# mitsuba-renderer/mitsuba2

Measured on AMD Instinct MI355X. Metric: Msamples/sec (whole node), 1080p/512spp path integrator, higher is better.
Workload: dtype f32

## Files before the change

mitsuba2_amd/csrc/device/resident_kernel.h:

```cpp
#ifndef MIW_KERNEL
#define MIW_KERNEL __global__
#endif
MIW_KERNEL __launch_bounds__(MIW_BLOCK) void k_init_pixels(RenderParams P, U4 *st_out, uint32_t *pixel_out, InitArgs A) {
    uint32_t lane = blockIdx.x * blockDim.x + threadIdx.x;
    if (lane >= P.n_lanes) return;
    uint32_t tile = lane >> A.bs2_log2, i = lane & ((1u << A.bs2_log2) - 1u);
    uint32_t b = A.tile_list ? A.tile_list[tile] : tile;
    uint32_t bx = b % A.blocks_x, by = b / A.blocks_x;
    uint32_t x, y;
    morton_decode2(i, x, y);
    int32_t bw = P.film.crop_w - (int32_t) (bx * A.bs), bh = P.film.crop_h - (int32_t) (by * A.bs);
    if (bw > (int32_t) A.bs) bw = (int32_t) A.bs;
    if (bh > (int32_t) A.bs) bh = (int32_t) A.bs;
    if ((int32_t) x >= bw || (int32_t) y >= bh) {
        U4 st; st.x = st.y = 0; st.z = LF_DONE; st.w = 0;
        st_out[lane] = st; pixel_out[lane] = 0;
        return;
    }
    uint32_t px = (uint32_t) P.film.crop_x + bx * A.bs + x, py = (uint32_t) P.film.crop_y + by * A.bs + y;
    pixel_out[lane] = px | (py << 16);
    st_out[lane] = lane_seed_state(A.base_seed + (uint64_t) A.block_ids[b] * (uint64_t) (A.bs * A.bs) + i);
}

struct TileArgs {
// ... 15 lines not shown
        ticks = 0; quarter = 0; tail_prio = 0; sample_end_ = spp;
        if (Jobs) job_pend() = 0u;
        if (Placed && Q->simd_ids) {
            const uint32_t hw = (uint32_t) __builtin_amdgcn_s_getreg(4 | (0 << 6) | (31 << 11)),
                           xcc = (uint32_t) __builtin_amdgcn_s_getreg(20 | (0 << 6) | (3 << 11));
            const uint32_t key = ((xcc & 15u) << 10) | (((hw >> 13) & 7u) << 7) | (((hw >> 12) & 1u) << 6) | (((hw >> 8) & 15u) << 2) | ((hw >> 4) & 3u);
            if (nq > 1u) { const uint32_t id = Q->simd_ids[1u + key]; q = id < nq ? id : key % nq; }
            else if ((threadIdx.x & 63u) == 0u) Q->simd_ids[1u + key] = 1u;
        }
    }
    uint32_t ticks, quarter, tail_prio, sample_end_; uint32_t *prog;
    __device__ __forceinline__ void tick(uint32_t sample_idx, bool has_pixel) {
        if (!tail_prio) { ++ticks; return; }
        if ((uint32_t) __builtin_amdgcn_readfirstlane((int) ++ticks) & 15u) return;
        if (has_pixel) atomicMin(prog, sample_idx);
        const uint32_t v = *prog;
        *prog = 0xffffffffu;
        const uint32_t v4 = 4u * v, se = sample_end_;
        uint32_t qtr = v == 0xffffffffu ? 3u : (v4 >= se ? 1u : 0u) + (v4 >= 2u * se ? 1u : 0u) + (v4 >= 3u * se ? 1u : 0u);
        qtr = (uint32_t) __builtin_amdgcn_readfirstlane((int) qtr);
        if (qtr == quarter) return;
        quarter = qtr;
        if (qtr == 0u) __builtin_amdgcn_s_setprio(3); else if (qtr == 1u) __builtin_amdgcn_s_setprio(2);
        else if (qtr == 2u) __builtin_amdgcn_s_setprio(1); else __builtin_amdgcn_s_setprio(0);
    }
    __device__ __forceinline__ void enable_tail_prio(uint32_t sample_end, uint32_t *wave_word) {
        tail_prio = 1u; sample_end_ = sample_end; quarter = 0; prog = wave_word; *prog = 0xffffffffu; __builtin_amdgcn_s_setprio(3);
    }
    typedef uint32_t U4v __attribute__((ext_vector_type(4)));
    __device__ __forceinline__ static uint32_t &job_pend() { __shared__ uint32_t s_job_pend[MIW_BLOCK]; return s_job_pend[threadIdx.x & (MIW_BLOCK - 1)]; }
    __device__ __forceinline__ bool exhausted() const { return !Jobs || !Q->job_chunk || job_pend() == 0xffffffffu; }
    __device__ __forceinline__ uint32_t job_end(uint32_t sample_idx, uint32_t sample_end) const {
        const uint32_t r = spp - sample_idx;
        return Jobs && (r & (r - 1u)) == 0u && r >= Q->job_min ? sample_idx : sample_end;
    }
    __device__ __forceinline__ bool fetch_job(uint32_t &pixel, U4 &st) {
        for (;;) {
            const uint32_t parked = job_pend();
            if (parked == 0xffffffffu) return false;
            uint32_t id = parked - 1u;
            const bool fresh = parked == 0u;
            const unsigned long long b = __ballot(fresh);
            if (fresh) {
                const uint32_t me = threadIdx.x & 63u, leader = (uint32_t) __ffsll((long long) b) - 1u;
                uint32_t base = 0;
                if (me == leader) base = atomicAdd(next_pixel, (uint32_t) __popcll(b));
                base = (uint32_t) __shfl((int) base, (int) leader, 64);
                id = base + __builtin_amdgcn_mbcnt_hi((uint32_t) (b >> 32), __builtin_amdgcn_mbcnt_lo((uint32_t) b, 0u));
                if (id >= Q->job_total) { job_pend() = 0xffffffffu; return false; }
            }
            const uint32_t j = id / n_lanes, slot = id - j * n_lanes;
            const uint32_t px = Q->pixel[slot];
            U4v w;
#if defined(__HIP_DEVICE_COMPILE__)
            asm volatile("global_load_dwordx4 %0, %1, off sc1\n\ts_waitcnt vmcnt(0)" : "=&v"(w) : "v"(Q->st + slot) : "memory");
#endif
            if (w.z & LF_DONE) { job_pend() = 0u; continue; }
            if (w.w != (j ? spp - (Q->job_pow >> (j - 1u)) : 0u)) { job_pend() = id + 1u; return false; }
            job_pend() = 0u;
            lane = slot; pixel = px;
            st.x = w.x; st.y = w.y; st.z = w.z; st.w = w.w;
            return true;
        }
    }
    __device__ __forceinline__ bool fetch(uint32_t &pixel, U4 &st) {
        if (Jobs && Q->job_chunk) return fetch_job(pixel, st);
        for (;;) {
            if (!Placed) {
                const unsigned long long b = __ballot(1);
                const uint32_t me = threadIdx.x & 63u, leader = (uint32_t) __ffsll((long long) b) - 1u;
                uint32_t base = 0;
                if (me == leader) base = atomicAdd(next_pixel, (uint32_t) __popcll(b));
                base = (uint32_t) __shfl((int) base, (int) leader, 64);
                const uint32_t l = base + __builtin_amdgcn_mbcnt_hi((uint32_t) (b >> 32), __builtin_amdgcn_mbcnt_lo((uint32_t) b, 0u));
                if (l >= n_lanes) return false;
                lane = l;
                st = Q->st[lane];
                if (st.z & LF_DONE) continue;
                pixel = Q->pixel[lane];
                return true;
            }
            if (dry >= nq) {
                if (nq > 1u) Q->simd_ids[0] = 1u;
                return false;
            }
            if (nq > 1u && __hip_atomic_load(Q->simd_ids, __ATOMIC_RELAXED, __HIP_MEMORY_SCOPE_AGENT)) { dry = nq; return false; }
            const unsigned long long all = __ballot(1);
            const uint32_t me = threadIdx.x & 63u, leader = (uint32_t) __ffsll((long long) all) - 1u;
            const uint32_t q_lead = (uint32_t) __shfl((int) q, (int) leader, 64);
            const bool mine = q == q_lead;
            const unsigned long long b = __ballot(mine);
            if (!mine) continue;
            uint32_t base = 0;
            if (me == leader) base = atomicAdd(next_pixel + q, (uint32_t) __popcll(b));
            base = (uint32_t) __shfl((int) base, (int) leader, 64);
            const uint32_t idx = base + __builtin_amdgcn_mbcnt_hi((uint32_t) (b >> 32), __builtin_amdgcn_mbcnt_lo((uint32_t) b, 0u));
            uint32_t l = idx;
            if (nq > 1u) {
                const uint32_t piece = idx < per ? Q->piece_list[q * MIW_PLACE_PIECES + (idx >> 6)] : 0xffffffffu;
                if (piece == 0xffffffffu) { q = q + 1u == nq ? 0u : q + 1u; ++dry; continue; }
                l = Q->lane_sorted[piece * Q->piece_a + (idx & 63u) * Q->piece_b];
                if (l >= n_lanes) continue;
            } else if (l >= n_lanes) { ++dry; continue; }
            lane = l;
            st = Q->st[lane];
            if (st.z & LF_DONE) continue;
            pixel = Q->pixel[lane];
            if (Placed) t_fetch = cost_clock();
            return true;
        }
    }
    __device__ __forceinline__ uint32_t cost_clock() const {
        return Clock ? (uint32_t) (__builtin_amdgcn_s_memtime() >> 8) : ticks;
    }
    __device__ __forceinline__ void store(U4 st) {
        if (Jobs && Q->job_chunk) {
            unsigned long long *words = reinterpret_cast<unsigned long long *>(Q->st + lane);
            __hip_atomic_store(words, (unsigned long long) st.x | ((unsigned long long) st.y << 32), __ATOMIC_RELAXED, __HIP_MEMORY_SCOPE_AGENT);
            asm volatile("s_waitcnt vmcnt(0)" ::: "memory");
            __hip_atomic_store(words + 1, (unsigned long long) st.z | ((unsigned long long) st.w << 32), __ATOMIC_RELAXED, __HIP_MEMORY_SCOPE_AGENT);
            return;
        }
        Q->st[lane] = st;
        if (Placed && Q->lane_cost) Q->lane_cost[lane] = cost_clock() - t_fetch + 1u;
        if (Groups && Q->group_done && (st.z & LF_DONE)) {
            __threadfence();
            const uint32_t g = lane >> Q->group_shift;
            if (atomicAdd(Q->group_done + g, 1u) + 1u == Q->group_expected[g]) {
                __threadfence_system();
                __hip_atomic_store(Q->group_flag + g, 1u, __ATOMIC_RELEASE, __HIP_MEMORY_SCOPE_SYSTEM);
            }
        }
    }
    __device__ __forceinline__ void put(uint32_t pixel, uint32_t sample_idx, V2 pos, const float *aovs) {
        if (Q->log_rec) {
            LogSink16<const float *> sink{ Q->log_rec, thr, film, lane, spp, Q->log_rej & 255u, Q->log_rej >> 8 };
            sink(pixel, sample_idx, pos, aovs);
        } else {
            LogSink sink; sink.log_pos = Q->log_pos; sink.log_val = Q->log_val; sink.lane = lane; sink.spp = spp; sink.warn_negative = warn_negative;
            sink(0u, sample_idx, pos, aovs);
        }
    }
};

#ifndef MIW_DIRECT_WAVES
#define MIW_DIRECT_WAVES 3
#endif
#ifndef MIW_PACKET_WAVES_ALL
#define MIW_PACKET_WAVES_ALL 4
#endif
#ifndef MIW_PACKET_WAVES
#define MIW_PACKET_WAVES 5
#endif
template <bool UseLog, int Tiny, int Mats = MATS_ALL, bool Analytic = (Tiny == 0), uint32_t Integ = INTEG_PATH, bool Groups = false, int Waves = 0>
__global__ __launch_bounds__(MIW_BLOCK, Waves ? Waves : Integ == INTEG_DIRECT ? MIW_DIRECT_WAVES : Tiny ? ((Mats == MATS_DIFFUSE && !MIW_SPECTRAL) ? (Tiny == 2 ? MIW_PACKET_WAVES : 4) : MIW_PACKET_WAVES_ALL) : MIW_TREE_WAVES) void k_path_resident(RenderParams P, SceneView sc, LaneQueues Q, double *accum, Counters *cnt,
                                                               TraceLds cfg, uint32_t sample_end, TileArgs T, uint32_t *next_pixel) {
    extern __shared__ uint4 smem[];
    stage_to_lds(sc, cfg, smem);
    const float *thr = stage_thresholds(smem, cfg, UseLog && Q.log_rec ? Q.log_thr : nullptr);
    constexpr bool Frames = MIW_LDS_TABLES && UseLog && Tiny != 0 && Integ != INTEG_DIRECT;
#if MIW_LDS_TABLES
    if constexpr (UseLog && Tiny != 0) stage_tables<true, mats_lights(Mats), mats_full(Mats), Frames>(sc, cfg, smem);
#endif
#if defined(MIW_SECTION_PROFILE) && defined(__HIP_DEVICE_COMPILE__)
    if ((threadIdx.x & 63u) == 0) { unsigned long long *b_ = miw_sec_buf(); for (int i = 0; i < 15; ++i) b_[i] = 0; b_[15] = __builtin_amdgcn_s_memtime(); }
#endif
    const uint32_t lane = blockIdx.x * blockDim.x + threadIdx.x;
    double *tile = reinterpret_cast<double *>(smem + T.geom16);
    int tile_x0 = 0, tile_y0 = 0;
    if (!UseLog && T.side) {
        const uint32_t lane0 = blockIdx.x * blockDim.x, t = lane0 >> T.bs2_log2, q0 = lane0 & ((1u << T.bs2_log2) - 1u);
        const uint32_t b = T.tile_list ? T.tile_list[t] : t;
        uint32_t qx, qy;
        morton_decode2(q0, qx, qy);
        const int margin = (int) (T.side - 16u) / 2;
        tile_x0 = (int) ((b % T.blocks_x) * T.bs + qx) - margin;
        tile_y0 = (int) ((b / T.blocks_x) * T.bs + qy) - margin;
        for (uint32_t i = threadIdx.x; i < T.side * T.side * MIW_FILM_CHANNELS; i += blockDim.x) tile[i] = 0.0;
        __syncthreads();
    }
    LaneCounters local; local.segments = local.samples = local.shadow_rays = 0;
    auto tr2 = [&](V3 o, float mint, V3 dE, float maxtE, bool hasE, V3 dS, float maxtS, bool hasS, F4 &hE, bool &occS) {
        trace2<Tiny, Analytic, Integ != INTEG_DIRECT>(sc, cfg, smem, o, mint, dE, maxtE, hasE, dS, maxtS, hasS, hE, occS);
    };
    if (UseLog) {
        QueueWork<Tiny != 0, false, Groups> work; work.Q = &Q; work.next_pixel = next_pixel; work.n_lanes = P.n_lanes; work.spp = P.spp; work.lane = 0; work.warn_negative = P.film.warn_negative;
        work.film = &P.film; work.thr = thr; work.init_queues(cfg.queues ? cfg.queues : 1u);
        __shared__ uint32_t s_prog[MIW_BLOCK / 64];
        if (cfg.tail_prio) work.enable_tail_prio(sample_end, &s_prog[threadIdx.x >> 6]);
        if constexpr (Integ == INTEG_DIRECT) pixel_stream_render_direct<Mats, Analytic>(P, sc, sample_end, work, tr2, &local);
        else pixel_stream_render<Mats, Analytic, Frames>(P, sc, sample_end, work, tr2, &local);
    } else if (lane < P.n_lanes) {
        U4 st = Q.st[lane];
        if (!(st.z & LF_DONE)) {
            const uint32_t pixel = Q.pixel[lane];
            if (T.side) {
                TileAdd add; add.tile = tile; add.x0 = tile_x0; add.y0 = tile_y0; add.side = (int) T.side;
                SplatXYSink<TileAdd> sink; sink.film = &P.film; sink.add = add;
                st = pixel_render<Integ, mats_nested(Mats) ? Mats : MATS_ALL>(P, sc, pixel, st, sample_end, tr2, sink, &local);
            } else {
                FilmAdd add; add.accum = accum;
                SplatSink<FilmAdd> sink; sink.film = &P.film; sink.add = add;
                st = pixel_render<Integ, mats_nested(Mats) ? Mats : MATS_ALL>(P, sc, pixel, st, sample_end, tr2, sink, &local);
            }
            Q.st[lane] = st;
        }
    }
    if (!UseLog && T.side) {
        __syncthreads();
        const int n = (int) (T.side * T.side);
        for (int i = (int) threadIdx.x; i < n * MIW_FILM_CHANNELS; i += (int) blockDim.x) {
            const double v = tile[i];
            if (v == 0.0) continue;
            const int texel = i / MIW_FILM_CHANNELS, k = i - texel * MIW_FILM_CHANNELS;
            const int fx = tile_x0 + texel % (int) T.side, fy = tile_y0 + texel / (int) T.side;
            unsafeAtomicAdd(accum + ((size_t) fy * P.film.crop_w + fx) * MIW_FILM_CHANNELS + k, v);
        }
    }
    unsigned long long a = wave_sum(local.segments), b = wave_sum(local.samples), c = wave_sum(local.shadow_rays);
    if ((threadIdx.x & 63) == 0) {
        Counters *shard = cnt + ((blockIdx.x * (MIW_BLOCK / 64) + (threadIdx.x >> 6)) & (MIW_CNT_SHARDS - 1));
        if (a) atomicAdd(&shard->segments, a);
        if (b) atomicAdd(&shard->samples, b);
        if (c) atomicAdd(&shard->shadow_rays, c);
#if defined(MIW_SECTION_PROFILE) && defined(__HIP_DEVICE_COMPILE__)
        { unsigned long long *b_ = miw_sec_buf(); for (int i = 0; i < 15; ++i) if (b_[i]) atomicAdd(&g_sections[i], b_[i]); }
#endif
    }
}
```

mitsuba2_amd/csrc/kernel_pick.h:

```cpp
#pragma once

namespace miw_pick {

enum : int { ALL = 0, DIFFUSE = 1, PLAIN = 2, TRIO = 3, NESTED = 4, LIGHTS = 5 };

struct Facts {
    bool tiny;
    bool small;
    bool diffuse_only, trio, nested, textured, lights_on;
    bool no_rects;
    bool trio_on;
};

struct Pick {
    int tiny;
    int mats;
    bool analytic;
};
inline bool operator==(const Pick &a, const Pick &b) { return a.tiny == b.tiny && a.mats == b.mats && a.analytic == b.analytic; }

inline bool trio_kernel(const Facts &f) { return f.trio && f.trio_on && f.no_rects && !f.textured; }

inline Pick resident_path(const Facts &f, bool with_trio) {
    if (f.tiny && f.diffuse_only) return { f.small ? 2 : 1, DIFFUSE, false };
    if (f.lights_on) return { f.tiny ? 1 : 0, LIGHTS, !f.tiny };
    if (f.nested) return { f.tiny ? 1 : 0, NESTED, !f.tiny };
    if (f.textured) return { f.tiny ? 1 : 0, ALL, !f.tiny };
    if (f.tiny) return { f.small ? 2 : 1, PLAIN, false };
    if (with_trio && trio_kernel(f)) return { 0, TRIO, false };
    return { 0, PLAIN, !f.no_rects };
}

inline Pick resident_direct(const Facts &f) {
    const int mats = f.lights_on ? LIGHTS : f.nested ? NESTED : f.textured ? ALL : PLAIN;
    return { f.tiny ? 1 : 0, mats, !f.tiny };
}

inline Pick resident_atomic(const Facts &f) {
    return { f.tiny ? 1 : 0, f.lights_on ? LIGHTS : f.nested ? NESTED : ALL, !f.tiny };
}

inline Pick tree_class(const Facts &f) {
    if (f.lights_on) return { 0, LIGHTS, true };
    if (f.nested) return { 0, NESTED, true };
    if (f.textured) return { 0, ALL, true };
    if (trio_kernel(f)) return { 0, TRIO, false };
    return { 0, PLAIN, !f.no_rects };
}

}
```

mitsuba2_amd/csrc/miw/path.h:

```cpp
#pragma once
#include "base.h"
#include "rng.h"
#include "scene.h"
#include "film.h"

namespace miw {

enum : uint32_t {
    LF_DEPTH_MASK  = 0x0fffu,
    LF_VALID_RAY   = 1u << 12,
    LF_PREV_DELTA  = 1u << 13,
    LF_HAS_SHADOW  = 1u << 14,
    LF_RAY_ACTIVE  = 1u << 15,
    LF_DONE        = 1u << 16,
    LF_DEAD_PENDING= 1u << 17,
};

struct LaneQueues {
    F4 *tp;
    F4 *res;
    U4 *st;
    F2 *pos;
    const uint32_t *pixel;
    F4 *ray_o;
    F4 *ray_d;
    F4 *hit;
    F4 *sh_d;
    F4 *sh_c;
    uint32_t *sh_vis;
    F2 *log_pos;
    F4 *log_val;
    U4 *log_rec;
    const float *log_thr;
    uint32_t log_rej;
    uint32_t *lane_cost; const uint32_t *lane_sorted; const uint32_t *piece_list; uint32_t *simd_ids; uint32_t piece_a, piece_b;
    uint32_t *group_done = nullptr; const uint32_t *group_expected = nullptr; uint32_t *group_flag = nullptr; uint32_t group_shift = 0;
    uint32_t job_chunk = 0, job_pow = 0, job_total = 0, job_min = 0x80000000u;
};

enum : uint32_t { INTEG_PATH = 0, INTEG_DIRECT = 1 };
struct DirectRec {
    uint32_t emitter_samples, bsdf_samples, hide_emitters;
    float frac_bsdf, frac_lum, weight_bsdf, weight_lum;
};

struct RenderParams {
    SensorRec sensor;
    FilmRec film;
    uint32_t spp;
    int32_t max_depth, rr_depth;
    uint32_t n_lanes;
    uint32_t integrator;
    DirectRec direct;
    uint32_t moment_pass;
    float cam_o[3];
    float crop_f[4];
};
MIW_HD void render_params_prepare(RenderParams &P) {
    const V3 o = sensor_origin(P.sensor);
    P.cam_o[0] = o.x; P.cam_o[1] = o.y; P.cam_o[2] = o.z;
    P.crop_f[0] = (float) P.film.crop_x; P.crop_f[1] = (float) P.film.crop_y; P.crop_f[2] = (float) P.film.crop_w; P.crop_f[3] = (float) P.film.crop_h;
}

struct Counters {
    unsigned long long segments;
    unsigned long long samples;
    unsigned long long shadow_rays;
    unsigned long long active_lanes;
};
struct LaneCounters { uint32_t segments, samples, shadow_rays; };

MIW_HD float next_1d(PCG32 &r) { return pcg32_next_f32(r); }
MIW_HD V2 next_2d(PCG32 &r) { float a = pcg32_next_f32(r); float b = pcg32_next_f32(r); return v2(a, b); }

struct LaneRegs {
    PCG32 rng;
    uint32_t flags, sample_idx;
    Spec tp, res; float eta, prev_pdf;
    V2 pos;
    Ray ray;
    Wavelengths wl; Spec ray_weight;
};

MIW_HD void lane_begin_sample(const RenderParams &P, uint32_t pixel, LaneRegs &L, uint32_t sample_end) {
    if (L.sample_idx >= sample_end) {
        L.flags = LF_DONE;
        L.ray.o = L.ray.d = v3(0.f); L.ray.mint = 0.f; L.ray.maxt = -1.f;
        return;
    }
    float px = (float) (pixel & 0xffffu), py = (float) (pixel >> 16);
    V2 j = next_2d(L.rng);
    L.pos = v2(px + j.x, py + j.y);
    const float wavelength_sample = next_1d(L.rng);
#if MIW_SPECTRAL
    sample_wavelengths(wavelength_sample, L.wl, L.ray_weight);
#else
    (void) wavelength_sample; L.ray_weight = spec(1.f);
#endif
    V2 adj = v2((L.pos.x - P.crop_f[0]) / P.crop_f[2],
                (L.pos.y - P.crop_f[1]) / P.crop_f[3]);
    L.ray = sensor_sample_ray(P.sensor, adj, v3(P.cam_o[0], P.cam_o[1], P.cam_o[2]));
    L.tp = spec(1.f); L.res = spec(0.f); L.eta = 1.f; L.prev_pdf = 0.f;
    L.flags = 1u | LF_RAY_ACTIVE;
}

template <typename Sink>
MIW_HD void lane_finish_sample(const RenderParams &P, uint32_t pixel, LaneRegs &L, Sink sink) {
#if MIW_SPECTRAL
    V3 xyz = spectrum_to_xyz(L.ray_weight * L.res, L.wl);
#else
    V3 xyz = srgb_to_xyz(L.res);
#endif
    float aovs[5] = { xyz.x, xyz.y, xyz.z, (L.flags & LF_VALID_RAY) ? 1.f : 0.f, 1.f };
    if (P.moment_pass) {
        const float sq[3] = { sqr(xyz.x), sqr(xyz.y), sqr(xyz.z) };
        bool ok = true;
        for (int k = 0; k < 3; ++k) ok = ok && isfinite_(aovs[k]) && isfinite_(sq[k]);
        if (P.moment_pass == 2u) { aovs[0] = sq[0]; aovs[1] = sq[1]; aovs[2] = sq[2]; }
        if (!ok) aovs[0] = __builtin_nanf("");
    }
    sink(pixel, L.sample_idx, L.pos, aovs);
    L.sample_idx++;
}

template <typename Add> struct SplatSink {
    const FilmRec *film; Add add;
    MIW_HD void operator()(uint32_t pixel, uint32_t, V2 pos, const float *aovs) const {
        film_splat(*film, (int) (pixel & 0xffffu), (int) (pixel >> 16), pos, aovs, add);
    }
};
template <typename AddXY> struct SplatXYSink {
    const FilmRec *film; AddXY add;
    MIW_HD void operator()(uint32_t pixel, uint32_t, V2 pos, const float *aovs) const {
        film_splat_xy(*film, (int) (pixel & 0xffffu), (int) (pixel >> 16), pos, aovs, add);
    }
};
struct LogSink {
    F2 *log_pos; F4 *log_val; uint32_t lane, spp;
    uint32_t warn_negative;
    MIW_HD void operator()(uint32_t, uint32_t sample_idx, V2 pos, const float *aovs) const {
        size_t i = (size_t) lane * spp + sample_idx;
        F2 p; p.x = sample_is_valid(aovs, warn_negative != 0) ? pos.x : __builtin_nanf(""); p.y = pos.y;
        F4 v; v.x = aovs[0]; v.y = aovs[1]; v.z = aovs[2]; v.w = aovs[3];
        log_pos[i] = p; log_val[i] = v;
    }
};

#ifndef MIW_LOG_NT
#define MIW_LOG_NT 1
#endif
template <typename Thr>
struct LogSink16 {
    U4 *log_rec; Thr thr; const FilmRec *film; uint32_t lane, spp, rej, il;
    MIW_HD void operator()(uint32_t pixel, uint32_t sample_idx, V2 pos, const float *aovs) const {
        const size_t i = log_index(il, lane, spp, sample_idx);
        U4 r; r.x = r.y = r.z = 0u; r.w = film_pack_meta(rej, rej, false);
        float least = aovs[0];
        bool ok = isfinite_(aovs[0]);
        for (int k = 1; k < MIW_FILM_CHANNELS; ++k) { least = __builtin_fminf(least, aovs[k]); ok = ok & isfinite_(aovs[k]); }
        ok = ok & ((film->warn_negative == 0) | (least >= -1e-5f));
        if (ok) {
            const uint32_t cx = film_class_of(thr, film_phase(*film, pos.x, (int) (pixel & 0xffffu), film->crop_x)),
                           cy = film_class_of(thr, film_phase(*film, pos.y, (int) (pixel >> 16), film->crop_y));
            r.x = f2u(aovs[0]); r.y = f2u(aovs[1]); r.z = f2u(aovs[2]); r.w = film_pack_meta(cx, cy, aovs[3] != 0.f);
        }
#if defined(__HIP_DEVICE_COMPILE__) && MIW_LOG_NT
        typedef uint32_t u4v_ __attribute__((ext_vector_type(4)));
        u4v_ v_; v_.x = r.x; v_.y = r.y; v_.z = r.z; v_.w = r.w;
        __builtin_nontemporal_store(v_, reinterpret_cast<u4v_ *>(log_rec + i));
#else
        log_rec[i] = r;
#endif
    }
};

MIW_HD void lane_load(const LaneQueues &Q, uint32_t lane, LaneRegs &L) {
    U4 st = Q.st[lane];
    L.rng.state = (uint64_t) st.x | ((uint64_t) st.y << 32);
    L.rng.inc = MIW_PCG32_SCALAR_INC;
    L.flags = st.z; L.sample_idx = st.w;
}
#if !MIW_SPECTRAL
MIW_HD void lane_load_path(const LaneQueues &Q, uint32_t lane, LaneRegs &L) {
    F4 a = Q.tp[lane], b = Q.res[lane];
    L.tp = v3(a.x, a.y, a.z); L.eta = a.w;
    L.res = v3(b.x, b.y, b.z); L.prev_pdf = b.w;
    L.pos = v2(0.f, 0.f);
}
MIW_HD void lane_store(const LaneQueues &Q, uint32_t lane, const LaneRegs &L, bool store_pos) {
    U4 st; st.x = (uint32_t) L.rng.state; st.y = (uint32_t) (L.rng.state >> 32);
    st.z = L.flags; st.w = L.sample_idx;
    Q.st[lane] = st;
    F4 a; a.x = L.tp.x; a.y = L.tp.y; a.z = L.tp.z; a.w = L.eta; Q.tp[lane] = a;
    F4 b; b.x = L.res.x; b.y = L.res.y; b.z = L.res.z; b.w = L.prev_pdf; Q.res[lane] = b;
    if (store_pos) { F2 p; p.x = L.pos.x; p.y = L.pos.y; Q.pos[lane] = p; }
    F4 o; o.x = L.ray.o.x; o.y = L.ray.o.y; o.z = L.ray.o.z; o.w = L.ray.mint; Q.ray_o[lane] = o;
    F4 d; d.x = L.ray.d.x; d.y = L.ray.d.y; d.z = L.ray.d.z; d.w = L.ray.maxt; Q.ray_d[lane] = d;
}
MIW_HD void lane_clear_shadow(const LaneQueues &Q, uint32_t lane) {
    F4 dead; dead.x = dead.y = dead.z = 0.f; dead.w = -1.f;
    Q.sh_d[lane] = dead;
}

MIW_HD void lane_init(const RenderParams &P, const LaneQueues &Q, uint32_t lane, uint32_t pixel, uint64_t seed) {
    LaneRegs L;
    pcg32_seed(L.rng, seed, MIW_PCG32_DEFAULT_STREAM);
    L.sample_idx = 0; L.flags = 0;
    L.tp = v3(1.f); L.res = v3(0.f); L.eta = 1.f; L.prev_pdf = 0.f; L.pos = v2(0.f, 0.f);
    L.ray.o = L.ray.d = v3(0.f); L.ray.mint = 0.f; L.ray.maxt = -1.f;
    lane_begin_sample(P, pixel, L, P.spp);
    lane_store(Q, lane, L, true);
    lane_clear_shadow(Q, lane);
    Q.sh_vis[lane] = 0;
}
MIW_HD void lane_init_unused(const LaneQueues &Q, uint32_t lane) {
    LaneRegs L;
    L.rng.state = 0; L.rng.inc = MIW_PCG32_SCALAR_INC; L.sample_idx = 0; L.flags = LF_DONE;
    L.tp = v3(0.f); L.res = v3(0.f); L.eta = 0.f; L.prev_pdf = 0.f; L.pos = v2(0.f, 0.f);
    L.ray.o = L.ray.d = v3(0.f); L.ray.mint = 0.f; L.ray.maxt = -1.f;
    lane_store(Q, lane, L, true);
    lane_clear_shadow(Q, lane);
    Q.sh_vis[lane] = 0;
}
#endif

#ifndef MIW_SECTION
#define MIW_SECTION(i) do { } while (0)
#endif

struct ShadowOut { bool has; V3 d; float maxt; Spec c; };

enum { STEP_CONTINUE = 0,
       STEP_FINISHED = 1,
       STEP_DEAD_PENDING = 2 };

enum { MATS_ALL = 0, MATS_DIFFUSE = 1, MATS_PLAIN = 2, MATS_TRIO = 3, MATS_NESTED = 4, MATS_LIGHTS = 5 };
MIW_HD constexpr bool mats_full(int mats) { return mats == MATS_ALL || mats == MATS_NESTED || mats == MATS_LIGHTS; }
MIW_HD constexpr bool mats_nested(int mats) { return mats == MATS_NESTED || mats == MATS_LIGHTS; }
MIW_HD constexpr bool mats_lights(int mats) { return mats == MATS_LIGHTS; }
template <int Mats = MATS_ALL, bool Analytic = true, bool Frames = false, typename PrevO, typename Cnt>
MIW_HD int path_step(const RenderParams &P, const SceneView &sc, LaneRegs &L, F4 h, PrevO prev_o,
                     ShadowOut &sh, Cnt *cnt_local) {
    sh.has = false;
    const uint32_t depth = L.flags & LF_DEPTH_MASK;
    const uint32_t tri_idx = f2u(h.w);
    const bool valid = tri_idx != MIW_MISS;
    const V3 ray_d = L.ray.d;

    SurfaceInteraction si;
    uint32_t bsdf_index = 0;
    int32_t emitter = -1;
    if (valid) hit_surface_interaction<Analytic, mats_full(Mats), Frames>(sc, tri_idx, h.x, h.y, h.z, prev_o, ray_d, si, bsdf_index, emitter);
    else emitter = miss_emitter<mats_lights(Mats)>(sc);
    if (depth == 1 && valid) L.flags |= LF_VALID_RAY;
    MIW_SECTION(7);

    if (emitter >= 0) {
        float emission_weight = 1.f;
        if (depth > 1) {
            float emitter_pdf = 0.f;
            if (!(L.flags & LF_PREV_DELTA)) {
                V3 d = ray_d; float dist = 0.f; V3 n = v3(0.f), ref_p = v3(0.f);
                if (valid) {
                    ref_p = prev_o();
                    d = si.p - ref_p;
                    dist = norm(d);
                    d = d / dist;
                    n = si.sh.n;
                }
                emitter_pdf = pdf_emitter_direction<Analytic, mats_lights(Mats)>(sc, (uint32_t) emitter, d, dist, n, ref_p);
            }
            emission_weight = mis_weight(L.prev_pdf, emitter_pdf);
        }
        Spec radiance = valid ? emitter_eval(sc.emitters[emitter], si.wi, L.wl) : miss_eval<mats_lights(Mats)>(sc, ray_d, L.wl);
        L.res = L.res + emission_weight * L.tp * radiance;
    }

    MIW_SECTION(8);
    bool active = valid;

    if ((int32_t) depth > P.rr_depth) {
        float q = min_(hmax(L.tp) * sqr(L.eta), .95f);
        active = (next_1d(L.rng) < q) && active;
        L.tp = L.tp * rcp(q);
    }

    if (depth >= (uint32_t) P.max_depth || !active) return STEP_FINISHED;

    if (cnt_local) cnt_local->segments++;
    BsdfSide bsdf;
    if (Mats == MATS_DIFFUSE) { bsdf.b = sc.bsdfs + bsdf_index; bsdf.flip = bsdf.none = false; bsdf.flags = BSDF_DiffuseReflection; }
    else bsdf = bsdf_side<mats_nested(Mats)>(sc.bsdfs, bsdf_index, si.wi);
    const uint32_t bflags = bsdf.flags;
    L.ray.o = si.p; L.ray.mint = spawn_mint(si.p);
    L.ray.d = v3(0.f); L.ray.maxt = -1.f;

    const TexCtx tc(L.wl, si.uv, mats_full(Mats) ? sc.bitmaps : nullptr, mats_full(Mats) ? sc.bsdf_tables : nullptr);
    constexpr bool Ext = mats_full(Mats);
    constexpr bool Trio = Mats == MATS_TRIO;
    constexpr bool Nested = mats_nested(Mats);

    if (bflags & BSDF_Smooth) {
        DirectionSample ds;
        Spec emitter_val = sample_emitter_direction<Analytic, mats_lights(Mats), Frames>(sc, si.p, next_2d(L.rng), ds, L.wl);
        if (ds.pdf != 0.f) {
            V3 wo = to_local(si.sh, ds.d);
            Spec bsdf_val = Mats == MATS_DIFFUSE ? diffuse_eval(*bsdf.b, si.wi, wo, tc) : bsdf_side_eval<Ext, Trio, Nested>(bsdf, si.wi, wo, tc);
            float bpdf = Mats == MATS_DIFFUSE ? diffuse_pdf(si.wi, wo) : bsdf_side_pdf<Ext, Trio, Nested>(bsdf, si.wi, wo, tc);
            float mis = (mats_lights(Mats) && ds.delta) ? 1.f : mis_weight(ds.pdf, bpdf);
            Spec c = mis * L.tp * bsdf_val * emitter_val;
            if (!all_zero(c)) {
                sh.has = true; sh.d = ds.d; sh.maxt = ds.dist * (1.f - MIW_SHADOW_EPSILON); sh.c = c;
                if (cnt_local) cnt_local->shadow_rays++;
            }
        }
    }

    MIW_SECTION(9);
    float s1 = next_1d(L.rng);
    V2 s2 = next_2d(L.rng);
    BSDFSample bs;
    Spec bsdf_val = Mats == MATS_DIFFUSE ? diffuse_sample(*bsdf.b, si.wi, s2, bs, tc) : bsdf_side_sample<Ext, Trio, Nested>(bsdf, si.wi, s1, s2, bs, tc);
    L.tp = L.tp * bsdf_val;
    if (all_zero(L.tp))
        return sh.has ? STEP_DEAD_PENDING : STEP_FINISHED;
    L.eta *= bs.eta;
    L.ray.d = to_world(si.sh, bs.wo);
    L.ray.maxt = MIW_INFINITY;
    L.prev_pdf = bs.pdf;
    L.flags = (L.flags & ~(LF_DEPTH_MASK | LF_PREV_DELTA)) | ((depth + 1) & LF_DEPTH_MASK)
            | ((bs.sampled_type & BSDF_Delta) ? LF_PREV_DELTA : 0u) | LF_RAY_ACTIVE;
    MIW_SECTION(10);
    return STEP_CONTINUE;
}

#if !MIW_SPECTRAL
template <int Mats = MATS_NESTED, typename Sink, typename Cnt>
MIW_HD uint32_t lane_shade(const RenderParams &P, const SceneView &sc, const LaneQueues &Q,
                           uint32_t lane, Cnt *cnt_local, Sink sink) {
    LaneRegs L;
    lane_load(Q, lane, L);
    if (L.flags & LF_DONE) return LF_DONE;
    lane_load_path(Q, lane, L);
    const bool had_shadow = (L.flags & LF_HAS_SHADOW) != 0;

    if (had_shadow) {
        if (Q.sh_vis[lane]) { F4 c = Q.sh_c[lane]; L.res = L.res + v3(c.x, c.y, c.z); }
        L.flags &= ~LF_HAS_SHADOW;
    }

    bool finished = false;

    if (L.flags & LF_DEAD_PENDING) {
        finished = true;
    } else {
        F4 rd = Q.ray_d[lane];
        L.ray.d = v3(rd.x, rd.y, rd.z);
        ShadowOut sh;
        const int r = path_step<Mats>(P, sc, L, Q.hit[lane],
                                [&]() { F4 ro = Q.ray_o[lane]; return v3(ro.x, ro.y, ro.z); }, sh, cnt_local);
        if (sh.has) {
            F4 sd; sd.x = sh.d.x; sd.y = sh.d.y; sd.z = sh.d.z; sd.w = sh.maxt;
            Q.sh_d[lane] = sd;
            F4 sc4; sc4.x = sh.c.x; sc4.y = sh.c.y; sc4.z = sh.c.z; sc4.w = 0.f;
            Q.sh_c[lane] = sc4;
            L.flags |= LF_HAS_SHADOW;
        }
        if (r == STEP_FINISHED) finished = true;
        else if (r == STEP_DEAD_PENDING)
            L.flags = (L.flags & ~LF_RAY_ACTIVE) | LF_DEAD_PENDING;
    }

    bool store_pos = false;
    if (finished) {
        const uint32_t pixel = Q.pixel[lane];
        F2 ps = Q.pos[lane]; L.pos = v2(ps.x, ps.y);
        lane_finish_sample(P, pixel, L, sink);
        if (cnt_local) cnt_local->samples++;
        L.flags = 0;
        lane_begin_sample(P, pixel, L, P.spp);
        store_pos = true;
    }
    lane_store(Q, lane, L, store_pos);
    if (had_shadow && !(L.flags & LF_HAS_SHADOW)) lane_clear_shadow(Q, lane);
    return L.flags;
}
#endif

template <int Mats = MATS_ALL, bool Analytic = true, bool Frames = false, typename Work, typename Trace2, typename Cnt>
MIW_HD void pixel_stream_render(const RenderParams &P, const SceneView &sc, uint32_t sample_end, Work &work,
                                Trace2 trace2, Cnt *cnt_local) {
    LaneRegs L;
    L.flags = LF_DONE; L.sample_idx = 0; L.rng.state = 0; L.rng.inc = MIW_PCG32_SCALAR_INC;
    uint32_t pixel = 0;
    bool have = false, dead_pending = false;
    ShadowOut sh; sh.has = false; sh.d = v3(0.f); sh.maxt = -1.f; sh.c = spec(0.f);
    auto sink = [&work](uint32_t px, uint32_t sample_idx, V2 pos, const float *aovs) { work.put(px, sample_idx, pos, aovs); };
    for (;;) {
        if (L.flags & LF_DONE) {
            if (have) {
                U4 st; st.x = (uint32_t) L.rng.state; st.y = (uint32_t) (L.rng.state >> 32);
                st.z = L.sample_idx >= P.spp ? (uint32_t) LF_DONE : 0u; st.w = L.sample_idx;
                work.store(st);
            }
            U4 st;
            have = work.fetch(pixel, st);
            if (!have) { if (work.exhausted()) break; continue; }
            L.rng.state = (uint64_t) st.x | ((uint64_t) st.y << 32);
            L.sample_idx = st.w; L.flags = 0;
            lane_begin_sample(P, pixel, L, sample_end);
            MIW_SECTION(0);
            continue;
        }
        work.tick(L.sample_idx, true);
        MIW_SECTION(0);
        const V3 o = L.ray.o;
        F4 h; bool occluded = false;
        trace2(o, L.ray.mint, L.ray.d, L.ray.maxt, !dead_pending, sh.d, sh.maxt, sh.has, h, occluded);
        if (sh.has && !occluded) L.res = L.res + sh.c;
        sh.has = false;
        int r = STEP_FINISHED;
        if (!dead_pending) {
            r = path_step<Mats, Analytic, Frames>(P, sc, L, h, [o]() { return o; }, sh, cnt_local);
            MIW_SECTION(4);
            if (r == STEP_DEAD_PENDING) { dead_pending = true; continue; }
            if (r == STEP_CONTINUE) continue;
        }
        dead_pending = false;
        lane_finish_sample(P, pixel, L, sink);
        if (cnt_local) cnt_local->samples++;
        L.flags = 0;
        lane_begin_sample(P, pixel, L, work.job_end(L.sample_idx, sample_end));
        MIW_SECTION(5);
    }
}

MIW_HD void lane_begin_path(LaneRegs &L) {
    L.tp = spec(1.f); L.res = spec(0.f); L.eta = 1.f; L.prev_pdf = 0.f;
    L.flags = 1u | LF_RAY_ACTIVE;
    L.sample_idx = 0; L.pos = v2(0.f, 0.f); L.ray_weight = spec(1.f);
}
template <int Mats = MATS_ALL, bool Analytic = true, typename Feed, typename Trace2, typename Cnt>
MIW_HD void ray_stream_sample(const RenderParams &P, const SceneView &sc, Feed &feed, Trace2 trace2, Cnt *cnt_local) {
    LaneRegs L;
    L.flags = LF_DONE; L.rng.state = 0; L.rng.inc = MIW_PCG32_SCALAR_INC;
    bool dead_pending = false;
    ShadowOut sh; sh.has = false; sh.d = v3(0.f); sh.maxt = -1.f; sh.c = spec(0.f);
    for (;;) {
        if (L.flags & LF_DONE) {
            if (!feed.fetch(L)) break;
            lane_begin_path(L);
            continue;
        }
        const V3 o = L.ray.o;
        F4 h; bool occluded = false;
        trace2(o, L.ray.mint, L.ray.d, L.ray.maxt, !dead_pending, sh.d, sh.maxt, sh.has, h, occluded);
        if (sh.has && !occluded) L.res = L.res + sh.c;
        sh.has = false;
        if (!dead_pending) {
            const int r = path_step<Mats, Analytic>(P, sc, L, h, [o]() { return o; }, sh, cnt_local);
            if (r == STEP_DEAD_PENDING) { dead_pending = true; continue; }
            if (r == STEP_CONTINUE) continue;
        }
        dead_pending = false;
        feed.store(L);
        if (cnt_local) cnt_local->samples++;
        L.flags = LF_DONE;
    }
}

template <int Mats, bool Analytic, typename Feed, typename Trace2, typename Cnt>
MIW_HD void ray_stream_sample_direct(const RenderParams &P, const SceneView &sc, Feed &feed, Trace2 trace2, Cnt *cnt_local);

template <int Mats, bool Analytic, typename Work, typename Trace2, typename Cnt>
MIW_HD void pixel_stream_render_direct(const RenderParams &P, const SceneView &sc, uint32_t sample_end, Work &work,
                                       Trace2 trace2, Cnt *cnt_local);

template <uint32_t Integ = INTEG_PATH, int Mats = MATS_NESTED, typename Trace2, typename Sink, typename Cnt>
MIW_HD U4 pixel_render(const RenderParams &P, const SceneView &sc, uint32_t pixel, U4 st, uint32_t sample_end,
                       Trace2 trace2, Sink sink, Cnt *cnt_local) {
    struct OnePixel {
        uint32_t pixel; U4 st; bool taken; Sink sink;
        MIW_HD bool fetch(uint32_t &px, U4 &s) { if (taken) return false; taken = true; px = pixel; s = st; return true; }
        MIW_HD void store(U4 s) { st = s; }
        MIW_HD bool exhausted() const { return true; }
        MIW_HD uint32_t job_end(uint32_t, uint32_t sample_end) const { return sample_end; }
        MIW_HD void tick(uint32_t, bool) { }
        MIW_HD void put(uint32_t px, uint32_t sample_idx, V2 pos, const float *aovs) { sink(px, sample_idx, pos, aovs); }
    } work{ pixel, st, false, sink };
    if constexpr (Integ == INTEG_DIRECT) pixel_stream_render_direct<Mats, true>(P, sc, sample_end, work, trace2, cnt_local);
    else pixel_stream_render<Mats>(P, sc, sample_end, work, trace2, cnt_local);
    return work.st;
}

MIW_HD U4 lane_seed_state(uint64_t seed) {
    PCG32 r; pcg32_seed(r, seed, MIW_PCG32_DEFAULT_STREAM);
    U4 st; st.x = (uint32_t) r.state; st.y = (uint32_t) (r.state >> 32); st.z = 0; st.w = 0;
    return st;
}

}
```

mitsuba2_amd/csrc/miw/scene.h:

```cpp
#pragma once
#include "base.h"
#include "shape.h"
#include "bsdf.h"
#include "envmap.h"
#include "light.h"

namespace miw {

#define MIW_MISS 0xffffffffu

struct BvhNode {
    float lo0[3], hi0[3];
    float lo1[3], hi1[3];
    int32_t child0, child1;
    int32_t parent;
    int32_t pad;
};

struct ShapeRec {
    uint32_t bsdf;
    int32_t  emitter;
    uint32_t flags;
    uint32_t pad;
};

struct EmitterRec {
    TexRec radiance;
    uint32_t shape;
    uint32_t tri_first;
    uint32_t tri_count;
    uint32_t valid_lo, valid_hi;
    float sum, normalization;
    uint32_t flags;
    uint32_t type;
};
enum : uint32_t { SHAPE_HAS_NORMALS = 1u, SHAPE_HAS_TEXCOORDS = 8u };

struct SceneView {
    const BvhNode *nodes;   uint32_t node_count;
    const Tri     *tris;    uint32_t tri_count;
    const float   *tri_vn;
    const float   *tri_uv;
    const ShapeRec *shapes; uint32_t shape_count;
    const BsdfRec  *bsdfs;  uint32_t bsdf_count;
    const EmitterRec *emitters; uint32_t emitter_count;
    float emitter_count_f, emitter_count_inv;
    const float *emit_tri;
    const float *emit_vnorm;
    const float *emit_pmf, *emit_cdf;
    const EnvmapRec *env;
    const AnalyticRec *rects;   uint32_t rect_count;
    const BitmapRec *bitmaps;
    const float *bsdf_tables;
    float accept_pad;
    const void *tri_bounds;
    const void *leaf_boxes;
    const struct Bvh4Node *nodes4;
    const struct Bvh8Node *nodes8;
    const float *env_top; uint32_t env_top_count, env_top_base;
    const TriFrame *tri_frames;
    const float *emit_face_n;
    const LightRec *lights;
    const LightRec *constant;
};
MIW_HD EnvTop env_top(const SceneView &sc) { EnvTop t; t.p = sc.env_top; t.count = sc.env_top_count; t.base = sc.env_top_base; return t; }
MIW_HD void scene_view_prepare(SceneView &v) {
    v.emitter_count_f = (float) v.emitter_count;
    v.emitter_count_inv = v.emitter_count ? 1.f / (float) v.emitter_count : 0.f;
}

MIW_HD PrimCtx prim_ctx(const SceneView &sc) { PrimCtx c; c.rects = sc.rects; c.accept_pad = sc.accept_pad; return c; }

template <bool Analytic, bool Texcoords, bool Frames = false, typename RayO>
MIW_HD void hit_surface_interaction(const SceneView &sc, uint32_t tri_idx, float t, float u, float v, RayO ray_o, V3 ray_d,
                                    SurfaceInteraction &si, uint32_t &bsdf_index, int32_t &emitter) {
    const Tri &tr = sc.tris[tri_idx];
    const ShapeRec &shape = sc.shapes[tr.shape];
    if (Analytic && tr.pad) {
        const AnalyticRec &a = sc.rects[tr.pad - 1u];
        if (a.kind == ANALYTIC_SPHERE) compute_surface_interaction_sphere(a, t, ray_o(), ray_d, si);
        else compute_surface_interaction_rect(a, t, u, v, ray_o(), ray_d, si);
    } else {
        const float *vn = (shape.flags & 1u) ? sc.tri_vn + 9 * (size_t) tri_idx : nullptr;
        const float *tc = (Texcoords && (shape.flags & SHAPE_HAS_TEXCOORDS)) ? sc.tri_uv + 6 * (size_t) tr.prim : nullptr;
        if constexpr (Frames) compute_surface_interaction(ld3(tr.p0), ld3(tr.p1), ld3(tr.p2), vn, tc, sc.tri_frames[tri_idx], t, u, v, ray_d, si);
        else compute_surface_interaction(ld3(tr.p0), ld3(tr.p1), ld3(tr.p2), vn, tc, t, u, v, ray_d, si);
    }
    si.shape = tr.shape; si.prim = tr.prim;
    emitter = shape.emitter; bsdf_index = shape.bsdf;
}

struct DirectionSample { V3 p, n, d; float dist, pdf; uint32_t emitter; bool delta; };

template <bool Lights = false>
MIW_HD int32_t miss_emitter(const SceneView &sc) {
    if (sc.env) return (int32_t) sc.env->emitter_index;
    if (Lights && sc.constant) return (int32_t) sc.constant->emitter_index;
    return -1;
}

MIW_HD MeshSampler emitter_mesh(const SceneView &sc, const EmitterRec &e) {
    MeshSampler m;
    m.tri = sc.emit_tri + 9 * (size_t) e.tri_first;
    m.vnorm = (e.flags & 1u) ? sc.emit_vnorm + 9 * (size_t) e.tri_first : nullptr;
    m.pmf = sc.emit_pmf + e.tri_first;
    m.cdf = sc.emit_cdf + e.tri_first;
    m.count = e.tri_count;
    m.valid_lo = e.valid_lo; m.valid_hi = e.valid_hi;
    m.sum = e.sum; m.normalization = e.normalization;
    return m;
}

MIW_HD void sphere_sample_direction(const AnalyticRec &r, V3 ref_p, V2 sample, DirectionSample &ds) {
    const V3 center = ld3(r.n);
    const float radius = r.radius;
    V3 dc_v = center - ref_p;
    float dc_2 = squared_norm(dc_v);
    float radius_adj = radius * (r.flip ? (1.f + MIW_RAY_EPSILON) : (1.f - MIW_RAY_EPSILON));
    if (dc_2 > sqr(radius_adj)) {
        float inv_dc = rsqrt(dc_2),
              sin_theta_max = radius * inv_dc,
              sin_theta_max_2 = sqr(sin_theta_max),
              inv_sin_theta_max = rcp(sin_theta_max),
              cos_theta_max = safe_sqrt(1.f - sin_theta_max_2);
        float sin_theta_2 = sin_theta_max_2 > 0.00068523f ? 1.f - sqr(fmadd(cos_theta_max - 1.f, sample.x, 1.f))
                                                          : sin_theta_max_2 * sample.x,
              cos_theta = safe_sqrt(1.f - sin_theta_2);
        float cos_alpha = sin_theta_2 * inv_sin_theta_max + cos_theta * safe_sqrt(fnmadd(sin_theta_2, sqr(inv_sin_theta_max), 1.f)),
              sin_alpha = safe_sqrt(fnmadd(cos_alpha, cos_alpha, 1.f));
        float sin_phi, cos_phi;
        sincos_(sample.y * (2.f * MIW_PI), sin_phi, cos_phi);
        Frame f; f.n = dc_v * -inv_dc;
        coordinate_system(f.n, f.s, f.t);
        V3 d = to_world(f, v3(cos_phi * sin_alpha, sin_phi * sin_alpha, cos_alpha));
        ds.p = v3(fmadd(d.x, radius, center.x), fmadd(d.y, radius, center.y), fmadd(d.z, radius, center.z));
        ds.n = d;
        ds.d = ds.p - ref_p;
        float dist2 = squared_norm(ds.d);
        ds.dist = __builtin_sqrtf(dist2);
        ds.d = ds.d / ds.dist;
        ds.pdf = (.5f * MIW_INV_PI) / (1.f - cos_theta_max);
        if (ds.dist == 0.f) ds.pdf = 0.f;
    } else {
        V3 d = square_to_uniform_sphere(sample);
        ds.p = v3(fmadd(d.x, radius, center.x), fmadd(d.y, radius, center.y), fmadd(d.z, radius, center.z));
        ds.n = d;
        ds.d = ds.p - ref_p;
        float dist2 = squared_norm(ds.d);
        ds.dist = __builtin_sqrtf(dist2);
        ds.d = ds.d / ds.dist;
        ds.pdf = r.inv_area * dist2 / abs_dot(ds.d, ds.n);
    }
    if (r.flip) ds.n = -ds.n;
}
MIW_HD float sphere_pdf_direction(const AnalyticRec &r, V3 ref_p, V3 ds_d, float ds_dist, V3 ds_n) {
    float sin_alpha = r.radius * rcp(norm(ld3(r.n) - ref_p)),
          cos_alpha = safe_sqrt(1.f - sin_alpha * sin_alpha);
    return sin_alpha < (1.f - MIW_EPSILON) ? (.5f * MIW_INV_PI) / (1.f - cos_alpha)
                                           : r.inv_area * sqr(ds_dist) / abs_dot(ds_d, ds_n);
}

#if MIW_SPECTRAL
MIW_HD Spec env_eval_uv_spec(const EnvmapRec &e, V2 uv, const Wavelengths &wl) {
    uv.x *= (float) (e.width - 1u); uv.y *= (float) (e.height - 1u);
    uint32_t px = (uint32_t) uv.x, py = (uint32_t) uv.y;
    if (px > e.width - 2u) px = e.width - 2u;
    if (py > e.height - 2u) py = e.height - 2u;
    const float w1x = uv.x - (float) px, w1y = uv.y - (float) py, w0x = 1.f - w1x, w0y = 1.f - w1y;
    const float *p = e.data + 4 * ((size_t) px + (size_t) py * e.width);
    const float *q = p + 4 * (size_t) e.width;
    const float f0 = fmadd(w0x, p[3], w1x * p[7]), f1 = fmadd(w0x, q[3], w1x * q[7]);
    const float f = fmadd(w0y, f0, w1y * f1);
    Spec r;
    for (int i = 0; i < MIW_SPEC_N; ++i) {
        const float l = wl.l[i];
        const float s00 = srgb_model_eval(p, l), s10 = srgb_model_eval(p + 4, l),
                    s01 = srgb_model_eval(q, l), s11 = srgb_model_eval(q + 4, l);
        const float s0 = fmadd(w0x, s00, w1x * s10), s1 = fmadd(w0x, s01, w1x * s11);
        const float sv = fmadd(w0y, s0, w1y * s1);
        const float wp = d65_eval(1.f * (1.f / 10568.f), l);
        r.c[i] = sv * wp * f * e.scale;
    }
    return r;
}
MIW_HD Spec env_eval_spec(const EnvmapRec &e, V3 d_world, const Wavelengths &wl) {
    return env_eval_uv_spec(e, env_dir_to_uv(xf_vector(e.to_local, d_world)), wl);
}
MIW_HD Spec env_sample_direction_spec(const EnvmapRec &e, V3 ref_p, V2 sample, V3 &d_out, float &dist_out, float &pdf_out,
                                      V3 &p_out, V3 &n_out, const Wavelengths &wl, EnvTop top = env_top_none()) {
    float pdf;
    V2 uv = hier2d_sample(e, sample, pdf, top);
    float theta = uv.y * MIW_PI, phi = uv.x * (2.f * MIW_PI);
    float st, ct, sp, cp;
    sincos_(theta, st, ct); sincos_(phi, sp, cp);
    V3 d = v3(cp * st, sp * st, ct);
    d = v3(d.y, d.z, -d.x);
    float dist = 2.f * e.radius;
    float inv_sin_theta = env_inv_sin_theta(d);
    d = xf_vector(e.to_world, d);
    p_out = ref_p + d * dist;
    n_out = -d;
    float ds_pdf = pdf > 0.f ? pdf * inv_sin_theta * (1.f / (2.f * sqr(MIW_PI))) : 0.f;
    d_out = d; dist_out = dist; pdf_out = ds_pdf;
    return env_eval_uv_spec(e, uv, wl) / ds_pdf;
}
#else
MIW_HD Spec env_sample_direction_spec(const EnvmapRec &e, V3 ref_p, V2 sample, V3 &d, float &dist, float &pdf, V3 &p, V3 &n, const Wavelengths &,
                                      EnvTop top = env_top_none()) {
    return env_sample_direction(e, ref_p, sample, d, dist, pdf, p, n, top);
}
MIW_HD Spec env_eval_spec(const EnvmapRec &e, V3 d, const Wavelengths &) { return env_eval(e, d); }
#endif

template <bool Analytic = true, bool Lights = false, bool Frames = false>
MIW_HD Spec emitter_sample_direction(const SceneView &sc, uint32_t index, V3 ref_p, V2 sample, DirectionSample &ds, const Wavelengths &wl) {
    const EmitterRec &e = sc.emitters[index];
    Spec value;
    ds.emitter = index;
    if (Lights) ds.delta = false;
    if (Lights && e.type >= EMITTER_POINT) {
        LightSample ls;
        value = light_sample_direction(sc.lights[e.tri_first], ref_p, sample, ls, wl);
        ds.p = ls.p; ds.n = ls.n; ds.d = ls.d; ds.dist = ls.dist; ds.pdf = ls.pdf; ds.delta = ls.delta;
    } else if (e.type == EMITTER_ENVMAP) {
        value = env_sample_direction_spec(*sc.env, ref_p, sample, ds.d, ds.dist, ds.pdf, ds.p, ds.n, wl, env_top(sc));
    } else {
        if (Analytic && (e.flags & 2u) && sc.rects[e.tri_first].kind == ANALYTIC_SPHERE) {
            sphere_sample_direction(sc.rects[e.tri_first], ref_p, sample, ds);
        } else {
            PositionSample ps;
            if (Analytic && (e.flags & 2u)) ps = rect_sample_position(sc.rects[e.tri_first], sample);
            else if constexpr (Frames) ps = mesh_sample_position(emitter_mesh(sc, e), sample, FaceNormalTable{ sc.emit_face_n + 4 * (size_t) e.tri_first });
            else ps = mesh_sample_position(emitter_mesh(sc, e), sample);
            ds.p = ps.p; ds.n = ps.n; ds.pdf = ps.pdf;
            ds.d = ds.p - ref_p;
            float dist_squared = squared_norm(ds.d);
            ds.dist = __builtin_sqrtf(dist_squared);
            ds.d = ds.d / ds.dist;
            float dp = abs_dot(ds.d, ds.n);
            ds.pdf *= (dp != 0.f) ? dist_squared / dp : 0.f;
        }
        bool active = dot(ds.d, ds.n) < 0.f && ds.pdf != 0.f;
        value = tex_eval(e.radiance, wl) / ds.pdf;
        if (!active) value = spec(0.f);
    }
    return value;
}

template <bool Analytic = true, bool Lights = false, bool Frames = false>
MIW_HD Spec sample_emitter_direction(const SceneView &sc, V3 ref_p, V2 sample, DirectionSample &ds, const Wavelengths &wl) {
    if (sc.emitter_count == 0) {
        ds.p = ds.n = ds.d = v3(0.f); ds.dist = 0.f; ds.pdf = 0.f; ds.emitter = 0;
        if (Lights) ds.delta = false;
        return spec(0.f);
    }
    uint32_t index = 0;
    float emitter_pdf = 1.f;
    if (sc.emitter_count > 1) {
        float n = sc.emitter_count_f;
        emitter_pdf = sc.emitter_count_inv;
        uint32_t i = (uint32_t) (sample.x * n);
        index = i < sc.emitter_count - 1 ? i : sc.emitter_count - 1;
        sample.x = (sample.x - (float) index * emitter_pdf) * n;
    }
    Spec value = emitter_sample_direction<Analytic, Lights, Frames>(sc, index, ref_p, sample, ds, wl);
    if (sc.emitter_count > 1) {
        ds.pdf *= emitter_pdf;
        value = value * rcp(emitter_pdf);
    }
    return value;
}

template <bool Analytic = true, bool Lights = false>
MIW_HD float emitter_pdf_direction(const SceneView &sc, uint32_t emitter, V3 ds_d, float ds_dist, V3 ds_n, V3 ref_p) {
    const EmitterRec &e = sc.emitters[emitter];
    if (Lights && e.type >= EMITTER_POINT) return light_pdf_direction(sc.lights[e.tri_first]);
    if (e.type == EMITTER_ENVMAP) return env_pdf_direction(*sc.env, ds_d);
    float dp = dot(ds_d, ds_n);
    bool active = dp < 0.f;
    float pdf;
    if (Analytic && (e.flags & 2u) && sc.rects[e.tri_first].kind == ANALYTIC_SPHERE) {
        pdf = sphere_pdf_direction(sc.rects[e.tri_first], ref_p, ds_d, ds_dist, ds_n);
    } else {
        pdf = e.normalization;
        float adp = abs_dot(ds_d, ds_n);
        pdf *= (adp != 0.f) ? (ds_dist * ds_dist) / adp : 0.f;
    }
    return active ? pdf : 0.f;
}
template <bool Analytic = true, bool Lights = false>
MIW_HD float pdf_emitter_direction(const SceneView &sc, uint32_t emitter, V3 ds_d, float ds_dist, V3 ds_n, V3 ref_p) {
    float value = emitter_pdf_direction<Analytic, Lights>(sc, emitter, ds_d, ds_dist, ds_n, ref_p);
    if (sc.emitter_count > 1) value = value * sc.emitter_count_inv;
    return value;
}

MIW_HD Spec emitter_eval(const EmitterRec &e, V3 wi, const Wavelengths &wl) {
    return wi.z > 0.f ? tex_eval(e.radiance, wl) : spec(0.f);
}
template <bool Lights = false>
MIW_HD Spec miss_eval(const SceneView &sc, V3 ray_d, const Wavelengths &wl) {
    if (Lights && !sc.env) return light_eval(*sc.constant, wl);
    return env_eval_spec(*sc.env, ray_d, wl);
}


MIW_HD float mis_weight(float pdf_a, float pdf_b) {
    pdf_a *= pdf_a; pdf_b *= pdf_b;
    return pdf_a > 0.f ? pdf_a / (pdf_a + pdf_b) : 0.f;
}

struct SensorRec {
    float sample_to_camera[16];
    float to_world[16];
    float near_clip, far_clip;
    float pp_offset[2];
};

MIW_HD V3 sensor_origin(const SensorRec &s) { return xf_point_affine(s.to_world, v3(0.f)); }
MIW_HD Ray sensor_sample_ray(const SensorRec &s, V2 position_sample, V3 origin) {
    V3 near_p = xf_point_persp(s.sample_to_camera,
                               v3(position_sample.x + s.pp_offset[0],
                                  position_sample.y + s.pp_offset[1], 0.f));
    V3 d = normalize(near_p);
    float inv_z = rcp(d.z);
    Ray r;
    r.mint = s.near_clip * inv_z;
    r.maxt = s.far_clip * inv_z;
    r.o = origin;
    r.d = xf_vector(s.to_world, d);
    return r;
}
MIW_HD Ray sensor_sample_ray(const SensorRec &s, V2 position_sample) { return sensor_sample_ray(s, position_sample, sensor_origin(s)); }

}
```

mitsuba2_amd/csrc/miwave.hip:

```cpp
#include <hip/hip_runtime.h>
#include <stdio.h>
#include <stdlib.h>
#include <string.h>
#include <stdarg.h>
#include <string>
#include <vector>
#include <chrono>
#include <atomic>
#include <cmath>
#include <map>
#include <string>
#include <algorithm>

#include "../../include/miwave.h"
#include "kernel_pick.h"
#if defined(MIW_CLASS_PART) || defined(MIW_AOV_UNIT)
#define MIW_KERNELS_ONLY 1
#endif
#if defined(MIW_SECTION_PROFILE)
__device__ unsigned long long g_sections[16];
#endif
#if defined(MIW_PHASE_STATS)
__device__ unsigned long long g_phase_stats[15];
#endif
#if defined(MIW_WALK_STATS)
__device__ unsigned long long g_walk_stats[8];
__device__ float g_walk_statsf[8];
#endif
#if defined(MIW_VERIFY_FILTER)
__device__ unsigned int g_verify_n;
__device__ float g_verify[16 * 16];
#endif
#if defined(MIW_SECTION_PROFILE) && defined(__HIP_DEVICE_COMPILE__)
__device__ __forceinline__ unsigned long long *miw_sec_buf() { __shared__ unsigned long long b[4][16]; return &b[threadIdx.x >> 6][0]; }
#define MIW_SECTION(i) do { const unsigned long long now_ = __builtin_amdgcn_s_memtime(); unsigned long long *b_ = miw_sec_buf(); \
        if ((threadIdx.x & 63u) == (unsigned) __ffsll((long long) __ballot(1)) - 1u) { b_[i] += now_ - b_[15]; b_[15] = now_; } } while (0)
#endif
#include "miw/base.h"
#include "miw/rng.h"
#include "miw/warp.h"
#include "miw/special.h"
#include "miw/shape.h"
#include "miw/bsdf.h"
#include "miw/scene.h"
#include "miw/film.h"
#include "miw/bvh.h"
#include "miw/path.h"
#include "miw/direct.h"
#if defined(MIW_KERNELS_ONLY)
#include "miw/bvh4.h"
#include "miw/bvh8.h"
#define MIW_KERNEL static __global__
#else
#include "rect_build.h"
#include "miw/film_gather.h"
#include "texture_build.h"
#include "bvh_build.h"
#include "bvh4_build.h"
#include "envmap_build.h"
#include "film_classes.h"
#include "lbvh_device.h"
#include "sah_device.h"
#include "bvh4_device.h"
#include "bvh8_device.h"
#include "film_reduce.h"
#endif

using namespace miw;

static_assert(sizeof(BvhNode) == 64, "BvhNode must be one 64-byte line");
static_assert(sizeof(Tri) == 48, "Tri must be 48 bytes");
static_assert(sizeof(BsdfRec) == 128 && sizeof(mi_bsdf) == 128, "bsdf record layout");
static_assert(sizeof(TexRec) == sizeof(mi_texture), "texture record layout");

#define MIW_BLOCK 256
#ifndef MIW_POOL_NW
#define MIW_POOL_NW 12
#endif
#define MIW_CNT_SHARDS 1024
#define MIW_BRUTE_MAX_LEAF 2
#define MIW_BRUTE_MAX_TRIS 64
#define MIW_PLACE_PIECES 4

#include "device/trace.h"
#include "device/wavefront_kernels.h"
#include "device/resident_kernel.h"
#include "device/phased_kernel.h"
#if !defined(MIW_KERNELS_ONLY)
#if !MIW_SPECTRAL
#include "device/pooled_kernel.h"
#endif
#include "device/stream_trace.h"
#include "device/film_kernels.h"
#endif
#include "device/eval_kernels.h"
#include "device/sample_kernel.h"
#include "device/class_instances.h"
#if defined(MIW_AOV_UNIT) || !defined(MIW_KERNELS_ONLY)
#include "miw/aov.h"
#include "miw/film_gather_n.h"
#include "device/aov_launch.h"
#if defined(MIW_AOV_UNIT) || !defined(MIW_SPLIT_AOV)
#include "device/aov_kernel.h"
#endif
#endif

#if !defined(MIW_KERNELS_ONLY)
__global__ void k_iota(uint32_t *out, uint32_t n) { const uint32_t i = blockIdx.x * blockDim.x + threadIdx.x; if (i < n) out[i] = i; }


template <typename T> struct DevBuf {
    T *p = nullptr; size_t n = 0;
    hipError_t resize(size_t count) {
        if (count <= n && p) return hipSuccess;
        if (p) (void) hipFree(p);
        p = nullptr; n = 0;
        if (count == 0) return hipSuccess;
        hipError_t e = hipMalloc((void **) &p, count * sizeof(T));
        if (e == hipSuccess) n = count;
        return e;
    }
    hipError_t upload(const std::vector<T> &v, hipStream_t s) {
        hipError_t e = resize(std::max<size_t>(v.size(), 1));
        if (e != hipSuccess || v.empty()) return e;
        return hipMemcpyAsync(p, v.data(), v.size() * sizeof(T), hipMemcpyHostToDevice, s);
    }
    void release() { if (p) (void) hipFree(p); p = nullptr; n = 0; }
};

template <typename T> struct TmpBuf : DevBuf<T> { TmpBuf() = default; TmpBuf(const TmpBuf &) = delete; ~TmpBuf() { this->release(); } };

struct KnobInfo { const char *name, *what; };
static const KnobInfo g_knobs[] = {
    { "MIW_DEBUG", "1: diagnostics on stderr (LDS layout, builder statistics, phase statistics of -DMIW_PHASE_STATS builds)" },
    { "MIW_DEBUG_ALLOC", "1: mi_bvh_build times its uploads and allocations" },
    { "MIW_DEVICE_BUILDER", "mi_bvh_build quality 0: sah (default) | lbvh: which device builder runs" },
    { "MIW_SAH_HUGE", "0: the device SAH sweep bins every candidate in one workgroup (round 4's form)" },
    { "MIW_LBVH_LEAF", "radix tree: triangles per leaf" },
    { "MIW_MAX_LEAF", "host SAH builder: triangles per leaf" },
    { "MIW_NO_STACK", "1: no LDS-stack walk (stackless BVH2 walk, wavefront plan)" },
    { "MIW_BVH4", "0: no 4-wide tree (the phase machine steps through the BVH2)" },
    { "MIW_BVH4_FAN", "2 | 3 | 4: widest node the 4-wide collapse may build" },
    { "MIW_BVH4_HOST", "1: the 4-wide tree is collapsed on the host from the read-back BVH2" },
    { "MIW_BVH8", "0: mi_bvh_build skips the 8-wide tree / mi_render keeps the 4-wide walk" },
    { "MIW_STACK8_FULL", "1: the 8-wide walk keeps the 16-entry LDS column instead of one entry per tree level" },
    { "MIW_ENV_TOP", "0: the environment warp's top levels are not staged in LDS" },
    { "MIW_PHASED", "0: tree scenes take the lock-step kernel instead of the phase machine" },
    { "MIW_PHASED_WAVES", "3 | 4: wavefronts per SIMD the phase machine is launched for" },
    { "MIW_TRIO", "0: MATS_PLAIN kernels where the MATS_TRIO class would do" },
    { "MIW_SHADE_VOTE", "num:den of the phase machine's shade vote" },
    { "MIW_LOOP_EXIT", "node:triangle hand-over ratios of the phase machine's walk loops" },
    { "MIW_POOLED", "1: tree scenes take k_path_pooled (walk jobs pooled across the workgroup; experimental, slower: DESIGN.md)" },
    { "MIW_POOL_SHAPE", "12x1 | 8x2: wavefronts per workgroup x pixels per lane of k_path_pooled" },
    { "MIW_POOL_VOTE", "shade_min:walk_min:node_min:tri_min:claim_min of k_path_pooled" },
    { "MIW_TAIL_PRIO", "0: no least-progress-first wave priorities" },
    { "MIW_WG_PER_CU", "workgroups per CU of the packet kernels' persistent grid" },
    { "MIW_PLACE", "0: shards of about one pixel per lane skip the measuring launch + placed queues" },
    { "MIW_JOB_CHUNK", "smallest chunk of a full frame's pixel jobs, in samples (a power of two; default 64, the phase machine 32): the pixels' sample streams are cut into halving chunks drawn chunk-major from one queue; 0: a job = all the samples of a pixel" },
    { "MIW_JOB_CHUNK_FORCE", "1: chunk jobs whatever the frame's size (tests of the hand-over between lanes)" },
    { "MIW_PACKET_SHARD4", "0: a plain-diffuse packet job of at most four wavefronts of pixels per SIMD keeps the five-wavefront (96-register) kernel" },
    { "MIW_PLACE_MEASURE", "divisor: the measuring launch runs spp / divisor samples" },
    { "MIW_PLACE_SPREAD", "0 | 1: placed pieces = consecutive sorted lanes | one lane of every cost stratum" },
    { "MIW_STREAM", "0: plan 1 walks with one kernel per list slice instead of the persistent stream kernel" },
    { "MIW_FILM_LEGACY", "1: the 24-byte position log + k_film_blocks for every filter" },
    { "MIW_FILM_LANES", "0 | 1 | 2: k_film_lanes off / over the tile-interleaved log / over [lane][sample]" },
    { "MIW_FILM_QUADS", "0 | 24 | 28 | 42 | 44: k_film_quads group shape (0: off)" },
    { "MIW_FILM_COLUMNS", "0 | 42 | 44 | 82: k_film_columns group shape" },
    { "MIW_FILM_GROUP", "2 | 3 | 4: k_film_groups group shape" },
    { "MIW_FL_NT", "0: k_film_lanes reads the log with plain instead of streaming loads" },
    { "MIW_FILM_OVERLAP", "1: part of the film replay of a full Cornell-class frame is queued on three more streams beside the path kernel, sets of 64-tile groups each behind the flags their last pixels raise (default 0: measured +0 - 1 %); 2: without the waits (timing probe: the film is the previous frame's)" },
    { "MIW_FILM_OVERLAP_SET", "groups of 64 tiles per launch of that replay (default 4)" },
    { "MIW_FILM_OVERLAP_ROOM", "workgroups the path kernel's grid is short of filling the device while the replay runs beside it (default 32: one per CU on 32 CUs)" },
    { "MIW_FILM_OVERLAP_LEAN", "0: the launches of that replay are the 168-register kernel (default 1: the 128-register form)" },
    { "MIW_FILM_OVERLAP_BESIDE", "groups of 64 tiles replayed beside the path kernel; the rest in one launch after it (default: three quarters)" },
    { "MIW_FILM_OVERLAP_PRIO", "s_setprio of the replay wavefronts that run beside the path kernel, 0 .. 3 (default 0)" },
    { "MIW_FQ_U", "2 | 4 | 8: records per trip of k_film_quads" },
    { "MIW_RCCL", "0: mi_film_reduce never uses RCCL (device add)" },
    { "MIW_RCCL_FORCE", "1: mi_film_reduce takes the RCCL branch for one context too (tests)" }
};
struct Options {
    std::map<std::string, std::string> v;
    void from_env() { for (const KnobInfo &k : g_knobs) if (const char *e = getenv(k.name)) v[k.name] = e; }
    static bool known(const char *name) { for (const KnobInfo &k : g_knobs) if (!strcmp(k.name, name)) return true; return false; }
    const char *get(const char *name) const { auto it = v.find(name); return it == v.end() ? nullptr : it->second.c_str(); }
    bool off(const char *name) const { const char *e = get(name); return e && atoi(e) == 0; }
    bool on(const char *name) const { const char *e = get(name); return e && atoi(e) != 0; }
    int num(const char *name, int unset) const { const char *e = get(name); return e ? atoi(e) : unset; }
};

struct mi_ctx {
    int device = 0;
    Options opt;
    hipStream_t stream = nullptr;
    std::string error;
    std::atomic<int> cancel{0};

    std::vector<Tri> tris_in;
    std::vector<float> tri_vn_in;
    std::vector<float> tri_uv_in;
    std::vector<ShapeRec> shapes;
    std::vector<AnalyticRec> rects;
    std::vector<BsdfRec> bsdfs; bool diffuse_only = false;
    bool trio = false;
    bool nested = false;
    bool textured = false;
    std::vector<float> bsdf_tables; DevBuf<float> d_bsdf_tables;
    std::vector<EmitterRec> emitters;
    std::vector<LightRec> lights; DevBuf<LightRec> d_lights; int32_t constant_light = -1;
    bool lights_on = false;
    std::vector<float> emit_tri, emit_vnorm, emit_pmf, emit_cdf;
    bool have_scene = false, have_bvh = false;

    DevBuf<BvhNode> d_nodes; DevBuf<Tri> d_tris; DevBuf<float> d_tri_vn, d_tri_uv, d_bitmap_data; DevBuf<BitmapRec> d_bitmaps; uint32_t bitmap_count = 0;
    DevBuf<ShapeRec> d_shapes; DevBuf<BsdfRec> d_bsdfs; DevBuf<EmitterRec> d_emitters; DevBuf<AnalyticRec> d_rects;
    DevBuf<float> d_emit_tri, d_emit_vnorm, d_emit_pmf, d_emit_cdf;
    DevBuf<LeafBox> d_leaf_boxes; DevBuf<TriBounds> d_tri_bounds; DevBuf<Bvh4Node> d_nodes4; uint32_t nodes4_count = 0, nodes4_stack = 0;
    DevBuf<Bvh8Node> d_nodes8; DevBuf<Tri> d_tris8; DevBuf<float> d_tri_vn8; uint32_t nodes8_count = 0, nodes8_depth = 0;
    DevBuf<float> d_env_data, d_env_levels; DevBuf<EnvmapRec> d_env; EnvmapRec env_host{}; size_t env_levels_total = 0;
    bool have_env = false;
    SceneView view{};
    TraceLds lds_cfg{}; size_t lds_bytes = 0;

    DevBuf<F4> q_tp, q_res, q_ray_o, q_ray_d, q_hit, q_sh_d, q_sh_c;
    DevBuf<U4> q_st; DevBuf<F2> q_pos; DevBuf<uint32_t> q_pixel, q_sh_vis;
    DevBuf<double> d_accum; DevBuf<unsigned char> d_out;
    DevBuf<F2> q_log_pos; DevBuf<F4> q_log_val;
    DevBuf<U4> q_log_rec;
    FilmClasses classes; FilmRec classes_of{}; bool classes_valid = false;
    DevBuf<float> d_fc_thr, d_fc_w;
    DevBuf<uint32_t> d_next_pixel; int cu_count = 256;
    DevBuf<uint32_t> d_lane_cost, d_cost_sorted, d_lane_iota, d_lane_sorted, d_piece_list, d_simd_ids;
    DevBuf<unsigned char> d_place_tmp;
    DevBuf<uint32_t> d_lists, d_list_counts;
    DevBuf<uint32_t> d_block_ids, d_tile_list; DevBuf<int32_t> d_block_tile; DevBuf<float> d_tiles;
    DevBuf<Counters> d_cnt;
    Counters *h_cnt = nullptr;
    std::vector<uint32_t> h_piece_list, h_simd_ids;
    hipStream_t stream2[3] = { nullptr, nullptr, nullptr }; hipEvent_t ev_fork = nullptr, ev_join[3] = { nullptr, nullptr, nullptr };
    DevBuf<uint32_t> d_group_done, d_group_expected; uint32_t *h_group_flag = nullptr; uint32_t group_flag_cap = 0;
    std::vector<uint32_t> h_group_expected; std::vector<int32_t> h_block_tile;
    int overlap_state = -1;
    bool replay_enqueued = false;
    uint32_t replay_launches = 0;

    DevBuf<unsigned char> d_sample_stage; DevBuf<uint32_t> d_next_ray;

    std::vector<hipEvent_t> ev_pool;
    mi_counters counters{};
};

static mi_status fail(mi_ctx *c, mi_status code, const char *fmt, ...) {
    char buf[512];
    va_list ap; va_start(ap, fmt); vsnprintf(buf, sizeof buf, fmt, ap); va_end(ap);
    if (c) c->error = buf;
    return code;
}
#define HIP_TRY(c, expr) do { hipError_t e_ = (expr); if (e_ != hipSuccess) \
    return fail(c, MI_ERR_DEVICE, "%s failed: %s (%s:%d)", #expr, hipGetErrorString(e_), __FILE__, __LINE__); } while (0)

static thread_local std::string g_global_error;

extern "C" {

int32_t mi_spectrum_channels(void) { return MIW_SPEC_N; }

mi_status mi_device_count(int32_t *count) {
    if (!count) return MI_ERR_INVALID;
    int n = 0;
    hipError_t e = hipGetDeviceCount(&n);
    if (e != hipSuccess) { *count = 0; g_global_error = hipGetErrorString(e); return MI_ERR_DEVICE; }
    *count = n;
    return MI_OK;
}

mi_status mi_create(int32_t device, mi_ctx **out) {
    if (!out) return MI_ERR_INVALID;
    *out = nullptr;
    int n = 0;
    if (hipGetDeviceCount(&n) != hipSuccess || n <= 0) { g_global_error = "no HIP device visible"; return MI_ERR_DEVICE; }
    if (device < 0 || device >= n) { g_global_error = "device index out of range"; return MI_ERR_INVALID; }
    if (hipSetDevice(device) != hipSuccess) { g_global_error = "hipSetDevice failed"; return MI_ERR_DEVICE; }
    mi_ctx *c = new mi_ctx();
    c->device = device;
    c->opt.from_env();
    { hipDeviceProp_t prop; if (hipGetDeviceProperties(&prop, device) == hipSuccess && prop.multiProcessorCount > 0) c->cu_count = prop.multiProcessorCount; }
    if (hipHostMalloc((void **) &c->h_cnt, sizeof(Counters) * MIW_CNT_SHARDS) != hipSuccess) { delete c; g_global_error = "hipHostMalloc failed"; return MI_ERR_DEVICE; }
    *out = c;
    g_live_contexts.fetch_add(1);
    return MI_OK;
}

void mi_destroy(mi_ctx *c) {
    if (!c) return;
    (void) hipSetDevice(c->device);
    (void) hipDeviceSynchronize();
    c->d_nodes.release(); c->d_tris.release(); c->d_tri_vn.release(); c->d_tri_uv.release(); c->d_bitmap_data.release(); c->d_bitmaps.release(); c->d_bsdf_tables.release(); c->d_shapes.release(); c->d_rects.release(); c->d_bsdfs.release();
    c->d_emitters.release(); c->d_lights.release(); c->d_leaf_boxes.release(); c->d_tri_bounds.release(); c->d_nodes4.release(); c->d_nodes8.release(); c->d_tris8.release(); c->d_tri_vn8.release(); c->d_env_data.release(); c->d_env_levels.release(); c->d_env.release(); c->d_emit_tri.release(); c->d_emit_vnorm.release(); c->d_emit_pmf.release(); c->d_emit_cdf.release();
    c->q_tp.release(); c->q_res.release(); c->q_ray_o.release(); c->q_ray_d.release(); c->q_hit.release();
    c->q_sh_d.release(); c->q_sh_c.release(); c->q_st.release(); c->q_pos.release(); c->q_pixel.release(); c->q_sh_vis.release();
    c->d_accum.release(); c->d_out.release(); c->d_next_pixel.release(); c->d_lane_cost.release(); c->d_cost_sorted.release(); c->d_lane_iota.release(); c->d_lane_sorted.release(); c->d_place_tmp.release(); c->d_piece_list.release(); c->d_simd_ids.release(); c->d_lists.release(); c->d_list_counts.release(); c->d_block_ids.release(); c->d_tile_list.release(); c->d_cnt.release();
    c->q_log_pos.release(); c->q_log_val.release(); c->q_log_rec.release(); c->d_fc_thr.release(); c->d_fc_w.release(); c->d_block_tile.release(); c->d_tiles.release();
    for (hipEvent_t e : c->ev_pool) (void) hipEventDestroy(e);
    c->d_group_done.release(); c->d_group_expected.release(); c->d_sample_stage.release(); c->d_next_ray.release();
    if (c->h_group_flag) (void) hipHostFree(c->h_group_flag);
    if (c->ev_fork) (void) hipEventDestroy(c->ev_fork);
    for (int i = 0; i < 3; ++i) { if (c->ev_join[i]) (void) hipEventDestroy(c->ev_join[i]); if (c->stream2[i]) (void) hipStreamDestroy(c->stream2[i]); }
    if (c->h_cnt) (void) hipHostFree(c->h_cnt);
    delete c;
    if (g_live_contexts.fetch_sub(1) == 1) rccl_release_comms();
}

mi_status mi_set_stream(mi_ctx *c, void *s) { if (!c) return MI_ERR_INVALID; c->stream = (hipStream_t) s; return MI_OK; }

const char *mi_last_error(mi_ctx *c) { return c ? c->error.c_str() : g_global_error.c_str(); }

mi_status mi_set_option(mi_ctx *c, const char *name, const char *value) {
    if (!c || !name) return MI_ERR_INVALID;
    if (!Options::known(name)) return fail(c, MI_ERR_INVALID, "mi_set_option: unknown option %s", name);
    if (value) c->opt.v[name] = value; else c->opt.v.erase(name);
    return MI_OK;
}
const char *mi_get_option(mi_ctx *c, const char *name) { return c && name ? c->opt.get(name) : nullptr; }
int32_t mi_option_count(void) { return (int32_t) (sizeof(g_knobs) / sizeof(g_knobs[0])); }
const char *mi_option_name(int32_t i) { return i >= 0 && i < mi_option_count() ? g_knobs[i].name : nullptr; }
const char *mi_option_help(int32_t i) { return i >= 0 && i < mi_option_count() ? g_knobs[i].what : nullptr; }

mi_status mi_cancel(mi_ctx *c) { if (!c) return MI_ERR_INVALID; c->cancel.store(1); return MI_OK; }

mi_status mi_get_counters(mi_ctx *c, mi_counters *out) {
    if (!c || !out) return MI_ERR_INVALID;
    *out = c->counters;
    return MI_OK;
}

mi_status mi_film_alloc(mi_ctx *c, uint64_t count, void **film) {
    if (!c || !film) return MI_ERR_INVALID;
    *film = nullptr;
    HIP_TRY(c, hipSetDevice(c->device));
    float *p = nullptr;
    HIP_TRY(c, hipMalloc((void **) &p, std::max<uint64_t>(count, 1) * sizeof(float)));
    hipError_t e = hipMemsetAsync(p, 0, count * sizeof(float), c->stream);
    if (e == hipSuccess) e = hipStreamSynchronize(c->stream);
    if (e != hipSuccess) { (void) hipFree(p); return fail(c, MI_ERR_DEVICE, "mi_film_alloc: %s", hipGetErrorString(e)); }
    *film = p;
    return MI_OK;
}
void mi_film_free(mi_ctx *c, void *film) {
    if (!c || !film) return;
    (void) hipSetDevice(c->device);
    (void) hipFree(film);
}
mi_status mi_film_download(mi_ctx *c, const void *film, float *host, uint64_t count) {
    if (!c || !film || !host) return MI_ERR_INVALID;
    HIP_TRY(c, hipSetDevice(c->device));
    HIP_TRY(c, hipMemcpyAsync(host, film, count * sizeof(float), hipMemcpyDeviceToHost, c->stream));
    HIP_TRY(c, hipStreamSynchronize(c->stream));
    return MI_OK;
}
mi_status mi_film_reduce(mi_ctx *const *ctxs, void *const *films, int32_t n, uint64_t count, int32_t root, int32_t *how) {
    if (how) *how = MI_REDUCE_NONE;
    if (!ctxs || !films || n < 1 || root < 0 || root >= n) return MI_ERR_INVALID;
    for (int32_t i = 0; i < n; ++i) if (!ctxs[i] || !films[i]) return MI_ERR_INVALID;
    mi_ctx *r = ctxs[root];
    for (int32_t i = 0; i < n; ++i) { HIP_TRY(r, hipSetDevice(ctxs[i]->device)); HIP_TRY(r, hipStreamSynchronize(ctxs[i]->stream)); }
    const bool force_rccl = r->opt.on("MIW_RCCL_FORCE");
    if (count == 0 || (n == 1 && !force_rccl)) return MI_OK;
    std::vector<int> devs(n);
    bool distinct = true;
    for (int32_t i = 0; i < n; ++i) { devs[i] = ctxs[i]->device; for (int32_t j = 0; j < i; ++j) distinct = distinct && devs[j] != devs[i]; }
    if (distinct) {
        std::lock_guard<std::mutex> lock(g_rccl_mutex);
        if (g_rccl.load(!r->opt.off("MIW_RCCL"))) {
// ... 114 lines not shown
    if (s->rectangle_count && !s->rectangles) return fail(c, MI_ERR_INVALID, "scene: rectangle_count without rectangles");
    std::vector<int32_t> shape_rect(s->shape_count, -1);
    for (uint32_t k = 0; k < s->rectangle_count; ++k) {
        const mi_rectangle &q = s->rectangles[k];
        if (q.shape >= s->shape_count || !(s->shapes[q.shape].flags & MI_SHAPE_RECTANGLE) || shape_rect[q.shape] >= 0)
            return fail(c, MI_ERR_INVALID, "rectangle %u: shape %u is not a (single) MI_SHAPE_RECTANGLE shape", k, q.shape);
        shape_rect[q.shape] = (int32_t) k;
        c->rects.push_back(rect_record(q.to_world, q.to_object, q.shape, s->shapes[q.shape].first_face));
        if (!(c->rects.back().inv_area > 0.f) || !isfinite_(c->rects.back().inv_area))
            return fail(c, MI_ERR_INVALID, "rectangle %u: degenerate to_world", k);
    }
    if (s->sphere_count && !s->spheres) return fail(c, MI_ERR_INVALID, "scene: sphere_count without spheres");
    for (uint32_t k = 0; k < s->sphere_count; ++k) {
        const mi_sphere &q = s->spheres[k];
        if (q.shape >= s->shape_count || !(s->shapes[q.shape].flags & MI_SHAPE_SPHERE) || shape_rect[q.shape] >= 0)
            return fail(c, MI_ERR_INVALID, "sphere %u: shape %u is not a (single) MI_SHAPE_SPHERE shape", k, q.shape);
        if (!(q.radius > 0.f) || !isfinite_(q.radius)) return fail(c, MI_ERR_INVALID, "sphere %u: radius must be positive", k);
        shape_rect[q.shape] = (int32_t) c->rects.size();
        c->rects.push_back(sphere_record(q.center, q.radius, q.flip_normals != 0, q.to_world, q.to_object, q.shape, s->shapes[q.shape].first_face));
    }
    for (uint32_t i = 0; i < s->shape_count; ++i)
        if ((s->shapes[i].flags & (MI_SHAPE_RECTANGLE | MI_SHAPE_SPHERE)) && shape_rect[i] < 0)
            return fail(c, MI_ERR_INVALID, "shape %u: no mi_rectangle record", i);
    if (!build_face_texcoords(s, c->tri_uv_in)) return fail(c, MI_ERR_INVALID, "scene: MI_SHAPE_HAS_TEXCOORDS without vertex_texcoords (or a vertex index out of range)");
    c->tris_in.resize((size_t) s->face_count + c->rects.size());
    c->tri_vn_in.clear();
    if (any_normals) c->tri_vn_in.assign(c->tris_in.size() * 9, 0.f);
    for (uint32_t f = 0; f < s->face_count; ++f) {
        if (face_shape[f] == 0xffffffffu) return fail(c, MI_ERR_INVALID, "face %u belongs to no shape", f);
        Tri &t = c->tris_in[f];
        if (shape_rect[face_shape[f]] >= 0) {
            Tri two[2];
            analytic_bounding_tris(c->rects[shape_rect[face_shape[f]]], (uint32_t) shape_rect[face_shape[f]], two);
            t = two[0]; c->tris_in[(size_t) s->face_count + shape_rect[face_shape[f]]] = two[1];
            continue;
        }
        for (int k = 0; k < 3; ++k) {
            uint32_t vi = s->faces[3 * f + k];
            if (vi >= s->vertex_count) return fail(c, MI_ERR_INVALID, "face %u: vertex index out of range", f);
            float *dst = k == 0 ? t.p0 : (k == 1 ? t.p1 : t.p2);
            memcpy(dst, s->vertex_positions + 3 * (size_t) vi, 12);
            if (any_normals && (c->shapes[face_shape[f]].flags & 1u))
                memcpy(&c->tri_vn_in[(size_t) f * 9 + 3 * k], s->vertex_normals + 3 * (size_t) vi, 12);
        }
        t.shape = face_shape[f]; t.prim = f; t.pad = 0;
    }
    c->bsdfs.resize(s->bsdf_count);
    for (uint32_t i = 0; i < s->bsdf_count; ++i) {
        const mi_bsdf &b = s->bsdfs[i];
        BsdfRec r; int slot = 0;
        if (s->bsdf_table_floats && !s->bsdf_tables) return fail(c, MI_ERR_INVALID, "scene: bsdf_table_floats without bsdf_tables");
        if (const char *why = bsdf_record_from_abi(b, s->bitmap_count, s->bsdf_table_floats, r, &slot))
            return slot < 0 ? fail(c, MI_ERR_INVALID, "bsdf %u: %s", i, why) : fail(c, MI_ERR_INVALID, "bsdf %u: texture %d: %s", i, slot, why);
        if (!(b.flags & MI_BSDF_FLAG_TWOSIDED) && b.type != BSDF_TYPE_MASK && b.type != BSDF_TYPE_BLEND) r.back = 0;
        c->bsdfs[i] = r;
    }
    for (uint32_t i = 0; i < s->bsdf_count; ++i)
        if (const char *why = bsdf_chain_check(c->bsdfs, i, s->bitmaps)) return fail(c, MI_ERR_INVALID, "bsdf %u: %s", i, why);
    c->diffuse_only = true;
    for (const BsdfRec &r : c->bsdfs) if (r.type != BSDF_TYPE_DIFFUSE || (r.flags & BSDF_REC_TWOSIDED)) c->diffuse_only = false;
    if (!c->tri_uv_in.empty()) c->diffuse_only = false;
    for (const BsdfRec &r : c->bsdfs) if (bsdf_uses_bitmap(r)) c->diffuse_only = false;
    {
        std::vector<BitmapRec> recs; uint32_t bad = 0;
        if (const char *why = build_bitmap_table(s, recs, &bad)) return fail(c, MI_ERR_INVALID, "bitmap %u: %s", bad, why);
        std::vector<size_t> first(recs.size() + 1, 0);
        for (size_t i = 0; i < recs.size(); ++i) first[i + 1] = first[i] + (size_t) recs[i].width * recs[i].height * recs[i].channels;
        HIP_TRY(c, c->d_bitmap_data.resize(std::max<size_t>(first.back(), 1)));
        for (size_t i = 0; i < recs.size(); ++i) {
            HIP_TRY(c, hipMemcpyAsync(c->d_bitmap_data.p + first[i], recs[i].data, (first[i + 1] - first[i]) * sizeof(float), hipMemcpyHostToDevice, c->stream));
            recs[i].data = c->d_bitmap_data.p + first[i];
        }
        HIP_TRY(c, hipStreamSynchronize(c->stream));
        HIP_TRY(c, c->d_bitmaps.upload(recs, c->stream));
        c->bitmap_count = (uint32_t) recs.size();
    }
    c->trio = true;
    for (const BsdfRec &r : c->bsdfs) if (r.type != BSDF_TYPE_DIFFUSE && r.type != BSDF_TYPE_DIELECTRIC && r.type != BSDF_TYPE_ROUGHCONDUCTOR) c->trio = false;
    c->textured = !c->tri_uv_in.empty();
    for (const BsdfRec &r : c->bsdfs) if (bsdf_uses_bitmap(r) || bsdf_is_extended(r)) c->textured = true;
    c->nested = false;
    for (const BsdfRec &r : c->bsdfs) if (bsdf_is_nested(r)) c->nested = c->textured = true;
    c->bsdf_tables.assign(s->bsdf_tables, s->bsdf_tables + s->bsdf_table_floats);
    HIP_TRY(c, c->d_bsdf_tables.upload(c->bsdf_tables, c->stream));
    HIP_TRY(c, hipStreamSynchronize(c->stream));
    c->emitters.clear(); c->emit_tri.clear(); c->emit_vnorm.clear(); c->emit_pmf.clear(); c->emit_cdf.clear();
    bool any_emit_normals = false;
    auto push_env = [&]() { EmitterRec r; memset(&r, 0, sizeof r); r.type = EMITTER_ENVMAP; r.shape = 0xffffffffu; c->emitters.push_back(r); };
    c->lights.clear(); c->constant_light = -1; c->lights_on = s->light_count != 0;
    auto push_light = [&](uint32_t k) {
        const mi_light &l = s->lights[k];
        LightRec q; memset(&q, 0, sizeof q);
#if MIW_SPECTRAL
        memcpy(&q.value, &l.value_tex, sizeof(TexRec));
#else
        q.value.type = TEX_RGB; memcpy(q.value.v, l.value, 12);
#endif
        q.type = EMITTER_POINT + l.type; q.emitter_index = (uint32_t) c->emitters.size();
        memcpy(q.position, l.position, 12); memcpy(q.direction, l.direction, 12); memcpy(q.to_object, l.to_object, 64);
        q.cutoff_angle = l.cutoff_angle; q.cos_cutoff_angle = l.cos_cutoff_angle; q.cos_beam_width = l.cos_beam_width; q.inv_transition_width = l.inv_transition_width;
        q.dist = 2.f * light_bsphere_radius(l.bsphere_radius);
        EmitterRec r; memset(&r, 0, sizeof r); r.type = q.type; r.shape = 0xffffffffu; r.tri_first = (uint32_t) c->lights.size();
        if (l.type == MI_LIGHT_CONSTANT) c->constant_light = (int32_t) c->lights.size();
        c->lights.push_back(q); c->emitters.push_back(r);
    };
    auto push_specials = [&]() { while (c->emitters.size() < emitter_total && slot_light[c->emitters.size()] != -1) { const int32_t k = slot_light[c->emitters.size()]; if (k == -2) push_env(); else push_light((uint32_t) k); } };
    for (uint32_t i = 0; i < s->emitter_count; ++i) {
        if (s->light_count) push_specials();
        else if (s->envmap && s->envmap->emitter_index == i) push_env();
        const mi_emitter &e = s->emitters[i];
        if (e.shape >= s->shape_count) return fail(c, MI_ERR_INVALID, "emitter %u: shape index out of range", i);
        const mi_shape &sh = s->shapes[e.shape];
        if (sh.emitter != (int32_t) i) return fail(c, MI_ERR_INVALID, "emitter %u: shape %u does not point back to it", i, e.shape);
        if (sh.face_count == 0) return fail(c, MI_ERR_INVALID, "emitter %u: cannot create sampling table for an empty mesh", i);
        EmitterRec r; memset(&r, 0, sizeof r);
#if MIW_SPECTRAL
        if (e.radiance_tex.type != MI_TEX_D65 && e.radiance_tex.type != MI_TEX_SRGB_D65 && e.radiance_tex.type != MI_TEX_UNIFORM)
            return fail(c, MI_ERR_INVALID, "emitter %u: the scalar_spectral library needs a spectral radiance record", i);
        memcpy(&r.radiance, &e.radiance_tex, sizeof(TexRec));
#else
        r.radiance.type = TEX_RGB; memcpy(r.radiance.v, e.radiance, 12);
#endif
        if (shape_rect[e.shape] >= 0) {
            const AnalyticRec &q = c->rects[shape_rect[e.shape]];
            r.shape = e.shape; r.tri_first = (uint32_t) shape_rect[e.shape]; r.tri_count = 0; r.flags = 2u;
            r.valid_lo = r.valid_hi = 0; r.normalization = q.inv_area; r.sum = rcp(q.inv_area);
            c->emitters.push_back(r);
            continue;
        }
        r.shape = e.shape; r.tri_first = (uint32_t) c->emit_pmf.size(); r.tri_count = sh.face_count;
        r.flags = (sh.flags & MI_SHAPE_HAS_NORMALS) ? 1u : 0u;
        any_emit_normals = any_emit_normals || r.flags;
        double sum = 0.0; uint32_t vlo = 0xffffffffu, vhi = 0;
        for (uint32_t k = 0; k < sh.face_count; ++k) {
            const Tri &t = c->tris_in[sh.first_face + k];
            float area = face_area(ld3(t.p0), ld3(t.p1), ld3(t.p2));
            if (area < 0.f) return fail(c, MI_ERR_INVALID, "emitter %u: negative face area", i);
            c->emit_pmf.push_back(area);
            sum += (double) area;
            c->emit_cdf.push_back((float) sum);
            if (area > 0.f) { if (vlo == 0xffffffffu) vlo = k; vhi = k; }
            for (int q = 0; q < 3; ++q) c->emit_tri.push_back(t.p0[q]);
            for (int q = 0; q < 3; ++q) c->emit_tri.push_back(t.p1[q]);
            for (int q = 0; q < 3; ++q) c->emit_tri.push_back(t.p2[q]);
            for (int q = 0; q < 9; ++q)
                c->emit_vnorm.push_back(r.flags ? c->tri_vn_in[(size_t) (sh.first_face + k) * 9 + q] : 0.f);
        }
        if (vlo == 0xffffffffu) return fail(c, MI_ERR_INVALID, "emitter %u: no probability mass found", i);
        r.valid_lo = vlo; r.valid_hi = vhi;
        r.sum = (float) sum; r.normalization = (float) (1.0 / sum);
        c->emitters.push_back(r);
    }
    if (!any_emit_normals) c->emit_vnorm.clear();
    if (s->light_count) push_specials();
    else if (s->envmap && s->envmap->emitter_index >= s->emitter_count) push_env();
    if (c->lights_on) { c->nested = c->textured = true; c->diffuse_only = c->trio = false; }

    HIP_TRY(c, hipSetDevice(c->device));
    c->have_env = false;
#if MIW_SPECTRAL
    if (s->envmap && !s->envmap->density)
        return fail(c, MI_ERR_INVALID, "envmap: the scalar_spectral library needs mi_envmap::density (its texels are model coefficients, include/miwave.h)");
#endif
    if (s->envmap) {
        EnvmapTables t = envmap_build(*s->envmap);
        if (!t.ok) return fail(c, MI_ERR_INVALID, "envmap: needs >= 2x2 texels, a non-zero luminance sum and an invertible to_world");
        HIP_TRY(c, c->d_env_data.upload(t.data, c->stream));
        HIP_TRY(c, c->d_env_levels.upload(t.levels, c->stream));
        t.rec.data = c->d_env_data.p; t.rec.levels = c->d_env_levels.p;
        c->env_host = t.rec; c->env_levels_total = t.levels.size();
        std::vector<EnvmapRec> one(1, t.rec);
        HIP_TRY(c, c->d_env.upload(one, c->stream));
        HIP_TRY(c, hipStreamSynchronize(c->stream));
        c->have_env = true;
    }
    HIP_TRY(c, c->d_shapes.upload(c->shapes, c->stream));
    HIP_TRY(c, c->d_tri_uv.upload(c->tri_uv_in, c->stream));
    HIP_TRY(c, c->d_rects.upload(c->rects, c->stream));
    HIP_TRY(c, c->d_bsdfs.upload(c->bsdfs, c->stream));
    HIP_TRY(c, c->d_emitters.upload(c->emitters, c->stream));
    HIP_TRY(c, c->d_lights.upload(c->lights, c->stream));
    HIP_TRY(c, c->d_emit_tri.upload(c->emit_tri, c->stream));
    HIP_TRY(c, c->d_emit_vnorm.upload(c->emit_vnorm, c->stream));
    HIP_TRY(c, c->d_emit_pmf.upload(c->emit_pmf, c->stream));
    HIP_TRY(c, c->d_emit_cdf.upload(c->emit_cdf, c->stream));
    HIP_TRY(c, hipStreamSynchronize(c->stream));
    c->have_scene = true;
    return MI_OK;
}

#define MIW_LDS_PER_CU (160u * 1024u)
#define MIW_LDS_PER_WORKGROUP (MIW_LDS_PER_CU / 4u)
#define MIW_LDS_STATIC 1024u
#define MIW_LDS_GRANULE 512u
static size_t lds_table_bytes(const mi_ctx *c, uint32_t words[12], bool with_tris) {
    words[0] = (uint32_t) (c->shapes.size() * sizeof(ShapeRec) / 4); words[1] = (uint32_t) (c->bsdfs.size() * sizeof(BsdfRec) / 4);
    words[2] = (uint32_t) (c->emitters.size() * sizeof(EmitterRec) / 4);
    words[3] = (uint32_t) c->emit_tri.size(); words[4] = (uint32_t) c->emit_vnorm.size(); words[5] = (uint32_t) c->emit_pmf.size(); words[6] = (uint32_t) c->emit_cdf.size();
    words[7] = with_tris ? (uint32_t) (c->tris_in.size() * sizeof(Tri) / 4) : 0u;
    words[8] = with_tris ? (uint32_t) c->tri_vn_in.size() : 0u; words[9] = with_tris ? (uint32_t) c->tri_uv_in.size() : 0u;
    words[10] = with_tris ? (uint32_t) (c->tris_in.size() * sizeof(TriFrame) / 4) : 0u;
    words[11] = with_tris ? (uint32_t) (c->emit_tri.size() / 9 * 4) : 0u;
    size_t total = 0;
    for (int k = 0; k < 12; ++k) total += ((size_t) words[k] + 3u) / 4u * 16u;
    total += c->lights.size() * sizeof(LightRec);
    return total;
}

mi_status mi_bvh_build(mi_ctx *c, int32_t quality) {
    if (!c) return MI_ERR_INVALID;
    if (!c->have_scene) return fail(c, MI_ERR_STATE, "mi_bvh_build: no scene uploaded");
    const bool force_tree = (quality & MI_BVH_FORCE_TREE) != 0;
    const int32_t quality_flags = quality;
    quality &= ~(MI_BVH_FORCE_TREE | MI_BVH_NO_LEAF_FILTER | MI_BVH_RADIX_TREE);
    if (quality != 1 && quality != 0) return fail(c, MI_ERR_INVALID, "mi_bvh_build: quality must be 0 or 1");
    auto t0 = std::chrono::steady_clock::now();
    HIP_TRY(c, hipSetDevice(c->device));
    const float pad_unit = scene_pad_unit(c->tris_in);
    BvhBuildResult r;
    uint32_t node_count = 0, tri_count = (uint32_t) c->tris_in.size(), depth = 0;
    bool built_on_device = false;
    bool wide_on_device = false; uint32_t dev4_nodes = 0, dev4_stack = 0;
    const bool wide_on = !c->opt.off("MIW_BVH4");
    const bool wide8_on = wide_on && !c->opt.off("MIW_BVH8") && !c->opt.get("MIW_BVH4_FAN");
    uint32_t dev8_nodes = 0, dev8_depth = 0; double ms_bvh8 = 0.0;
    std::vector<uint32_t> sah_level_start;
    int max_fan = 4;
    if (const char *e = c->opt.get("MIW_BVH4_FAN")) max_fan = std::min(4, std::max(2, atoi(e)));
    double ms_bvh4 = 0.0;
    uint32_t tab_words_[12];
    const bool tiny = c->tris_in.size() <= MIW_BRUTE_MAX_TRIS && !force_tree && c->rects.empty() &&
                      (!MIW_LDS_TABLES || lds_table_bytes(c, tab_words_, true) <= 24u * 1024u);
    if (quality == 0 && !tiny && tri_count >= 2) {
        hipStream_t s = c->stream;
        const int n = (int) tri_count;
        TmpBuf<Tri> d_in; TmpBuf<float> d_vn_in; TmpBuf<uint64_t> d_keys, d_keys_sorted; TmpBuf<uint32_t> d_bounds, d_arrivals, d_height, d_span, d_first;
        uint32_t lbvh_leaf = 2u;
        if (const char *e = c->opt.get("MIW_LBVH_LEAF")) lbvh_leaf = (uint32_t) std::min(16, std::max(1, atoi(e)));
        if ((uint32_t) n <= lbvh_leaf) lbvh_leaf = 1u;
        TmpBuf<LbvhBox> d_boxes; TmpBuf<LbvhLinks> d_inner; TmpBuf<int32_t> d_leaf_parent; TmpBuf<unsigned char> d_tmp;
        auto free_tmp = [&]() { d_in.release(); d_vn_in.release(); d_keys.release(); d_keys_sorted.release(); d_bounds.release();
                                d_arrivals.release(); d_height.release(); d_boxes.release(); d_inner.release(); d_leaf_parent.release(); d_tmp.release();
                                d_span.release(); d_first.release(); };
        auto lap_t = std::chrono::steady_clock::now();
        auto lap = [&](const char *what) {
            if (!c->opt.get("MIW_DEBUG_ALLOC")) return;
            (void) hipStreamSynchronize(s);
            const auto now = std::chrono::steady_clock::now();
            fprintf(stderr, "[miwave]   build set-up: %-28s %8.2f ms\n", what, std::chrono::duration<double, std::milli>(now - lap_t).count());
            lap_t = now;
        };
        HIP_TRY(c, d_in.upload(c->tris_in, s));
        lap("triangle upload");
        if (!c->tri_vn_in.empty()) HIP_TRY(c, d_vn_in.upload(c->tri_vn_in, s));
        lap("vertex-normal upload");
        HIP_TRY(c, c->d_nodes.resize(n)); HIP_TRY(c, c->d_tris.resize(n)); HIP_TRY(c, d_height.resize(n));
        if (!c->tri_vn_in.empty()) HIP_TRY(c, c->d_tri_vn.resize((size_t) n * 9));
        lap("node / triangle buffers");
        const dim3 blk(256), grd((unsigned) ((n + 255) / 256));
        enum { DEV_SAH = 0, DEV_LBVH = 1 } dev_builder = (quality_flags & MI_BVH_RADIX_TREE) ? DEV_LBVH : DEV_SAH;
        if (const char *e = c->opt.get("MIW_DEVICE_BUILDER")) {
            if (!strcmp(e, "lbvh")) dev_builder = DEV_LBVH; else if (!strcmp(e, "sah")) dev_builder = DEV_SAH;
        }
        bool sah_need_host = false;
        if (dev_builder == DEV_SAH) {
            uint32_t max_leaf = 4u;
            if (const char *e = c->opt.get("MIW_MAX_LEAF")) max_leaf = (uint32_t) std::min(16, std::max(1, atoi(e)));
            const uint32_t un = (uint32_t) n;
            const float pad = 2.f * pad_unit;
            TmpBuf<SahPrim> d_prim; TmpBuf<uint32_t> d_ia, d_ib, d_flags, d_rank; TmpBuf<SahCand> d_ca, d_cb; TmpBuf<SahDecision> d_dec; TmpBuf<SahState> d_state;
            TmpBuf<unsigned char> d_scan_tmp; TmpBuf<SahHuge> d_huge;
            HIP_TRY(c, d_huge.resize(MIW_SAH_HUGE_CANDS));
            HIP_TRY(c, d_prim.resize(un)); HIP_TRY(c, d_ia.resize(un)); HIP_TRY(c, d_ib.resize(un)); HIP_TRY(c, d_flags.resize(un)); HIP_TRY(c, d_rank.resize(un));
            HIP_TRY(c, d_ca.resize(un)); HIP_TRY(c, d_cb.resize(un)); HIP_TRY(c, d_dec.resize(un)); HIP_TRY(c, d_state.resize(1));
            size_t scan_bytes = 0;
            HIP_TRY(c, rocprim::exclusive_scan(nullptr, scan_bytes, d_flags.p, d_rank.p, 0u, (size_t) n, rocprim::plus<uint32_t>(), s));
            HIP_TRY(c, d_scan_tmp.resize(scan_bytes + 16));
            lap("builder temporaries");
            HIP_TRY(c, hipStreamSynchronize(s));
            const auto t_setup = std::chrono::steady_clock::now();
            hipLaunchKernelGGL(k_sah_prims, grd, blk, 0, s, d_in.p, un, pad, d_prim.p, d_ia.p);
            const SahCand root = { 0u, un, -1, 0u };
            HIP_TRY(c, hipMemcpyAsync(d_ca.p, &root, sizeof root, hipMemcpyHostToDevice, s));
            HIP_TRY(c, hipMemsetAsync(d_state.p, 0, sizeof(SahState), s));
            std::vector<uint32_t> level_start{ 0u };
            uint32_t n_cand = 1u, base = 0u, level = 0u;
            bool big_left = true;
            uint32_t level_max = un;
            const bool huge_on = !c->opt.off("MIW_SAH_HUGE");
            while (n_cand > 0u && !sah_need_host) {
                const SahCand *cur = (level & 1u) ? d_cb.p : d_ca.p; SahCand *nxt = (level & 1u) ? d_ca.p : d_cb.p;
                const uint32_t *ic = (level & 1u) ? d_ib.p : d_ia.p; uint32_t *in = (level & 1u) ? d_ia.p : d_ib.p;
                const bool all_big = n_cand <= 512u;
                const uint32_t none = 0u, all = 0xffffffffu;
                const bool huge = huge_on && level_max > MIW_SAH_HUGE && n_cand <= MIW_SAH_HUGE_CANDS;
                if (huge) {
                    const dim3 hgrid(n_cand, (level_max + MIW_SAH_SLICE - 1u) / MIW_SAH_SLICE);
                    const uint32_t words = n_cand * (uint32_t) (sizeof(SahHuge) / 4u);
                    hipLaunchKernelGGL(k_sah_huge_init, dim3((words + 255u) / 256u), dim3(256), 0, s, d_huge.p, n_cand);
                    hipLaunchKernelGGL(k_sah_huge_box, hgrid, dim3(1024), 0, s, cur, n_cand, ic, d_prim.p, d_huge.p);
                    hipLaunchKernelGGL(k_sah_huge_bins, hgrid, dim3(1024), 0, s, cur, n_cand, ic, d_prim.p, level, d_huge.p);
                    hipLaunchKernelGGL(k_sah_huge_finish, dim3(n_cand), dim3(64), 0, s, cur, n_cand, level, max_leaf, d_huge.p, d_dec.p, d_flags.p, d_state.p);
                }
                if (all_big || big_left) hipLaunchKernelGGL(k_sah_decide<1024>, dim3(n_cand), dim3(1024), 0, s, cur, n_cand, ic, d_prim.p, level, max_leaf, d_dec.p, d_flags.p, d_state.p, all_big ? none : MIW_SAH_BIG, huge ? MIW_SAH_HUGE : all);
                if (!all_big) hipLaunchKernelGGL(k_sah_decide<64>, dim3(n_cand), dim3(64), 0, s, cur, n_cand, ic, d_prim.p, level, max_leaf, d_dec.p, d_flags.p, d_state.p, none, big_left ? MIW_SAH_BIG : all);
                HIP_TRY(c, rocprim::exclusive_scan(d_scan_tmp.p, scan_bytes, d_flags.p, d_rank.p, 0u, (size_t) n_cand, rocprim::plus<uint32_t>(), s));
// ... 274 lines not shown
    if (hits->v) HIP_TRY(c, hipMemcpyAsync(hits->v, out.p + 2 * n, n * sizeof(float), hipMemcpyDeviceToHost, c->stream));
    if (hits->prim) HIP_TRY(c, hipMemcpyAsync(hits->prim, outu.p, n * sizeof(uint32_t), hipMemcpyDeviceToHost, c->stream));
    if (hits->shape) HIP_TRY(c, hipMemcpyAsync(hits->shape, outu.p + n, n * sizeof(uint32_t), hipMemcpyDeviceToHost, c->stream));
    HIP_TRY(c, hipStreamSynchronize(c->stream));
    return MI_OK;
}

mi_status mi_ray_intersect(mi_ctx *c, const mi_rays_soa *rays, mi_surface_interaction *si, uint64_t n) {
    if (!c || !rays || !si) return MI_ERR_INVALID;
    if (!c->have_bvh) return fail(c, MI_ERR_STATE, "mi_ray_intersect: call mi_scene_upload and mi_bvh_build first");
    if (n == 0) return MI_OK;
    HIP_TRY(c, hipSetDevice(c->device));
    TmpBuf<float> in; TmpBuf<mi_surface_interaction> out;
    HIP_TRY(c, in.resize(8 * n)); HIP_TRY(c, out.resize(n));
    const float *src[8] = { rays->ox, rays->oy, rays->oz, rays->dx, rays->dy, rays->dz, rays->mint, rays->maxt };
    for (int k = 0; k < 8; ++k) {
        if (!src[k]) return fail(c, MI_ERR_INVALID, "mi_ray_intersect: null ray array");
        HIP_TRY(c, hipMemcpyAsync(in.p + k * n, src[k], n * sizeof(float), hipMemcpyHostToDevice, c->stream));
    }
    SoaRays R = { in.p, in.p + n, in.p + 2 * n, in.p + 3 * n, in.p + 4 * n, in.p + 5 * n, in.p + 6 * n, in.p + 7 * n };
    hipLaunchKernelGGL(k_ray_intersect, dim3((unsigned) ((n + MIW_BLOCK - 1) / MIW_BLOCK)), dim3(MIW_BLOCK), c->lds_bytes, c->stream, c->view, R, out.p, n, c->lds_cfg);
    HIP_TRY(c, hipGetLastError());
    HIP_TRY(c, hipMemcpyAsync(si, out.p, n * sizeof(mi_surface_interaction), hipMemcpyDeviceToHost, c->stream));
    HIP_TRY(c, hipStreamSynchronize(c->stream));
    return MI_OK;
}

mi_status mi_sample_emitter_direction(mi_ctx *c, int32_t emitter, const float *ref_p, const float *sample, const float *wavelengths,
                                      int32_t test_visibility, mi_direction_sample *ds, float *spec_out, uint64_t n) {
    if (!c || !ref_p || !sample || !ds || !spec_out) return MI_ERR_INVALID;
    if (!c->have_bvh) return fail(c, MI_ERR_STATE, "mi_sample_emitter_direction: call mi_scene_upload and mi_bvh_build first");
    if (emitter >= (int32_t) c->emitters.size()) return fail(c, MI_ERR_INVALID, "mi_sample_emitter_direction: emitter index out of range");
    if (MIW_SPECTRAL && !wavelengths) return fail(c, MI_ERR_INVALID, "mi_sample_emitter_direction: the scalar_spectral library needs wavelengths");
    if (n == 0) return MI_OK;
    HIP_TRY(c, hipSetDevice(c->device));
    TmpBuf<float> d_ref, d_smp, d_wl, d_spec; TmpBuf<mi_direction_sample> d_ds;
    HIP_TRY(c, d_ref.resize(3 * n)); HIP_TRY(c, d_smp.resize(2 * n)); HIP_TRY(c, d_spec.resize(MIW_SPEC_N * n)); HIP_TRY(c, d_ds.resize(n));
    HIP_TRY(c, hipMemcpyAsync(d_ref.p, ref_p, 3 * n * sizeof(float), hipMemcpyHostToDevice, c->stream));
    HIP_TRY(c, hipMemcpyAsync(d_smp.p, sample, 2 * n * sizeof(float), hipMemcpyHostToDevice, c->stream));
    if (MIW_SPECTRAL) {
        HIP_TRY(c, d_wl.resize(4 * n));
        HIP_TRY(c, hipMemcpyAsync(d_wl.p, wavelengths, 4 * n * sizeof(float), hipMemcpyHostToDevice, c->stream));
    }
    hipLaunchKernelGGL(k_sample_emitter_direction, dim3((unsigned) ((n + MIW_BLOCK - 1) / MIW_BLOCK)), dim3(MIW_BLOCK), c->lds_bytes, c->stream,
                       c->view, emitter, d_ref.p, d_smp.p, d_wl.p, test_visibility, d_ds.p, d_spec.p, n, c->lds_cfg);
    HIP_TRY(c, hipGetLastError());
    HIP_TRY(c, hipMemcpyAsync(ds, d_ds.p, n * sizeof(mi_direction_sample), hipMemcpyDeviceToHost, c->stream));
    HIP_TRY(c, hipMemcpyAsync(spec_out, d_spec.p, MIW_SPEC_N * n * sizeof(float), hipMemcpyDeviceToHost, c->stream));
    HIP_TRY(c, hipStreamSynchronize(c->stream));
    return MI_OK;
}

mi_status mi_pdf_emitter_direction(mi_ctx *c, int32_t emitter, const float *ref_p, const mi_direction_sample *ds, float *pdf, uint64_t n) {
    if (!c || !ref_p || !ds || !pdf) return MI_ERR_INVALID;
    if (!c->have_bvh) return fail(c, MI_ERR_STATE, "mi_pdf_emitter_direction: call mi_scene_upload and mi_bvh_build first");
    if (emitter >= (int32_t) c->emitters.size()) return fail(c, MI_ERR_INVALID, "mi_pdf_emitter_direction: emitter index out of range");
    if (n == 0) return MI_OK;
    HIP_TRY(c, hipSetDevice(c->device));
    TmpBuf<float> d_ref, d_pdf; TmpBuf<mi_direction_sample> d_ds;
    HIP_TRY(c, d_ref.resize(3 * n)); HIP_TRY(c, d_pdf.resize(n)); HIP_TRY(c, d_ds.resize(n));
    HIP_TRY(c, hipMemcpyAsync(d_ref.p, ref_p, 3 * n * sizeof(float), hipMemcpyHostToDevice, c->stream));
    HIP_TRY(c, hipMemcpyAsync(d_ds.p, ds, n * sizeof(mi_direction_sample), hipMemcpyHostToDevice, c->stream));
    hipLaunchKernelGGL(k_pdf_emitter_direction, dim3((unsigned) ((n + 255) / 256)), dim3(256), 0, c->stream, c->view, emitter, d_ref.p, d_ds.p, d_pdf.p, n);
    HIP_TRY(c, hipGetLastError());
    HIP_TRY(c, hipMemcpyAsync(pdf, d_pdf.p, n * sizeof(float), hipMemcpyDeviceToHost, c->stream));
    HIP_TRY(c, hipStreamSynchronize(c->stream));
    return MI_OK;
}

mi_status mi_emitter_eval(mi_ctx *c, const mi_surface_interaction *si, const float *wavelengths, float *spec_out, uint64_t n) {
    if (!c || !si || !spec_out) return MI_ERR_INVALID;
    if (!c->have_bvh) return fail(c, MI_ERR_STATE, "mi_emitter_eval: call mi_scene_upload and mi_bvh_build first");
    if (MIW_SPECTRAL && !wavelengths) return fail(c, MI_ERR_INVALID, "mi_emitter_eval: the scalar_spectral library needs wavelengths");
    if (n == 0) return MI_OK;
    HIP_TRY(c, hipSetDevice(c->device));
    TmpBuf<float> d_wl, d_spec; TmpBuf<mi_surface_interaction> d_si;
    HIP_TRY(c, d_spec.resize(MIW_SPEC_N * n)); HIP_TRY(c, d_si.resize(n));
    HIP_TRY(c, hipMemcpyAsync(d_si.p, si, n * sizeof(mi_surface_interaction), hipMemcpyHostToDevice, c->stream));
    if (MIW_SPECTRAL) {
        HIP_TRY(c, d_wl.resize(4 * n));
        HIP_TRY(c, hipMemcpyAsync(d_wl.p, wavelengths, 4 * n * sizeof(float), hipMemcpyHostToDevice, c->stream));
    }
    hipLaunchKernelGGL(k_emitter_eval, dim3((unsigned) ((n + 255) / 256)), dim3(256), 0, c->stream, c->view, d_si.p, d_wl.p, d_spec.p, n);
    HIP_TRY(c, hipGetLastError());
    HIP_TRY(c, hipMemcpyAsync(spec_out, d_spec.p, MIW_SPEC_N * n * sizeof(float), hipMemcpyDeviceToHost, c->stream));
    HIP_TRY(c, hipStreamSynchronize(c->stream));
    return MI_OK;
}

static void direct_constants(DirectRec &D, uint32_t ne, uint32_t nb, bool hide_emitters) {
    D.emitter_samples = ne; D.bsdf_samples = nb; D.hide_emitters = hide_emitters ? 1u : 0u;
    D.weight_bsdf = 1.f / (float) nb; D.weight_lum = 1.f / (float) ne;
    D.frac_bsdf = (float) nb / (float) (ne + nb); D.frac_lum = (float) ne / (float) (ne + nb);
}
static mi_status fill_params(mi_ctx *c, const mi_render_cfg *cfg, RenderParams &P) {
    if (cfg->crop_w <= 0 || cfg->crop_h <= 0 || cfg->crop_x < 0 || cfg->crop_y < 0)
        return fail(c, MI_ERR_INVALID, "render: bad crop window");
    if (cfg->crop_x + cfg->crop_w > 65535 || cfg->crop_y + cfg->crop_h > 65535)
        return fail(c, MI_ERR_INVALID, "render: film larger than 65535 pixels per side");
    if (cfg->block_size <= 0 || (cfg->block_size & (cfg->block_size - 1)))
        return fail(c, MI_ERR_INVALID, "render: block_size must be a power of two");
    if (cfg->integrator == MI_INTEGRATOR_PATH && cfg->rr_depth <= 0) return fail(c, MI_ERR_INVALID, "\"rr_depth\" must be set to a value greater than zero!");
    if (cfg->integrator == MI_INTEGRATOR_PATH && cfg->max_depth < 0 && cfg->max_depth != -1) return fail(c, MI_ERR_INVALID, "\"max_depth\" must be set to -1 (infinite) or a value >= 0");
    if (cfg->filter_radius <= 0.f || cfg->filter_radius > 4.f) return fail(c, MI_ERR_INVALID, "render: filter radius out of range (0, 4]");
    memset(&P, 0, sizeof P);
    memcpy(P.sensor.sample_to_camera, cfg->sample_to_camera, 64);
    memcpy(P.sensor.to_world, cfg->to_world, 64);
    P.sensor.near_clip = cfg->near_clip; P.sensor.far_clip = cfg->far_clip;
    P.sensor.pp_offset[0] = cfg->principal_point_offset[0]; P.sensor.pp_offset[1] = cfg->principal_point_offset[1];
    P.film.crop_w = cfg->crop_w; P.film.crop_h = cfg->crop_h; P.film.crop_x = cfg->crop_x; P.film.crop_y = cfg->crop_y;
    P.film.block_size = cfg->block_size; P.film.border = cfg->filter_border;
    P.film.radius = cfg->filter_radius;
    P.film.scale_factor = (float) MIW_FILTER_RESOLUTION / cfg->filter_radius;
    memcpy(P.film.lut, cfg->filter_lut, sizeof P.film.lut);
    P.film.warn_negative = cfg->moment_pass ? 0u : 1u;
    P.spp = cfg->spp; P.max_depth = cfg->max_depth; P.rr_depth = cfg->rr_depth;
    if (cfg->integrator == MI_INTEGRATOR_DIRECT) {
        const uint32_t ne = cfg->emitter_samples, nb = cfg->bsdf_samples;
        if (ne + nb == 0) return fail(c, MI_ERR_INVALID, "Must have at least 1 BSDF or emitter sample!");
        P.integrator = INTEG_DIRECT;
        direct_constants(P.direct, ne, nb, cfg->hide_emitters != 0);
    } else if (cfg->integrator != MI_INTEGRATOR_PATH)
        return fail(c, MI_ERR_INVALID, "render: unknown integrator %d", cfg->integrator);
    if (cfg->moment_pass < MI_MOMENT_OFF || cfg->moment_pass > MI_MOMENT_SQUARES) return fail(c, MI_ERR_INVALID, "render: moment_pass must be 0, 1 or 2");
#if MIW_SPECTRAL
    if (cfg->moment_pass) return fail(c, MI_ERR_INVALID, "render: the moment integrator is provided by the scalar_rgb library only");
#endif
    P.moment_pass = (uint32_t) cfg->moment_pass;
    render_params_prepare(P);
    return MI_OK;
}

static_assert(miw_pick::ALL == MATS_ALL && miw_pick::DIFFUSE == MATS_DIFFUSE && miw_pick::PLAIN == MATS_PLAIN && miw_pick::TRIO == MATS_TRIO &&
              miw_pick::NESTED == MATS_NESTED && miw_pick::LIGHTS == MATS_LIGHTS, "kernel_pick.h names the classes by miw/path.h's values");
#define MIW_PATH_TUPLES(X)                                                                                                              \
    X(2, MATS_DIFFUSE, false, INTEG_PATH) X(1, MATS_DIFFUSE, false, INTEG_PATH)    \
    X(1, MATS_LIGHTS, false, INTEG_PATH) X(0, MATS_LIGHTS, true, INTEG_PATH) X(1, MATS_NESTED, false, INTEG_PATH) X(0, MATS_NESTED, true, INTEG_PATH) \
    X(1, MATS_ALL, false, INTEG_PATH) X(0, MATS_ALL, true, INTEG_PATH)                                                                  \
    X(2, MATS_PLAIN, false, INTEG_PATH) X(1, MATS_PLAIN, false, INTEG_PATH) X(0, MATS_PLAIN, false, INTEG_PATH) X(0, MATS_PLAIN, true, INTEG_PATH)
#define MIW_DIRECT_TUPLES(X)                                                                                                            \
    X(1, MATS_LIGHTS, false, INTEG_DIRECT) X(0, MATS_LIGHTS, true, INTEG_DIRECT) X(1, MATS_NESTED, false, INTEG_DIRECT) X(0, MATS_NESTED, true, INTEG_DIRECT) \
    X(1, MATS_ALL, false, INTEG_DIRECT) X(0, MATS_ALL, true, INTEG_DIRECT) X(1, MATS_PLAIN, false, INTEG_DIRECT) X(0, MATS_PLAIN, true, INTEG_DIRECT)
#define MIW_RESIDENT_LIST(X) MIW_PATH_TUPLES(X) MIW_DIRECT_TUPLES(X)
#define MIW_SAMPLE_LIST(X) MIW_PATH_TUPLES(X) X(0, MATS_TRIO, false, INTEG_PATH) MIW_DIRECT_TUPLES(X)
#define MIW_ATOMIC_LIST(X)                                                                                                              \
    X(1, MATS_LIGHTS, false, INTEG_PATH) X(0, MATS_LIGHTS, true, INTEG_PATH) X(1, MATS_NESTED, false, INTEG_PATH) X(0, MATS_NESTED, true, INTEG_PATH) \
    X(1, MATS_ALL, false, INTEG_PATH) X(0, MATS_ALL, true, INTEG_PATH)                                                                  \
    X(1, MATS_LIGHTS, false, INTEG_DIRECT) X(0, MATS_LIGHTS, true, INTEG_DIRECT) X(1, MATS_NESTED, false, INTEG_DIRECT) X(0, MATS_NESTED, true, INTEG_DIRECT) \
    X(1, MATS_ALL, false, INTEG_DIRECT) X(0, MATS_ALL, true, INTEG_DIRECT)
#define MIW_TREE_CLASSES(X, ...) X(MATS_LIGHTS, true, __VA_ARGS__) X(MATS_NESTED, true, __VA_ARGS__) X(MATS_ALL, true, __VA_ARGS__) \
    X(MATS_TRIO, false, __VA_ARGS__) X(MATS_PLAIN, false, __VA_ARGS__) X(MATS_PLAIN, true, __VA_ARGS__)
#define MIW_PHASED_LIST(X) MIW_TREE_CLASSES(X, 4, 2, true) MIW_TREE_CLASSES(X, 4, 2, false) MIW_TREE_CLASSES(X, 4, 1, true) MIW_TREE_CLASSES(X, 4, 1, false) MIW_TREE_CLASSES(X, 3, 1, false)
#define MIW_POOLED_LIST(X) X(MATS_ALL, true, 12, 1) X(MATS_TRIO, false, 12, 1) X(MATS_TRIO, false, 8, 2) X(MATS_PLAIN, false, 12, 1) X(MATS_PLAIN, true, 12, 1)
#define MIW_PICKED(T, M, A) (pick.tiny == (T) && pick.mats == (M) && pick.analytic == (A))

static miw_pick::Facts pick_facts(const mi_ctx *c, const Options &opt) {
    miw_pick::Facts f;
    f.tiny = c->lds_cfg.brute != 0; f.small = c->view.tri_count <= 32u;
    f.diffuse_only = c->diffuse_only; f.trio = c->trio; f.nested = c->nested; f.textured = c->textured; f.lights_on = c->lights_on;
    f.no_rects = c->rects.empty(); f.trio_on = !opt.off("MIW_TRIO");
    return f;
}
static bool tree8_on(const mi_ctx *c, const Options &opt) { return c->view.nodes4 != nullptr && c->nodes8_count != 0u && !opt.off("MIW_BVH8"); }

#define MIW_SAMPLE_CHUNK_HOST (1u << 21)
#define MIW_SAMPLE_CHUNK_DEVICE (1u << 26)
static mi_status sample_launch(mi_ctx *c, const RenderParams &P, const SampleIO &io, hipStream_t s) {
    const bool tiny = c->lds_cfg.brute != 0, direct = P.integrator == INTEG_DIRECT;
    const unsigned waves = direct ? (unsigned) MIW_DIRECT_WAVES : tiny ? 4u : (unsigned) MIW_TREE_WAVES;
    const dim3 grid(std::min<unsigned>((io.n + MIW_BLOCK - 1u) / MIW_BLOCK, (unsigned) c->cu_count * waves)), block(MIW_BLOCK);
    HIP_TRY(c, hipMemsetAsync(c->d_next_ray.p, 0, sizeof(uint32_t), s));
    const miw_pick::Facts facts = pick_facts(c, c->opt);
    const miw_pick::Pick pick = direct ? miw_pick::resident_direct(facts) : miw_pick::resident_path(facts, true);
    const uint32_t integ = direct ? INTEG_DIRECT : INTEG_PATH;
#define MIW_SAMPLE_LAUNCH(T, M, A, I) if (integ == (I) && MIW_PICKED(T, M, A)) hipLaunchKernelGGL((k_sample_rays<T, M, A, I>), grid, block, c->lds_bytes, s, P, c->view, io, c->lds_cfg, c->d_next_ray.p); else
    MIW_SAMPLE_LIST(MIW_SAMPLE_LAUNCH) return fail(c, MI_ERR_STATE, "mi_sample: no k_sample_rays<%d, %d, %d, %u> in the library", pick.tiny, pick.mats, (int) pick.analytic, integ);
#undef MIW_SAMPLE_LAUNCH
    HIP_TRY(c, hipGetLastError());
    return MI_OK;
}

static std::string sample_cfg_problem(const mi_sample_cfg *cfg) {
    char buf[160];
    if (cfg->struct_size != sizeof(mi_sample_cfg)) {
        snprintf(buf, sizeof buf, "mi_sample: unknown mi_sample_cfg::struct_size %u (this library: %zu)", cfg->struct_size, sizeof(mi_sample_cfg));
        return buf;
    }
    if (cfg->integrator == MI_INTEGRATOR_PATH) {
        if (cfg->rr_depth <= 0) return "\"rr_depth\" must be set to a value greater than zero!";
        if (cfg->max_depth < -1) return "\"max_depth\" must be set to -1 (infinite) or a value >= 0";
    } else if (cfg->integrator == MI_INTEGRATOR_DIRECT) {
        if (cfg->emitter_samples + cfg->bsdf_samples == 0) return "Must have at least 1 BSDF or emitter sample!";
    } else {
        snprintf(buf, sizeof buf, "mi_sample: unknown integrator %d (served: MI_INTEGRATOR_PATH, MI_INTEGRATOR_DIRECT)", cfg->integrator);
        return buf;
    }
    return std::string();
}

mi_status mi_sample(mi_ctx *c, const mi_sample_cfg *cfg, const mi_rays_soa *rays, const float *wavelengths,
                    uint64_t *rng_state, const uint64_t *rng_inc, float *spec_out, uint8_t *valid, uint64_t n) {
    if (!cfg) return MI_ERR_INVALID;
    {
        const std::string why = sample_cfg_problem(cfg);
        if (!why.empty()) { if (c) c->error = why; else g_global_error = why; return MI_ERR_INVALID; }
    }
    if (!c) return MI_ERR_INVALID;
    if (!rays || !rng_state || !spec_out || !valid) return fail(c, MI_ERR_INVALID, "mi_sample: null rays / rng_state / spec / valid");
    if (!c->have_bvh) return fail(c, MI_ERR_STATE, "mi_sample: call mi_scene_upload and mi_bvh_build first");
    RenderParams P;
    memset(&P, 0, sizeof P);
    P.spp = 1u; P.max_depth = cfg->max_depth; P.rr_depth = cfg->rr_depth;
    if (cfg->integrator == MI_INTEGRATOR_DIRECT) {
        P.integrator = INTEG_DIRECT;
        direct_constants(P.direct, cfg->emitter_samples, cfg->bsdf_samples, cfg->hide_emitters != 0);
    }
    if (MIW_SPECTRAL && !wavelengths) return fail(c, MI_ERR_INVALID, "mi_sample: the scalar_spectral library needs wavelengths");
    const float *src[8] = { rays->ox, rays->oy, rays->oz, rays->dx, rays->dy, rays->dz, rays->mint, rays->maxt };
    for (int k = 0; k < 8; ++k) if (!src[k]) return fail(c, MI_ERR_INVALID, "mi_sample: null ray array");
    if (n == 0) return MI_OK;
    HIP_TRY(c, hipSetDevice(c->device));
    hipStream_t s = c->stream;
    c->cancel.store(0);
    HIP_TRY(c, c->d_next_ray.resize(1));
    const bool dev = cfg->on_device != 0;
    const uint64_t chunk = dev ? MIW_SAMPLE_CHUNK_DEVICE : MIW_SAMPLE_CHUNK_HOST;
    const uint64_t m_max = std::min<uint64_t>(n, chunk), m_pad = (m_max + 15u) & ~(uint64_t) 15u;
    const size_t off_wl = 8 * m_pad * 4, off_st = off_wl + (MIW_SPECTRAL ? 4 * m_pad * 4 : 0), off_inc = off_st + m_pad * 8,
                 off_spec = off_inc + m_pad * 8, off_valid = off_spec + MIW_SPEC_N * m_pad * 4, stage_bytes = off_valid + m_pad;
    if (!dev) HIP_TRY(c, c->d_sample_stage.resize(stage_bytes));
    for (uint64_t done = 0; done < n; done += chunk) {
        if (c->cancel.load()) return fail(c, MI_ERR_CANCELLED, "mi_sample: cancelled after %llu of %llu rays", (unsigned long long) done, (unsigned long long) n);
        const uint64_t m = std::min<uint64_t>(chunk, n - done);
        SampleIO io;
        io.n = (uint32_t) m;
        if (dev) {
            io.R = { src[0] + done, src[1] + done, src[2] + done, src[3] + done, src[4] + done, src[5] + done, src[6] + done, src[7] + done };
            io.wavelengths = wavelengths ? wavelengths + 4 * done : nullptr;
            io.rng_state = rng_state + done; io.rng_inc = rng_inc ? rng_inc + done : nullptr;
            io.spec = spec_out + MIW_SPEC_N * done; io.valid = valid + done;
        } else {
            unsigned char *b = c->d_sample_stage.p;
            float *f = reinterpret_cast<float *>(b);
            for (int k = 0; k < 8; ++k) HIP_TRY(c, hipMemcpyAsync(f + k * m_pad, src[k] + done, m * sizeof(float), hipMemcpyHostToDevice, s));
            io.R = { f, f + m_pad, f + 2 * m_pad, f + 3 * m_pad, f + 4 * m_pad, f + 5 * m_pad, f + 6 * m_pad, f + 7 * m_pad };
            io.wavelengths = nullptr;
            if (MIW_SPECTRAL) {
                HIP_TRY(c, hipMemcpyAsync(b + off_wl, wavelengths + 4 * done, 4 * m * sizeof(float), hipMemcpyHostToDevice, s));
                io.wavelengths = reinterpret_cast<const float *>(b + off_wl);
            }
            HIP_TRY(c, hipMemcpyAsync(b + off_st, rng_state + done, m * sizeof(uint64_t), hipMemcpyHostToDevice, s));
            io.rng_state = reinterpret_cast<uint64_t *>(b + off_st);
            io.rng_inc = nullptr;
            if (rng_inc) {
                HIP_TRY(c, hipMemcpyAsync(b + off_inc, rng_inc + done, m * sizeof(uint64_t), hipMemcpyHostToDevice, s));
                io.rng_inc = reinterpret_cast<const uint64_t *>(b + off_inc);
            }
            io.spec = reinterpret_cast<float *>(b + off_spec); io.valid = b + off_valid;
        }
        const mi_status ls = sample_launch(c, P, io, s);
        if (ls != MI_OK) return ls;
        if (!dev) {
            HIP_TRY(c, hipMemcpyAsync(rng_state + done, io.rng_state, m * sizeof(uint64_t), hipMemcpyDeviceToHost, s));
            HIP_TRY(c, hipMemcpyAsync(spec_out + MIW_SPEC_N * done, io.spec, MIW_SPEC_N * m * sizeof(float), hipMemcpyDeviceToHost, s));
            HIP_TRY(c, hipMemcpyAsync(valid + done, io.valid, m, hipMemcpyDeviceToHost, s));
        }
        HIP_TRY(c, hipStreamSynchronize(s));
    }
    return MI_OK;
}

struct LaunchTimer {
    struct Stamp { int cls; size_t e0, e1; };
    mi_ctx *c; mi_counters &K; bool on;
    std::vector<Stamp> stamps; size_t ev_used = 0;
    hipError_t get_event(size_t &idx) {
        if (ev_used == c->ev_pool.size()) {
            hipEvent_t e; hipError_t r = hipEventCreate(&e);
            if (r != hipSuccess) return r;
            c->ev_pool.push_back(e);
        }
        idx = ev_used++;
        return hipSuccess;
    }
    void drain() {
        if (!on) return;
        for (const Stamp &t : stamps) {
            float ms = 0.f;
            if (hipEventElapsedTime(&ms, c->ev_pool[t.e0], c->ev_pool[t.e1]) != hipSuccess) continue;
            switch (t.cls) {
                case 0: K.ms_trace_closest += ms; break;
                case 1: K.ms_trace_any += ms; break;
                case 2: K.ms_shade += ms; break;
                case 3: K.ms_init += ms; break;
                case 6: K.ms_path += ms; break;
                case 4: K.ms_film_blocks += ms; K.ms_resolve += ms; break;
                case 5: K.ms_film_merge += ms; K.ms_resolve += ms; break;
                default: K.ms_resolve += ms; break;
            }
        }
        stamps.clear(); ev_used = 0;
    }
};

struct FilmPlan { int film_mode = 0; bool rec16 = false; int film_lanes = 0; uint32_t log_il = 0; size_t log_entries = 0, rec_bytes = 0; };
static mi_status plan_film_log(mi_ctx *c, const mi_render_cfg *cfg, const Options &ropt, const RenderParams &P, hipStream_t s, int plan,
// ... 398 lines not shown
#if MIW_SPECTRAL
    if (cfg->plan == 1) return fail(c, MI_ERR_INVALID, "render: the scalar_spectral library runs the resident plan only (plan 0 or 2)");
    plan = 2;
#endif
    const bool direct = P.integrator == INTEG_DIRECT;
    const uint32_t integ = direct ? INTEG_DIRECT : INTEG_PATH;
    if (direct) {
        if (cfg->plan == 1) return fail(c, MI_ERR_INVALID, "render: the direct integrator runs the resident plan only (plan 0 or 2)");
        plan = 2;
    }
    c->counters.plan = (uint32_t) plan;

    size_t nl = std::max<uint32_t>(n_lanes, 1);
    HIP_TRY(c, c->q_st.resize(nl)); HIP_TRY(c, c->q_pixel.resize(nl));
    if (plan == 1) {
        HIP_TRY(c, c->q_tp.resize(nl)); HIP_TRY(c, c->q_res.resize(nl)); HIP_TRY(c, c->q_ray_o.resize(nl));
        HIP_TRY(c, c->q_ray_d.resize(nl)); HIP_TRY(c, c->q_hit.resize(nl)); HIP_TRY(c, c->q_sh_d.resize(nl));
        HIP_TRY(c, c->q_sh_c.resize(nl)); HIP_TRY(c, c->q_pos.resize(nl)); HIP_TRY(c, c->q_sh_vis.resize(nl));
    }
    HIP_TRY(c, c->d_cnt.resize(MIW_CNT_SHARDS));
    HIP_TRY(c, hipMemsetAsync(c->d_cnt.p, 0, sizeof(Counters) * MIW_CNT_SHARDS, s));

    FilmPlan FP;
    FilmReplay replay;
    { const mi_status fs = plan_film_log(c, cfg, ropt, P, s, plan, n_tiles, n_lanes, bs2, bs2_log2, film_n, FP); if (fs != MI_OK) return fs; }
    const int film_mode = FP.film_mode; const bool rec16 = FP.rec16; const int film_lanes = FP.film_lanes; const uint32_t log_il = FP.log_il;
    HIP_TRY(c, c->d_block_ids.resize(cfg->block_count));
    HIP_TRY(c, hipMemcpyAsync(c->d_block_ids.p, cfg->block_ids, cfg->block_count * sizeof(uint32_t), hipMemcpyHostToDevice, s));
    if (cfg->tile_list && n_tiles) {
        HIP_TRY(c, c->d_tile_list.resize(n_tiles));
        HIP_TRY(c, hipMemcpyAsync(c->d_tile_list.p, cfg->tile_list, n_tiles * sizeof(uint32_t), hipMemcpyHostToDevice, s));
    }

    LaneQueues Q;
    Q.tp = c->q_tp.p; Q.res = c->q_res.p; Q.st = c->q_st.p; Q.pos = c->q_pos.p; Q.pixel = c->q_pixel.p;
    Q.ray_o = c->q_ray_o.p; Q.ray_d = c->q_ray_d.p; Q.hit = c->q_hit.p;
    Q.sh_d = c->q_sh_d.p; Q.sh_c = c->q_sh_c.p; Q.sh_vis = c->q_sh_vis.p;
    Q.log_pos = film_mode == 1 && !rec16 ? c->q_log_pos.p : nullptr; Q.log_val = film_mode == 1 && !rec16 ? c->q_log_val.p : nullptr;
    Q.lane_cost = nullptr; Q.lane_sorted = nullptr; Q.piece_list = nullptr; Q.simd_ids = nullptr; Q.piece_a = 64u; Q.piece_b = 1u;
    Q.log_rec = film_mode == 1 && rec16 ? c->q_log_rec.p : nullptr; Q.log_thr = rec16 ? c->d_fc_thr.p : nullptr; Q.log_rej = rec16 ? c->classes.count | ((film_mode == 1 ? log_il : 0u) << 8) : 0u;
    struct LdsLayout { TraceLds cfg; size_t rlds, rlds_plain, table_bytes; bool tables_fit; };
    const size_t lds_budget4 = MIW_LDS_PER_WORKGROUP - MIW_LDS_STATIC - MIW_LDS_GRANULE;
    auto lay_out = [&](size_t base, size_t env_cap, size_t lds_budget) {
        LdsLayout L; L.cfg = c->lds_cfg; L.rlds = base;
        L.cfg.thr16 = (uint32_t) ((L.rlds + 15) / 16);
        if (rec16) L.rlds = (size_t) L.cfg.thr16 * 16 + (MIW_FC_TABLE + 3) / 4 * 16;
        L.cfg.tab16 = (uint32_t) ((L.rlds + 15) / 16);
        L.table_bytes = lds_table_bytes(c, L.cfg.tab_words, c->lds_cfg.brute != 0);
        L.cfg.light_words = (uint32_t) (c->lights.size() * sizeof(LightRec) / 4);
        L.tables_fit = (size_t) L.cfg.tab16 * 16 + L.table_bytes <= (c->lds_cfg.brute ? 64u * 1024u - MIW_LDS_STATIC - MIW_LDS_GRANULE : lds_budget);
        L.cfg.env_top_count = L.cfg.env_top_base = L.cfg.env_top_words = 0;
        if (L.tables_fit && c->have_env && !ropt.off("MIW_ENV_TOP")) {
            const EnvmapRec &e = c->env_host;
            const size_t used = (size_t) L.cfg.tab16 * 16 + L.table_bytes;
            const size_t room = used < lds_budget ? std::min<size_t>(env_cap, lds_budget - used) : 0;
            uint32_t count = 0;
            while (count + 1 < e.n_levels && ((size_t) c->env_levels_total - e.level_offset[e.n_levels - 1 - count]) * 4 <= room) ++count;
            if (count) {
                L.cfg.env_top_count = count; L.cfg.env_top_base = e.level_offset[e.n_levels - count];
                L.cfg.env_top_words = (uint32_t) (c->env_levels_total - L.cfg.env_top_base);
                L.table_bytes += ((size_t) L.cfg.env_top_words + 3) / 4 * 16;
            }
        }
        L.rlds_plain = L.rlds;
        if (L.tables_fit) L.rlds = (size_t) L.cfg.tab16 * 16 + L.table_bytes;
        return L;
    };
    LdsLayout lay = lay_out(c->lds_bytes, 4096, lds_budget4);
    const miw_pick::Facts facts = pick_facts(c, ropt);
    const bool pre8 = plan == 2 && cfg->integrator != MI_INTEGRATOR_DIRECT && !c->lds_cfg.brute && c->lds_cfg.stack && tree8_on(c, ropt) &&
                      !ropt.off("MIW_PHASED") && ropt.num("MIW_PHASED_WAVES", 4) == 4 && film_mode == 1;
    bool stack8_sized = false;
    if (pre8 && !ropt.on("MIW_STACK8_FULL")) {
        const size_t base8 = (size_t) c->lds_cfg.stack16 * 16 + (size_t) std::max<uint32_t>(c->nodes8_depth, 2u) * MIW_BLOCK * sizeof(U2);
        const LdsLayout lay8 = lay_out(base8, 12288, lds_budget4);
        if (lay8.tables_fit && base8 <= c->lds_bytes) { lay = lay8; stack8_sized = true; }
    }
    LdsLayout layp{}; bool pooled_fits = false;
    int pool_nw = 12, pool_pp = 1;
    if (const char *e = ropt.get("MIW_POOL_SHAPE")) { int a = 0, b = 0; if (sscanf(e, "%dx%d", &a, &b) == 2 && ((a == 12 && b == 1) || (a == 8 && b == 2))) { pool_nw = a; pool_pp = b; } }
    if (!miw_pick::trio_kernel(facts)) { pool_nw = 12; pool_pp = 1; }
    if (pre8 && ropt.on("MIW_POOLED")) {
        const size_t NJ = (size_t) pool_nw * pool_pp * 64u;
        size_t base = (size_t) std::max<uint32_t>(c->nodes8_depth, 2u) * NJ * sizeof(U2);
        const uint32_t pool16 = (uint32_t) (base / 16); base += 5u * NJ * 16u;
        const uint32_t stat16 = (uint32_t) (base / 16); base += NJ;
        layp = lay_out(base, 32768, (size_t) 160u * 1024u - 1024u);
        layp.cfg.stack16 = 0u; layp.cfg.pool16 = pool16; layp.cfg.stat16 = stat16; layp.cfg.nodes_staged = layp.cfg.tris_staged = 0u;
        pooled_fits = layp.tables_fit;
        if (ropt.get("MIW_DEBUG")) fprintf(stderr, "[miwave] pooled phase machine: %d wavefronts per workgroup x %d pixels per lane, LDS %zu bytes (stacks %zu, job records %zu, tables %zu of which environment warp levels %u), fits %d\n",
                                         pool_nw, pool_pp, layp.rlds, (size_t) pool16 * 16, 5u * NJ * 16u, layp.table_bytes, layp.cfg.env_top_words * 4u, (int) pooled_fits);
    }
    TraceLds rcfg = lay.cfg; size_t rlds = lay.rlds; const size_t rlds_plain = lay.rlds_plain, table_bytes = lay.table_bytes; const bool tables_fit = lay.tables_fit;
    if (MIW_LDS_TABLES && c->lds_cfg.brute && !tables_fit) return fail(c, MI_ERR_STATE, "render: the tables of this packet scene do not fit a workgroup's LDS");
    auto lds_workgroups = [](size_t dyn) -> uint32_t {
        const size_t per = (dyn + MIW_LDS_STATIC + 16u + MIW_LDS_GRANULE - 1u) / MIW_LDS_GRANULE * MIW_LDS_GRANULE;
        return (uint32_t) (MIW_LDS_PER_CU / per);
    };
    if (ropt.get("MIW_DEBUG")) fprintf(stderr, "[miwave] LDS per workgroup: %zu bytes dynamic with the scene tables (%zu without), tables %zu B of which environment warp levels %u B and built frame tables %u B, budget %zu%s; + %u static: %u workgroups per CU by LDS\n",
                                     rlds, rlds_plain, table_bytes, rcfg.env_top_words * 4u, (rcfg.tab_words[10] + rcfg.tab_words[11]) * 4u, lds_budget4, stack8_sized ? "; stack sized for the 8-wide tree's depth" : "",
                                     MIW_LDS_STATIC + 16u, lds_workgroups(rlds));

    mi_counters &K = c->counters;
    K.samples = K.segments = K.shadow_rays = K.iterations = 0; K.lanes = n_lanes;
    K.ms_trace_closest = K.ms_trace_any = K.ms_shade = K.ms_init = K.ms_resolve = K.ms_path = K.ms_film_blocks = K.ms_film_merge = K.ms_film_pack = 0;
    K.n_trace_closest = K.n_trace_any = K.n_shade = K.n_path = 0; K.path_kernel = 0; K.placed = 0; K.tree_width = 0; K.pooled = 0; K.pool_waves = 0; K.film_overlapped = 0; K.film_groups = 0; K.job_chunk = 0; K.job_chunks = 0; c->replay_enqueued = false; K.place_cost_max = K.place_cost_unit = K.place_max_pixel = K.place_measure_spp = 0; K.place_cost_mean = 0.0;

    LaunchTimer T{ c, K, cfg->profile != 0 };
#define MIW_TIMED(cls_, launch) do {                                                   \
        size_t e0_ = 0, e1_ = 0;                                                       \
        if (T.on) { HIP_TRY(c, T.get_event(e0_)); HIP_TRY(c, hipEventRecord(c->ev_pool[e0_], s)); } \
        launch;                                                                        \
        if (T.on) { HIP_TRY(c, T.get_event(e1_)); HIP_TRY(c, hipEventRecord(c->ev_pool[e1_], s)); \
                    T.stamps.push_back({ cls_, e0_, e1_ }); }                          \
    } while (0)

    mi_status result = MI_OK;
    auto read_counters = [&](Counters &sum) -> mi_status {
        HIP_TRY(c, hipMemcpyAsync(c->h_cnt, c->d_cnt.p, sizeof(Counters) * MIW_CNT_SHARDS, hipMemcpyDeviceToHost, s));
        HIP_TRY(c, hipStreamSynchronize(s));
        sum.segments = sum.samples = sum.shadow_rays = sum.active_lanes = 0;
        for (int i = 0; i < MIW_CNT_SHARDS; ++i) {
            sum.segments += c->h_cnt[i].segments; sum.samples += c->h_cnt[i].samples;
            sum.shadow_rays += c->h_cnt[i].shadow_rays; sum.active_lanes += c->h_cnt[i].active_lanes;
        }
        K.samples = sum.samples; K.segments = sum.segments; K.shadow_rays = sum.shadow_rays;
        return MI_OK;
    };
    auto out_of_time = [&]() {
        return cfg->timeout_s > 0.f &&
               std::chrono::duration<double>(std::chrono::steady_clock::now() - wall0).count() > cfg->timeout_s;
    };
    if (n_lanes > 0 && plan == 2) {
        dim3 grid((n_lanes + MIW_BLOCK - 1) / MIW_BLOCK), block(MIW_BLOCK);
        InitArgs A; A.block_ids = c->d_block_ids.p; A.tile_list = cfg->tile_list ? c->d_tile_list.p : nullptr;
        A.blocks_x = blocks_x; A.blocks_y = blocks_y; A.bs = bs; A.bs2_log2 = bs2_log2; A.base_seed = cfg->base_seed;
        MIW_TIMED(3, hipLaunchKernelGGL(k_init_pixels, grid, block, 0, s, P, c->q_st.p, c->q_pixel.p, A));
        HIP_TRY(c, hipGetLastError());
        const uint32_t n_simd = (uint32_t) c->cu_count * 4u;
        HIP_TRY(c, c->d_next_pixel.resize(std::max<uint32_t>(8u, n_simd)));
        const uint32_t per_launch = cfg->samples_per_launch > 0 ? (uint32_t) cfg->samples_per_launch : 128u;
        const bool tiny = facts.tiny;
        const bool phased_on = !ropt.off("MIW_PHASED");
        const bool trio_kernel = miw_pick::trio_kernel(facts);
        const bool phased = phased_on && !direct && !tiny && c->lds_cfg.stack && (c->view.nodes4 != nullptr || trio_kernel) && (tables_fit || !MIW_LDS_TABLES);
        const int ph_waves = ropt.num("MIW_PHASED_WAVES", 4) == 4 ? 4 : 3;
        const bool phased_placeable = phased && c->view.nodes4 != nullptr && ph_waves == 4;
        const bool phased8 = phased_placeable && tree8_on(c, ropt);
        if (stack8_sized && !phased8) return fail(c, MI_ERR_STATE, "render: the LDS stack was sized for the 8-wide walk, which this launch does not run");
        SceneView view8 = c->view;
        if (phased8) { view8.nodes8 = c->d_nodes8.p; view8.tris = c->d_tris8.p; if (view8.tri_vn) view8.tri_vn = c->d_tri_vn8.p; }
        bool packet_shard4 = !phased && tiny && c->diffuse_only && !MIW_SPECTRAL && !direct && c->view.tri_count <= 32u && MIW_PACKET_WAVES > 4 && film_mode == 1 && n_lanes <= 64u * 4u * n_simd;
        if (ropt.off("MIW_PACKET_SHARD4")) packet_shard4 = false;
        const uint32_t res_waves_compiled = phased ? (uint32_t) ph_waves : !tiny ? (uint32_t) MIW_TREE_WAVES : (c->diffuse_only && !MIW_SPECTRAL ? (c->view.tri_count <= 32u && !packet_shard4 ? (uint32_t) MIW_PACKET_WAVES : 4u) : (uint32_t) MIW_PACKET_WAVES_ALL);
        const uint32_t res_waves = tiny && film_mode == 1 ? std::max(1u, std::min(res_waves_compiled, lds_workgroups(rlds))) : res_waves_compiled;
        bool place = film_mode == 1 && !direct && (tiny || phased_placeable) && n_lanes >= 64u * n_simd / 2u && n_lanes <= 64u * res_waves * n_simd &&
                     cfg->spp >= 128u && per_launch >= cfg->spp && cfg->timeout_s <= 0.f;
        if (ropt.off("MIW_PLACE")) place = false;
        uint32_t measure_div = (uint32_t) std::max(2, ropt.num("MIW_PLACE_MEASURE", 8));
        const uint32_t measure_end = place ? std::max<uint32_t>(16u, cfg->spp / measure_div) : 0u;
        const uint32_t n_pieces = (n_lanes + 63u) / 64u;
        size_t place_tmp_bytes = 0;
        if (place) {
            HIP_TRY(c, c->d_lane_cost.resize(n_lanes)); HIP_TRY(c, c->d_cost_sorted.resize(n_lanes)); HIP_TRY(c, c->d_lane_iota.resize(n_lanes));
            HIP_TRY(c, c->d_lane_sorted.resize((size_t) n_pieces * 64u));
            HIP_TRY(c, c->d_piece_list.resize((size_t) n_simd * MIW_PLACE_PIECES)); HIP_TRY(c, c->d_simd_ids.resize(1u + (1u << 14)));
            HIP_TRY(c, hipMemsetAsync(c->d_lane_cost.p, 0, n_lanes * sizeof(uint32_t), s));
            HIP_TRY(c, hipMemsetAsync(c->d_lane_sorted.p, 0xff, (size_t) n_pieces * 64u * sizeof(uint32_t), s));
            HIP_TRY(c, hipMemsetAsync(c->d_simd_ids.p, 0, c->d_simd_ids.n * sizeof(uint32_t), s));
            hipLaunchKernelGGL(k_iota, dim3((n_lanes + 255u) / 256u), dim3(256), 0, s, c->d_lane_iota.p, n_lanes);
            HIP_TRY(c, rocprim::radix_sort_pairs_desc(nullptr, place_tmp_bytes, c->d_lane_cost.p, c->d_cost_sorted.p, c->d_lane_iota.p, c->d_lane_sorted.p, (size_t) n_lanes, 0u, 32u, s));
            HIP_TRY(c, c->d_place_tmp.resize(place_tmp_bytes + 16));
        }
        TileArgs TA; memset(&TA, 0, sizeof TA);
        size_t tile_bytes = 0;
        if (film_mode == 2 && bs >= 16) {
            TA.tile_list = A.tile_list; TA.blocks_x = blocks_x; TA.bs = bs; TA.bs2_log2 = bs2_log2;
            TA.side = 16u + 2u * std::max<uint32_t>((uint32_t) cfg->filter_border, (uint32_t) floorf(cfg->filter_radius + .5f));
            TA.geom16 = (uint32_t) ((c->lds_bytes + 15) / 16);
            tile_bytes = (size_t) TA.geom16 * 16 - c->lds_bytes + (size_t) TA.side * TA.side * MIW_FILM_CHANNELS * sizeof(double);
            if (c->lds_bytes + tile_bytes > 64 * 1024) {
#define MIW_ATOMIC_ATTR(T, M, A, I) HIP_TRY(c, hipFuncSetAttribute((const void *) k_path_resident<false, T, M, A, I>, hipFuncAttributeMaxDynamicSharedMemorySize, (int) (c->lds_bytes + tile_bytes)));
                MIW_ATOMIC_LIST(MIW_ATOMIC_ATTR)
#undef MIW_ATOMIC_ATTR
            }
        }
        const uint32_t sync_every = 8;
        uint32_t launches = 0;
        bool place_stats_due = false;
        const int overlap_mode = ropt.num("MIW_FILM_OVERLAP", 0);
        const bool overlap = overlap_mode != 0 && c->overlap_state != 0 && film_mode == 1 && FP.rec16 && FP.film_lanes != 0 && FP.log_il != 0 && !place && !phased  && tiny && c->diffuse_only && !MIW_SPECTRAL && !direct  &&
                             per_launch >= cfg->spp && cfg->timeout_s <= 0.f && n_tiles > 0;
        for (uint32_t done = 0; done < cfg->spp; ) {
            uint32_t end = cfg->spp - done < per_launch ? cfg->spp : done + per_launch;
            if (film_mode == 1) {
                HIP_TRY(c, hipMemsetAsync(c->d_next_pixel.p, 0, c->d_next_pixel.n * sizeof(uint32_t), s));
                rcfg.queues = 1u; Q.lane_cost = nullptr; Q.lane_sorted = nullptr; Q.piece_list = nullptr; Q.simd_ids = nullptr;
                if (overlap && done == 0) {
                    mi_status os = film_replay_setup(c, cfg, s, FP, n_tiles, bs, bs2_log2, blocks_x, blocks_y, replay);
                    if (os == MI_OK) os = overlap_prepare(c, cfg, s, n_tiles, bs, blocks_x, Q, bs2_log2);
                    if (os != MI_OK) return os;
                    if (Q.group_done) HIP_TRY(c, hipEventRecord(c->ev_fork, s));
                }
                Q.job_chunk = Q.job_pow = Q.job_total = 0u; Q.job_min = 0x80000000u;
                if ((tiny || (phased && MIW_PHASED_JOBS != 0)) && !pooled_fits && !place && !overlap && done == 0 && per_launch >= cfg->spp && cfg->timeout_s <= 0.f) {
                    uint32_t jmin = tiny ? 64u : 32u;
                    if (const char *e = ropt.get("MIW_JOB_CHUNK")) { const uint32_t v = (uint32_t) std::max(0, atoi(e)); jmin = (v & (v - 1u)) ? 0u : v; }
                    bool enough = (uint64_t) n_lanes * 5u >= (uint64_t) 6u * 64u * res_waves * n_simd;
                    if (ropt.on("MIW_JOB_CHUNK_FORCE")) enough = true;
                    uint32_t pow2 = 1u;
                    while (pow2 * 2u < cfg->spp) pow2 *= 2u;
                    uint64_t chunks = 1u;
                    for (uint32_t r = pow2; jmin && r >= jmin && r < cfg->spp; r >>= 1) ++chunks;
                    if (jmin && enough && chunks >= 2u && (uint64_t) n_lanes * chunks < (1ull << 31)) {
                        Q.job_chunk = jmin; Q.job_min = jmin; Q.job_pow = pow2; Q.job_total = (uint32_t) ((uint64_t) n_lanes * chunks);
                        K.job_chunk = jmin; K.job_chunks = (uint32_t) chunks;
                    }
                }
                if (place && done == 0) { end = measure_end; Q.lane_cost = c->d_lane_cost.p; Q.simd_ids = c->d_simd_ids.p; }
                else if (place) {
                    HIP_TRY(c, rocprim::radix_sort_pairs_desc(c->d_place_tmp.p, place_tmp_bytes, c->d_lane_cost.p, c->d_cost_sorted.p, c->d_lane_iota.p, c->d_lane_sorted.p, (size_t) n_lanes, 0u, 32u, s));
                    bool spread = phased && ((phased8 ? (size_t) c->nodes8_count * sizeof(Bvh8Node) : (size_t) c->nodes4_count * sizeof(Bvh4Node)) + (size_t) c->view.tri_count * sizeof(Tri)) > ((size_t) 32 << 20);
                    if (const char *e = ropt.get("MIW_PLACE_SPREAD")) spread = atoi(e) != 0;
                    Q.piece_a = spread ? 1u : 64u; Q.piece_b = spread ? n_pieces : 1u;
                    std::vector<uint32_t> &ids = c->h_simd_ids;
                    ids.resize(c->d_simd_ids.n);
                    HIP_TRY(c, hipMemcpyAsync(ids.data(), c->d_simd_ids.p, ids.size() * sizeof(uint32_t), hipMemcpyDeviceToHost, s));
                    HIP_TRY(c, hipStreamSynchronize(s));
                    place_stats_due = cfg->profile != 0;
                    uint32_t nqueues = 0;
                    for (size_t k = 1; k < ids.size(); ++k) ids[k] = ids[k] ? nqueues++ : 0xffffffffu;
                    ids[0] = 0u;
                    if (nqueues < 2u || (uint64_t) nqueues * MIW_PLACE_PIECES < n_pieces) nqueues = 0;
                    if (nqueues) {
                    std::vector<uint32_t> &list = c->h_piece_list;
                    list.assign((size_t) nqueues * MIW_PLACE_PIECES, 0xffffffffu);
                    for (uint32_t i = 0; i < n_pieces; ++i) {
                        const uint32_t round = i / nqueues, k = i % nqueues, qd = (round & 1u) ? nqueues - 1u - k : k;
                        list[(size_t) qd * MIW_PLACE_PIECES + round] = i;
                    }
                    HIP_TRY(c, c->d_piece_list.resize(list.size()));
                    HIP_TRY(c, hipMemcpyAsync(c->d_piece_list.p, list.data(), list.size() * sizeof(uint32_t), hipMemcpyHostToDevice, s));
                    HIP_TRY(c, hipMemcpyAsync(c->d_simd_ids.p, ids.data(), ids.size() * sizeof(uint32_t), hipMemcpyHostToDevice, s));
                    rcfg.queues = nqueues; Q.piece_list = c->d_piece_list.p; Q.lane_sorted = c->d_lane_sorted.p; Q.simd_ids = c->d_simd_ids.p;
                    K.placed = 1u;
                    }
                }
                unsigned wg_per_cu = std::max(4u, direct ? 4u : (unsigned) res_waves);
                if (const char *e = ropt.get("MIW_WG_PER_CU")) wg_per_cu = (unsigned) std::max(1, atoi(e));
                unsigned room = 0u;
                if (Q.group_done) { room = 32u; if (const char *e = ropt.get("MIW_FILM_OVERLAP_ROOM")) room = (unsigned) std::max(0, atoi(e)); }
                const unsigned resident = (unsigned) c->cu_count * (direct ? (unsigned) MIW_DIRECT_WAVES : (unsigned) res_waves);
                const unsigned full = room ? std::min((unsigned) c->cu_count * wg_per_cu, resident) : (unsigned) c->cu_count * wg_per_cu;
                const dim3 pgrid(std::min<unsigned>(grid.x, full > 2u * room ? full - room : full));
                K.path_kernel = phased ? (c->view.nodes4 ? 1u : 3u) : 0u;
                const dim3 phgrid(std::min<unsigned>(grid.x, (unsigned) c->cu_count * (unsigned) ph_waves));
                rcfg.tail_prio = 1u;
                if (ropt.off("MIW_TAIL_PRIO")) rcfg.tail_prio = 0u;
                TraceLds ph_cfg = rcfg;
                ph_cfg.shade_num = 2; ph_cfg.shade_den = c->have_env ? 4 : 3;
                if (const char *e = ropt.get("MIW_SHADE_VOTE")) { int a = 0, b = 0; if (sscanf(e, "%d:%d", &a, &b) == 2 && a > 0 && b > 0) { ph_cfg.shade_num = (uint32_t) a; ph_cfg.shade_den = (uint32_t) b; } }
                ph_cfg.node_exit = c->have_env ? 2u : 1u; ph_cfg.tri_exit = c->have_env ? 3u : 2u;
                if (const char *e = ropt.get("MIW_LOOP_EXIT")) { int a = 0, b = 0; if (sscanf(e, "%d:%d", &a, &b) == 2 && a >= 0 && b >= 0) { ph_cfg.node_exit = (uint32_t) a; ph_cfg.tri_exit = (uint32_t) b; } }
#define MIW_PHASED_LAUNCH_(M, A, WV, W, PL) MIW_TIMED(6, hipLaunchKernelGGL((k_path_phased<M, A, MIW_PHASE_SPEC != 0, WV, W, PL>), phgrid, block, rlds, s, P, (W) == 2 ? view8 : c->view, Q, c->d_cnt.p, ph_cfg, end, c->d_next_pixel.p))
#define MIW_PHASED_LAUNCH(M, A, W) do { if (ph_waves == 4) MIW_PHASED_LAUNCH_(M, A, 4, W, false); else MIW_PHASED_LAUNCH_(M, A, 3, W, false); } while (0)
                K.tree_width = phased ? (phased8 ? 8u : (c->view.nodes4 ? 4u : 2u)) : 0u;
#if MIW_SPECTRAL
                const bool pooled = false;
                if (pooled) { }
#else
                const bool pooled = phased8 && !place && pooled_fits;
                if (pooled) {
                    TraceLds pcfg = layp.cfg; pcfg.queues = 1u; pcfg.tail_prio = ph_cfg.tail_prio;
                    pcfg.shade_num = 48; pcfg.shade_den = 16; pcfg.node_exit = 40u; pcfg.tri_exit = 20u; pcfg.pool_claim_min = 8u;
                    if (const char *e = ropt.get("MIW_POOL_VOTE")) { int a = 0, b = 0, n = 0, t = 0, m = 0; if (sscanf(e, "%d:%d:%d:%d:%d", &a, &b, &n, &t, &m) == 5 && a > 0 && b >= 0) { pcfg.shade_num = (uint32_t) a; pcfg.shade_den = (uint32_t) b; pcfg.node_exit = (uint32_t) n; pcfg.tri_exit = (uint32_t) t; pcfg.pool_claim_min = (uint32_t) std::max(m, 1); } }
                    const unsigned NL = (unsigned) pool_nw * 64u;
                    const dim3 qgrid(std::min<unsigned>((n_lanes + NL - 1u) / NL, (unsigned) c->cu_count)), qblock(NL);
                    SceneView pview = view8;
                    if (c->lights_on) return fail(c, MI_ERR_INVALID, "render: the pooled kernel (MI_PATH_KERNEL_POOLED) does not serve scenes with point / spot / directional / constant emitters");
                    if (c->nested) return fail(c, MI_ERR_INVALID, "render: the pooled kernel (MI_PATH_KERNEL_POOLED) does not serve scenes with mask / blendbsdf / null / thindielectric records");
                    const miw_pick::Pick pick = miw_pick::tree_class(facts);
#define MIW_POOLED_LAUNCH(M, A, NW_, PP_) if (pick.mats == (M) && pick.analytic == (A) && pool_nw == (NW_) && pool_pp == (PP_)) { \
                        HIP_TRY(c, hipFuncSetAttribute((const void *) k_path_pooled<M, A, NW_, PP_>, hipFuncAttributeMaxDynamicSharedMemorySize, (int) layp.rlds)); \
                        MIW_TIMED(6, hipLaunchKernelGGL((k_path_pooled<M, A, NW_, PP_>), qgrid, qblock, layp.rlds, s, P, pview, Q, c->d_cnt.p, pcfg, end, c->d_next_pixel.p)); } else
                    MIW_POOLED_LIST(MIW_POOLED_LAUNCH) return fail(c, MI_ERR_STATE, "render: no k_path_pooled<%d, %d, %d, %d> in the library", pick.mats, (int) pick.analytic, pool_nw, pool_pp);
#undef MIW_POOLED_LAUNCH
                    K.pooled = 1u; K.pool_waves = (uint32_t) pool_nw;
                }
#endif
                else
                if (phased && !c->view.nodes4) MIW_PHASED_LAUNCH(MATS_TRIO, false, 0);
                else if (phased) {
                    const miw_pick::Pick pick = miw_pick::tree_class(facts);
                    const int wide = phased8 ? 2 : 1;
#define MIW_PHASED_PICKED(M, A, WV, W, PL) if (pick.mats == (M) && pick.analytic == (A) && ph_waves == (WV) && wide == (W) && place == (PL)) MIW_PHASED_LAUNCH_(M, A, WV, W, PL); else
                    MIW_PHASED_LIST(MIW_PHASED_PICKED) return fail(c, MI_ERR_STATE, "render: no k_path_phased<%d, %d, ., %d, %d, %d> in the library", pick.mats, (int) pick.analytic, ph_waves, wide, (int) place);
#undef MIW_PHASED_PICKED
                }
#undef MIW_PHASED_LAUNCH
#undef MIW_PHASED_LAUNCH_
                else if (Q.group_done && c->view.tri_count <= 32u)
                    MIW_TIMED(6, hipLaunchKernelGGL((k_path_resident<true, 2, MATS_DIFFUSE, false, INTEG_PATH, true>), pgrid, block, rlds, s, P, c->view, Q, (double *) nullptr, c->d_cnt.p, rcfg, end, TA, c->d_next_pixel.p));
                else if (Q.group_done)
                    MIW_TIMED(6, hipLaunchKernelGGL((k_path_resident<true, 1, MATS_DIFFUSE, false, INTEG_PATH, true>), pgrid, block, rlds, s, P, c->view, Q, (double *) nullptr, c->d_cnt.p, rcfg, end, TA, c->d_next_pixel.p));
                else if (packet_shard4 && !Q.group_done)
                    MIW_TIMED(6, hipLaunchKernelGGL((k_path_resident<true, 2, MATS_DIFFUSE, false, INTEG_PATH, false, 4>), pgrid, block, rlds, s, P, c->view, Q, (double *) nullptr, c->d_cnt.p, rcfg, end, TA, c->d_next_pixel.p));
                else {
                    const miw_pick::Pick pick = direct ? miw_pick::resident_direct(facts) : miw_pick::resident_path(facts, false);
#define MIW_RESIDENT_LAUNCH(T, M, A, I) if (integ == (I) && MIW_PICKED(T, M, A)) MIW_TIMED(6, hipLaunchKernelGGL((k_path_resident<true, T, M, A, I>), pgrid, block, (T) != 0 ? rlds : rlds_plain, s, P, c->view, Q, (double *) nullptr, c->d_cnt.p, rcfg, end, TA, c->d_next_pixel.p)); else
                    MIW_RESIDENT_LIST(MIW_RESIDENT_LAUNCH) return fail(c, MI_ERR_STATE, "render: no k_path_resident<true, %d, %d, %d, %u> in the library", pick.tiny, pick.mats, (int) pick.analytic, integ);
#undef MIW_RESIDENT_LAUNCH
                }
            } else {
                const miw_pick::Pick pick = miw_pick::resident_atomic(facts);
#define MIW_ATOMIC_LAUNCH(T, M, A, I) if (integ == (I) && MIW_PICKED(T, M, A)) MIW_TIMED(6, hipLaunchKernelGGL((k_path_resident<false, T, M, A, I>), grid, block, c->lds_bytes + tile_bytes, s, P, c->view, Q, c->d_accum.p, c->d_cnt.p, c->lds_cfg, end, TA, (uint32_t *) nullptr)); else
                MIW_ATOMIC_LIST(MIW_ATOMIC_LAUNCH) return fail(c, MI_ERR_STATE, "render: no k_path_resident<false, %d, %d, %d, %u> in the library", pick.tiny, pick.mats, (int) pick.analytic, integ);
#undef MIW_ATOMIC_LAUNCH
            }
            if (Q.group_done) {
                const mi_status os = overlap_enqueue(c, ropt, P, s, T, replay, n_tiles, overlap_mode != 2);
                if (os != MI_OK) return os;
                if (c->replay_enqueued) { K.film_overlapped = 1u; K.film_groups = c->replay_launches; }
                Q.group_done = nullptr; Q.group_expected = nullptr; Q.group_flag = nullptr;
            }
            K.n_path++; K.iterations++;
            done = end;
            if ((++launches % sync_every == 0 || cfg->timeout_s > 0.f || c->cancel.load()) && done < cfg->spp) {
                HIP_TRY(c, hipGetLastError());
                HIP_TRY(c, hipStreamSynchronize(s));
                T.drain();
                if (c->cancel.load() || out_of_time()) { result = MI_ERR_CANCELLED; break; }
            }
        }
        HIP_TRY(c, hipGetLastError());
        Counters sum;
        mi_status rs = read_counters(sum);
        if (rs != MI_OK) return rs;
        if (place_stats_due) {
            std::vector<uint32_t> all(n_lanes); uint32_t first_lane = 0, px = 0;
            HIP_TRY(c, hipMemcpyAsync(all.data(), c->d_cost_sorted.p, (size_t) n_lanes * sizeof(uint32_t), hipMemcpyDeviceToHost, s));
            HIP_TRY(c, hipMemcpyAsync(&first_lane, c->d_lane_sorted.p, sizeof(uint32_t), hipMemcpyDeviceToHost, s));
            HIP_TRY(c, hipStreamSynchronize(s));
            if (first_lane < n_lanes) HIP_TRY(c, hipMemcpy(&px, c->q_pixel.p + first_lane, sizeof(uint32_t), hipMemcpyDeviceToHost));
            double csum = 0.0; uint32_t with = 0;
            for (uint32_t v : all) if (v) { csum += (double) v; ++with; }
            K.place_cost_max = all.empty() ? 0u : all[0]; K.place_cost_mean = with ? csum / with : 0.0; K.place_max_pixel = px;
            K.place_cost_unit = phased ? 1u : 0u; K.place_measure_spp = measure_end;
        }
        if (K.placed && ropt.get("MIW_DEBUG")) {
            std::vector<uint32_t> cur(n_simd), ids(1u + (1u << 14)), cost(n_pieces);
            (void) hipMemcpy(cur.data(), c->d_next_pixel.p, n_simd * sizeof(uint32_t), hipMemcpyDeviceToHost);
            (void) hipMemcpy(ids.data(), c->d_simd_ids.p, ids.size() * sizeof(uint32_t), hipMemcpyDeviceToHost);
            (void) hipMemcpy2D(cost.data(), sizeof(uint32_t), c->d_cost_sorted.p, Q.piece_a * sizeof(uint32_t), sizeof(uint32_t), n_pieces, hipMemcpyDeviceToHost);
            uint32_t keys = 0, key_or = 0, full = 0, over = 0; uint64_t csum = 0; uint32_t cmin = ~0u, cmax = 0;
            for (uint32_t k = 0; k < (1u << 14); ++k) if (ids[1 + k] != 0xffffffffu) { ++keys; key_or |= k; }
            ids[0] = keys;
            for (uint32_t v : cur) { full += v >= 64u * MIW_PLACE_PIECES; over += v > 64u * MIW_PLACE_PIECES; }
            for (uint32_t v : cost) { csum += v; cmin = std::min(cmin, v); cmax = std::max(cmax, v); }
            fprintf(stderr, "[miwave] placed queues: %u SIMDs numbered, %u distinct hardware keys (bits used 0x%x), %u of %u queues drained (%u asked beyond their end), "
                            "cost of the dearest pixel of a piece min / mean / max = %u / %.0f / %u (iterations, or 256-cycle units)\n", ids[0], keys, key_or, full, n_simd, over, cmin, (double) csum / n_pieces, cmax);
        }
        print_debug_statistics(c, ropt, K);
        T.drain();
    }
#if !MIW_SPECTRAL
    else if (n_lanes > 0) {
        dim3 grid((n_lanes + MIW_BLOCK - 1) / MIW_BLOCK), block(MIW_BLOCK);
        InitArgs A; A.block_ids = c->d_block_ids.p; A.tile_list = cfg->tile_list ? c->d_tile_list.p : nullptr;
        A.blocks_x = blocks_x; A.blocks_y = blocks_y; A.bs = bs; A.bs2_log2 = bs2_log2; A.base_seed = cfg->base_seed;
        const size_t n_wg = grid.x, seg_lanes = n_wg * MIW_BLOCK;
        HIP_TRY(c, c->d_lists.resize((size_t) 2 * WL_LISTS * seg_lanes));
        HIP_TRY(c, c->d_list_counts.resize(2 * WL_LISTS * n_wg));
        HIP_TRY(c, hipMemsetAsync(c->d_list_counts.p, 0, 2 * WL_LISTS * n_wg * sizeof(uint32_t), s));
        WorkLists WL[2];
        for (int p = 0; p < 2; ++p) {
            for (int l = 0; l < WL_LISTS; ++l) WL[p].list[l] = c->d_lists.p + ((size_t) p * WL_LISTS + l) * seg_lanes;
            WL[p].count = c->d_list_counts.p + (size_t) p * WL_LISTS * n_wg;
        }
        MIW_TIMED(3, hipLaunchKernelGGL(k_init_lanes, grid, block, 0, s, P, Q, c->q_pixel.p, A, WL[0]));
        HIP_TRY(c, hipGetLastError());

        const bool stream_on = !ropt.off("MIW_STREAM");
        const bool stream = stream_on && c->lds_cfg.stack && !c->lds_cfg.brute && c->lds_cfg.nodes_staged == 0;
        K.path_kernel = stream ? 2u : 0u;
        const bool stream8 = stream && tree8_on(c, ropt);
        SceneView pview = c->view;
        if (stream8) { pview.nodes8 = c->d_nodes8.p; pview.tris = c->d_tris8.p; if (pview.tri_vn) pview.tri_vn = c->d_tri_vn8.p; }
        K.tree_width = stream8 ? 8u : 0u;
        if (stream) {
            HIP_TRY(c, c->d_next_pixel.resize(1));
            HIP_TRY(c, hipMemsetAsync(c->d_next_pixel.p, 0, sizeof(uint32_t), s));
        }
        const dim3 sgrid(std::min<unsigned>(grid.x, (unsigned) c->cu_count * (stream8 ? 4u : (unsigned) MIW_STREAM_WAVES)));
        const int check_every = 16;
        bool first = true;
        unsigned long long active_prev = 0;
        uint32_t parity = 0;
        for (;;) {
            for (int it = 0; it < check_every; ++it, parity ^= 1u) {
                const WorkLists &cur = WL[parity], &nxt = WL[parity ^ 1u];
                if (stream) {
                    if (stream8) MIW_TIMED(0, hipLaunchKernelGGL(k_trace_stream<2>, sgrid, block, c->lds_bytes, s, pview, Q, c->lds_cfg, cur, (uint32_t) n_wg, c->d_next_pixel.p));
                    else MIW_TIMED(0, hipLaunchKernelGGL(k_trace_stream<0>, sgrid, block, c->lds_bytes, s, pview, Q, c->lds_cfg, cur, (uint32_t) n_wg, c->d_next_pixel.p));
                    MIW_TIMED(1, hipLaunchKernelGGL(k_sort_hits, grid, block, 0, s, pview, Q, cur, c->d_next_pixel.p));
                    K.n_trace_closest++; K.n_trace_any++;
                } else {
                    if (!first) {
                        MIW_TIMED(1, hipLaunchKernelGGL(k_trace<true>, grid, block, c->lds_bytes, s, c->view, Q, c->lds_cfg, cur));
                        K.n_trace_any++;
                    }
                    MIW_TIMED(0, hipLaunchKernelGGL(k_trace<false>, grid, block, c->lds_bytes, s, c->view, Q, c->lds_cfg, cur));
                    K.n_trace_closest++;
                }
                const uint32_t count_active = it == check_every - 1 ? 1u : 0u;
                if (film_mode == 1)
                    MIW_TIMED(2, hipLaunchKernelGGL(k_shade<true>, grid, block, 0, s, P, pview, Q, (double *) nullptr, c->d_cnt.p, count_active, cur, nxt));
                else
                    MIW_TIMED(2, hipLaunchKernelGGL(k_shade<false>, grid, block, 0, s, P, pview, Q, c->d_accum.p, c->d_cnt.p, count_active, cur, nxt));
                K.n_shade++; K.iterations++;
                first = false;
            }
            HIP_TRY(c, hipGetLastError());
            Counters sum;
            mi_status rs = read_counters(sum);
            if (rs != MI_OK) return rs;
            T.drain();
            unsigned long long active_now = sum.active_lanes - active_prev;
            active_prev = sum.active_lanes;
            if (active_now == 0) break;
            if (c->cancel.load()) { result = MI_ERR_CANCELLED; break; }
            if (out_of_time()) { result = MI_ERR_CANCELLED; break; }
        }
    }
#endif

    { const mi_status fs = assemble_film(c, cfg, ropt, P, s, T, FP, n_tiles, bs, bs2_log2, blocks_x, blocks_y, film_n, film, result, c->replay_enqueued ? &replay : nullptr); c->replay_enqueued = false; if (fs != MI_OK) return fs; }
#undef MIW_TIMED
    K.ms_render = std::chrono::duration<double, std::milli>(std::chrono::steady_clock::now() - wall0).count();
    if (result == MI_ERR_CANCELLED) c->error = "render cancelled";
    return result;
}

mi_status mi_eval(mi_ctx *c, int32_t op, const mi_render_cfg *cfg, const float *in, int32_t is, float *out, int32_t os, uint64_t n) {
    if (!c || !in || !out || is <= 0 || os <= 0) return MI_ERR_INVALID;
    if (n == 0) return MI_OK;
    RenderParams P; memset(&P, 0, sizeof P);
    if (op == MI_EVAL_CAMERA_RAY) {
        if (!cfg) return fail(c, MI_ERR_INVALID, "mi_eval: camera ray needs a render cfg");
        mi_status st = fill_params(c, cfg, P);
        if (st != MI_OK) return st;
    }
    if ((op == MI_EVAL_BSDF || op == MI_EVAL_EMITTER_SAMPLE || op == MI_EVAL_ENVMAP || op == MI_EVAL_TEXTURE) && !c->have_bvh)
        return fail(c, MI_ERR_STATE, "mi_eval: scene required");
    HIP_TRY(c, hipSetDevice(c->device));
    TmpBuf<float> din, dout;
    HIP_TRY(c, din.resize(n * is)); HIP_TRY(c, dout.resize(n * os));
    HIP_TRY(c, hipMemcpyAsync(din.p, in, n * is * sizeof(float), hipMemcpyHostToDevice, c->stream));
    HIP_TRY(c, hipMemsetAsync(dout.p, 0, n * os * sizeof(float), c->stream));
    hipLaunchKernelGGL(k_eval, dim3((unsigned) ((n + 255) / 256)), dim3(256), 0, c->stream, op, P, c->view, din.p, is, dout.p, os, n);
    HIP_TRY(c, hipGetLastError());
    HIP_TRY(c, hipMemcpyAsync(out, dout.p, n * os * sizeof(float), hipMemcpyDeviceToHost, c->stream));
    HIP_TRY(c, hipStreamSynchronize(c->stream));
    return MI_OK;
}

__global__ void k_selftest_rcp(unsigned long long *mismatches) {
    unsigned long long bad = 0;
    const uint32_t stride = gridDim.x * blockDim.x;
    for (uint64_t i = blockIdx.x * blockDim.x + threadIdx.x; i < (1ull << 32); i += stride) {
        const float x = u2f((uint32_t) i);
        volatile float one = 1.f;
        const float ref = one / x, got = miw::rcp(x), got_l = miw::rcp_loop(x);
        if (f2u(ref) != f2u(got) && !(ref != ref && got != got)) ++bad;
        if (f2u(ref) != f2u(got_l) && !(ref != ref && got_l != got_l)) ++bad;
    }
    bad = wave_sum(bad);
    if ((threadIdx.x & 63) == 0 && bad) atomicAdd(mismatches, bad);
// ... 23 lines not shown
```

Measured before the change: 4801.

## Add lean packet path kernels compiled without env, normals and moment features

Adds a Feat template mask threaded through path_step, surface interaction and emitter sampling. Branches for environment maps, shape and emitter vertex normals and the moment pass can then be compiled out. The host works out which features the scene needs and, for packet diffuse and plain scenes needing none, launches a FEAT_NONE instantiation. This is meant to cut register pressure and dead branches in the hot kernel, at the cost of more kernel instantiations and binary size.

```diff
diff --git a/mitsuba2_amd/csrc/device/resident_kernel.h b/mitsuba2_amd/csrc/device/resident_kernel.h
--- a/mitsuba2_amd/csrc/device/resident_kernel.h
+++ b/mitsuba2_amd/csrc/device/resident_kernel.h
@@ -191,7 +191,7 @@
 #ifndef MIW_PACKET_WAVES
 #define MIW_PACKET_WAVES 5
 #endif
-template <bool UseLog, int Tiny, int Mats = MATS_ALL, bool Analytic = (Tiny == 0), uint32_t Integ = INTEG_PATH, bool Groups = false, int Waves = 0>
+template <bool UseLog, int Tiny, int Mats = MATS_ALL, bool Analytic = (Tiny == 0), uint32_t Integ = INTEG_PATH, bool Groups = false, int Waves = 0, uint32_t Feat = FEAT_ALL>
 __global__ __launch_bounds__(MIW_BLOCK, Waves ? Waves : Integ == INTEG_DIRECT ? MIW_DIRECT_WAVES : Tiny ? ((Mats == MATS_DIFFUSE && !MIW_SPECTRAL) ? (Tiny == 2 ? MIW_PACKET_WAVES : 4) : MIW_PACKET_WAVES_ALL) : MIW_TREE_WAVES) void k_path_resident(RenderParams P, SceneView sc, LaneQueues Q, double *accum, Counters *cnt,
                                                                TraceLds cfg, uint32_t sample_end, TileArgs T, uint32_t *next_pixel) {
     extern __shared__ uint4 smem[];
@@ -228,7 +228,7 @@
         __shared__ uint32_t s_prog[MIW_BLOCK / 64];
         if (cfg.tail_prio) work.enable_tail_prio(sample_end, &s_prog[threadIdx.x >> 6]);
         if constexpr (Integ == INTEG_DIRECT) pixel_stream_render_direct<Mats, Analytic>(P, sc, sample_end, work, tr2, &local);
-        else pixel_stream_render<Mats, Analytic, Frames>(P, sc, sample_end, work, tr2, &local);
+        else pixel_stream_render<Mats, Analytic, Frames, Feat>(P, sc, sample_end, work, tr2, &local);
     } else if (lane < P.n_lanes) {
         U4 st = Q.st[lane];
         if (!(st.z & LF_DONE)) {
diff --git a/mitsuba2_amd/csrc/kernel_pick.h b/mitsuba2_amd/csrc/kernel_pick.h
--- a/mitsuba2_amd/csrc/kernel_pick.h
+++ b/mitsuba2_amd/csrc/kernel_pick.h
@@ -48,4 +48,13 @@
     return { 0, PLAIN, !f.no_rects };
 }
 
+enum : unsigned { FEAT_ENV = 1u, FEAT_SHAPE_NORMALS = 2u, FEAT_EMITTER_NORMALS = 4u, FEAT_MOMENT = 8u, FEAT_ALL = 15u, FEAT_NONE = 0u };
+
+inline unsigned packet_features(bool has_env, bool shape_normals, bool emitter_normals, bool moment) {
+    return (has_env ? FEAT_ENV : 0u) | (shape_normals ? FEAT_SHAPE_NORMALS : 0u) | (emitter_normals ? FEAT_EMITTER_NORMALS : 0u) | (moment ? FEAT_MOMENT : 0u);
 }
+inline bool packet_features_exist(unsigned mask) { return mask == FEAT_ALL || mask == FEAT_NONE; }
+inline unsigned packet_features_kernel(unsigned needed, bool lean_on) { return lean_on && packet_features_exist(needed) ? needed : (unsigned) FEAT_ALL; }
+inline bool packet_lean_class(const Pick &p) { return p.tiny != 0 && !p.analytic && (p.mats == DIFFUSE || p.mats == PLAIN); }
+
+}
diff --git a/mitsuba2_amd/csrc/miw/path.h b/mitsuba2_amd/csrc/miw/path.h
--- a/mitsuba2_amd/csrc/miw/path.h
+++ b/mitsuba2_amd/csrc/miw/path.h
@@ -104,7 +104,7 @@
     L.flags = 1u | LF_RAY_ACTIVE;
 }
 
-template <typename Sink>
+template <uint32_t Feat = FEAT_ALL, typename Sink>
 MIW_HD void lane_finish_sample(const RenderParams &P, uint32_t pixel, LaneRegs &L, Sink sink) {
 #if MIW_SPECTRAL
     V3 xyz = spectrum_to_xyz(L.ray_weight * L.res, L.wl);
@@ -112,7 +112,7 @@
     V3 xyz = srgb_to_xyz(L.res);
 #endif
     float aovs[5] = { xyz.x, xyz.y, xyz.z, (L.flags & LF_VALID_RAY) ? 1.f : 0.f, 1.f };
-    if (P.moment_pass) {
+    if ((Feat & FEAT_MOMENT) && P.moment_pass) {
         const float sq[3] = { sqr(xyz.x), sqr(xyz.y), sqr(xyz.z) };
         bool ok = true;
         for (int k = 0; k < 3; ++k) ok = ok && isfinite_(aovs[k]) && isfinite_(sq[k]);
@@ -238,7 +238,7 @@
 MIW_HD constexpr bool mats_full(int mats) { return mats == MATS_ALL || mats == MATS_NESTED || mats == MATS_LIGHTS; }
 MIW_HD constexpr bool mats_nested(int mats) { return mats == MATS_NESTED || mats == MATS_LIGHTS; }
 MIW_HD constexpr bool mats_lights(int mats) { return mats == MATS_LIGHTS; }
-template <int Mats = MATS_ALL, bool Analytic = true, bool Frames = false, typename PrevO, typename Cnt>
+template <int Mats = MATS_ALL, bool Analytic = true, bool Frames = false, uint32_t Feat = FEAT_ALL, typename PrevO, typename Cnt>
 MIW_HD int path_step(const RenderParams &P, const SceneView &sc, LaneRegs &L, F4 h, PrevO prev_o,
                      ShadowOut &sh, Cnt *cnt_local) {
     sh.has = false;
@@ -250,8 +250,8 @@
     SurfaceInteraction si;
     uint32_t bsdf_index = 0;
     int32_t emitter = -1;
-    if (valid) hit_surface_interaction<Analytic, mats_full(Mats), Frames>(sc, tri_idx, h.x, h.y, h.z, prev_o, ray_d, si, bsdf_index, emitter);
-    else emitter = miss_emitter<mats_lights(Mats)>(sc);
+    if (valid) hit_surface_interaction<Analytic, mats_full(Mats), Frames, Feat>(sc, tri_idx, h.x, h.y, h.z, prev_o, ray_d, si, bsdf_index, emitter);
+    else emitter = miss_emitter<mats_lights(Mats), Feat>(sc);
     if (depth == 1 && valid) L.flags |= LF_VALID_RAY;
     MIW_SECTION(7);
 
@@ -268,11 +268,11 @@
                     d = d / dist;
                     n = si.sh.n;
                 }
-                emitter_pdf = pdf_emitter_direction<Analytic, mats_lights(Mats)>(sc, (uint32_t) emitter, d, dist, n, ref_p);
+                emitter_pdf = pdf_emitter_direction<Analytic, mats_lights(Mats), Feat>(sc, (uint32_t) emitter, d, dist, n, ref_p);
             }
             emission_weight = mis_weight(L.prev_pdf, emitter_pdf);
         }
-        Spec radiance = valid ? emitter_eval(sc.emitters[emitter], si.wi, L.wl) : miss_eval<mats_lights(Mats)>(sc, ray_d, L.wl);
+        Spec radiance = valid ? emitter_eval(sc.emitters[emitter], si.wi, L.wl) : miss_eval<mats_lights(Mats), Feat>(sc, ray_d, L.wl);
         L.res = L.res + emission_weight * L.tp * radiance;
     }
 
@@ -302,7 +302,7 @@
 
     if (bflags & BSDF_Smooth) {
         DirectionSample ds;
-        Spec emitter_val = sample_emitter_direction<Analytic, mats_lights(Mats), Frames>(sc, si.p, next_2d(L.rng), ds, L.wl);
+        Spec emitter_val = sample_emitter_direction<Analytic, mats_lights(Mats), Frames, Feat>(sc, si.p, next_2d(L.rng), ds, L.wl);
         if (ds.pdf != 0.f) {
             V3 wo = to_local(si.sh, ds.d);
             Spec bsdf_val = Mats == MATS_DIFFUSE ? diffuse_eval(*bsdf.b, si.wi, wo, tc) : bsdf_side_eval<Ext, Trio, Nested>(bsdf, si.wi, wo, tc);
@@ -387,7 +387,7 @@
 }
 #endif
 
-template <int Mats = MATS_ALL, bool Analytic = true, bool Frames = false, typename Work, typename Trace2, typename Cnt>
+template <int Mats = MATS_ALL, bool Analytic = true, bool Frames = false, uint32_t Feat = FEAT_ALL, typename Work, typename Trace2, typename Cnt>
 MIW_HD void pixel_stream_render(const RenderParams &P, const SceneView &sc, uint32_t sample_end, Work &work,
                                 Trace2 trace2, Cnt *cnt_local) {
     LaneRegs L;
@@ -421,13 +421,13 @@
         sh.has = false;
         int r = STEP_FINISHED;
         if (!dead_pending) {
-            r = path_step<Mats, Analytic, Frames>(P, sc, L, h, [o]() { return o; }, sh, cnt_local);
+            r = path_step<Mats, Analytic, Frames, Feat>(P, sc, L, h, [o]() { return o; }, sh, cnt_local);
             MIW_SECTION(4);
             if (r == STEP_DEAD_PENDING) { dead_pending = true; continue; }
             if (r == STEP_CONTINUE) continue;
         }
         dead_pending = false;
-        lane_finish_sample(P, pixel, L, sink);
+        lane_finish_sample<Feat>(P, pixel, L, sink);
         if (cnt_local) cnt_local->samples++;
         L.flags = 0;
         lane_begin_sample(P, pixel, L, work.job_end(L.sample_idx, sample_end));
diff --git a/mitsuba2_amd/csrc/miw/scene.h b/mitsuba2_amd/csrc/miw/scene.h
--- a/mitsuba2_amd/csrc/miw/scene.h
+++ b/mitsuba2_amd/csrc/miw/scene.h
@@ -4,6 +4,7 @@
 #include "bsdf.h"
 #include "envmap.h"
 #include "light.h"
+#include "../kernel_pick.h"
 
 namespace miw {
 
@@ -35,6 +36,8 @@
     uint32_t type;
 };
 enum : uint32_t { SHAPE_HAS_NORMALS = 1u, SHAPE_HAS_TEXCOORDS = 8u };
+enum : uint32_t { FEAT_ENV = miw_pick::FEAT_ENV, FEAT_SHAPE_NORMALS = miw_pick::FEAT_SHAPE_NORMALS, FEAT_EMITTER_NORMALS = miw_pick::FEAT_EMITTER_NORMALS,
+                  FEAT_MOMENT = miw_pick::FEAT_MOMENT, FEAT_ALL = miw_pick::FEAT_ALL, FEAT_NONE = miw_pick::FEAT_NONE };
 
 struct SceneView {
     const BvhNode *nodes;   uint32_t node_count;
@@ -71,7 +74,7 @@
 
 MIW_HD PrimCtx prim_ctx(const SceneView &sc) { PrimCtx c; c.rects = sc.rects; c.accept_pad = sc.accept_pad; return c; }
 
-template <bool Analytic, bool Texcoords, bool Frames = false, typename RayO>
+template <bool Analytic, bool Texcoords, bool Frames = false, uint32_t Feat = FEAT_ALL, typename RayO>
 MIW_HD void hit_surface_interaction(const SceneView &sc, uint32_t tri_idx, float t, float u, float v, RayO ray_o, V3 ray_d,
                                     SurfaceInteraction &si, uint32_t &bsdf_index, int32_t &emitter) {
     const Tri &tr = sc.tris[tri_idx];
@@ -81,7 +84,7 @@
         if (a.kind == ANALYTIC_SPHERE) compute_surface_interaction_sphere(a, t, ray_o(), ray_d, si);
         else compute_surface_interaction_rect(a, t, u, v, ray_o(), ray_d, si);
     } else {
-        const float *vn = (shape.flags & 1u) ? sc.tri_vn + 9 * (size_t) tri_idx : nullptr;
+        const float *vn = ((Feat & FEAT_SHAPE_NORMALS) && (shape.flags & 1u)) ? sc.tri_vn + 9 * (size_t) tri_idx : nullptr;
         const float *tc = (Texcoords && (shape.flags & SHAPE_HAS_TEXCOORDS)) ? sc.tri_uv + 6 * (size_t) tr.prim : nullptr;
         if constexpr (Frames) compute_surface_interaction(ld3(tr.p0), ld3(tr.p1), ld3(tr.p2), vn, tc, sc.tri_frames[tri_idx], t, u, v, ray_d, si);
         else compute_surface_interaction(ld3(tr.p0), ld3(tr.p1), ld3(tr.p2), vn, tc, t, u, v, ray_d, si);
@@ -92,17 +95,18 @@
 
 struct DirectionSample { V3 p, n, d; float dist, pdf; uint32_t emitter; bool delta; };
 
-template <bool Lights = false>
+template <bool Lights = false, uint32_t Feat = FEAT_ALL>
 MIW_HD int32_t miss_emitter(const SceneView &sc) {
-    if (sc.env) return (int32_t) sc.env->emitter_index;
+    if ((Feat & FEAT_ENV) && sc.env) return (int32_t) sc.env->emitter_index;
     if (Lights && sc.constant) return (int32_t) sc.constant->emitter_index;
     return -1;
 }
 
+template <uint32_t Feat = FEAT_ALL>
 MIW_HD MeshSampler emitter_mesh(const SceneView &sc, const EmitterRec &e) {
     MeshSampler m;
     m.tri = sc.emit_tri + 9 * (size_t) e.tri_first;
-    m.vnorm = (e.flags & 1u) ? sc.emit_vnorm + 9 * (size_t) e.tri_first : nullptr;
+    m.vnorm = ((Feat & FEAT_EMITTER_NORMALS) && (e.flags & 1u)) ? sc.emit_vnorm + 9 * (size_t) e.tri_first : nullptr;
     m.pmf = sc.emit_pmf + e.tri_first;
     m.cdf = sc.emit_cdf + e.tri_first;
     m.count = e.tri_count;
@@ -212,7 +216,7 @@
 MIW_HD Spec env_eval_spec(const EnvmapRec &e, V3 d, const Wavelengths &) { return env_eval(e, d); }
 #endif
 
-template <bool Analytic = true, bool Lights = false, bool Frames = false>
+template <bool Analytic = true, bool Lights = false, bool Frames = false, uint32_t Feat = FEAT_ALL>
 MIW_HD Spec emitter_sample_direction(const SceneView &sc, uint32_t index, V3 ref_p, V2 sample, DirectionSample &ds, const Wavelengths &wl) {
     const EmitterRec &e = sc.emitters[index];
     Spec value;
@@ -222,7 +226,7 @@
         LightSample ls;
         value = light_sample_direction(sc.lights[e.tri_first], ref_p, sample, ls, wl);
         ds.p = ls.p; ds.n = ls.n; ds.d = ls.d; ds.dist = ls.dist; ds.pdf = ls.pdf; ds.delta = ls.delta;
-    } else if (e.type == EMITTER_ENVMAP) {
+    } else if ((Feat & FEAT_ENV) && e.type == EMITTER_ENVMAP) {
         value = env_sample_direction_spec(*sc.env, ref_p, sample, ds.d, ds.dist, ds.pdf, ds.p, ds.n, wl, env_top(sc));
     } else {
         if (Analytic && (e.flags & 2u) && sc.rects[e.tri_first].kind == ANALYTIC_SPHERE) {
@@ -230,8 +234,8 @@
         } else {
             PositionSample ps;
             if (Analytic && (e.flags & 2u)) ps = rect_sample_position(sc.rects[e.tri_first], sample);
-            else if constexpr (Frames) ps = mesh_sample_position(emitter_mesh(sc, e), sample, FaceNormalTable{ sc.emit_face_n + 4 * (size_t) e.tri_first });
-            else ps = mesh_sample_position(emitter_mesh(sc, e), sample);
+            else if constexpr (Frames) ps = mesh_sample_position(emitter_mesh<Feat>(sc, e), sample, FaceNormalTable{ sc.emit_face_n + 4 * (size_t) e.tri_first });
+            else ps = mesh_sample_position(emitter_mesh<Feat>(sc, e), sample);
             ds.p = ps.p; ds.n = ps.n; ds.pdf = ps.pdf;
             ds.d = ds.p - ref_p;
             float dist_squared = squared_norm(ds.d);
@@ -247,7 +251,7 @@
     return value;
 }
 
-template <bool Analytic = true, bool Lights = false, bool Frames = false>
+template <bool Analytic = true, bool Lights = false, bool Frames = false, uint32_t Feat = FEAT_ALL>
 MIW_HD Spec sample_emitter_direction(const SceneView &sc, V3 ref_p, V2 sample, DirectionSample &ds, const Wavelengths &wl) {
     if (sc.emitter_count == 0) {
         ds.p = ds.n = ds.d = v3(0.f); ds.dist = 0.f; ds.pdf = 0.f; ds.emitter = 0;
@@ -263,7 +267,7 @@
         index = i < sc.emitter_count - 1 ? i : sc.emitter_count - 1;
         sample.x = (sample.x - (float) index * emitter_pdf) * n;
     }
-    Spec value = emitter_sample_direction<Analytic, Lights, Frames>(sc, index, ref_p, sample, ds, wl);
+    Spec value = emitter_sample_direction<Analytic, Lights, Frames, Feat>(sc, index, ref_p, sample, ds, wl);
     if (sc.emitter_count > 1) {
         ds.pdf *= emitter_pdf;
         value = value * rcp(emitter_pdf);
@@ -271,11 +275,11 @@
     return value;
 }
 
-template <bool Analytic = true, bool Lights = false>
+template <bool Analytic = true, bool Lights = false, uint32_t Feat = FEAT_ALL>
 MIW_HD float emitter_pdf_direction(const SceneView &sc, uint32_t emitter, V3 ds_d, float ds_dist, V3 ds_n, V3 ref_p) {
     const EmitterRec &e = sc.emitters[emitter];
     if (Lights && e.type >= EMITTER_POINT) return light_pdf_direction(sc.lights[e.tri_first]);
-    if (e.type == EMITTER_ENVMAP) return env_pdf_direction(*sc.env, ds_d);
+    if ((Feat & FEAT_ENV) && e.type == EMITTER_ENVMAP) return env_pdf_direction(*sc.env, ds_d);
     float dp = dot(ds_d, ds_n);
     bool active = dp < 0.f;
     float pdf;
@@ -288,9 +292,9 @@
     }
     return active ? pdf : 0.f;
 }
-template <bool Analytic = true, bool Lights = false>
+template <bool Analytic = true, bool Lights = false, uint32_t Feat = FEAT_ALL>
 MIW_HD float pdf_emitter_direction(const SceneView &sc, uint32_t emitter, V3 ds_d, float ds_dist, V3 ds_n, V3 ref_p) {
-    float value = emitter_pdf_direction<Analytic, Lights>(sc, emitter, ds_d, ds_dist, ds_n, ref_p);
+    float value = emitter_pdf_direction<Analytic, Lights, Feat>(sc, emitter, ds_d, ds_dist, ds_n, ref_p);
     if (sc.emitter_count > 1) value = value * sc.emitter_count_inv;
     return value;
 }
@@ -298,9 +302,9 @@
 MIW_HD Spec emitter_eval(const EmitterRec &e, V3 wi, const Wavelengths &wl) {
     return wi.z > 0.f ? tex_eval(e.radiance, wl) : spec(0.f);
 }
-template <bool Lights = false>
+template <bool Lights = false, uint32_t Feat = FEAT_ALL>
 MIW_HD Spec miss_eval(const SceneView &sc, V3 ray_d, const Wavelengths &wl) {
-    if (Lights && !sc.env) return light_eval(*sc.constant, wl);
+    if (Lights && (!(Feat & FEAT_ENV) || !sc.env)) return light_eval(*sc.constant, wl);
     return env_eval_spec(*sc.env, ray_d, wl);
 }
 
diff --git a/mitsuba2_amd/csrc/miwave.hip b/mitsuba2_amd/csrc/miwave.hip
--- a/mitsuba2_amd/csrc/miwave.hip
+++ b/mitsuba2_amd/csrc/miwave.hip
@@ -158,6 +158,7 @@
     { "MIW_PLACE", "0: shards of about one pixel per lane skip the measuring launch + placed queues" },
     { "MIW_JOB_CHUNK", "smallest chunk of a full frame's pixel jobs, in samples (a power of two; default 64, the phase machine 32): the pixels' sample streams are cut into halving chunks drawn chunk-major from one queue; 0: a job = all the samples of a pixel" },
     { "MIW_JOB_CHUNK_FORCE", "1: chunk jobs whatever the frame's size (tests of the hand-over between lanes)" },
+    { "MIW_LEAN", "0: a packet scene without environment map and vertex normals, rendered without the moment integrator, keeps the full path kernel instead of its lean twin (kernel_pick.h: packet_features)" },
     { "MIW_PACKET_SHARD4", "0: a plain-diffuse packet job of at most four wavefronts of pixels per SIMD keeps the five-wavefront (96-register) kernel" },
     { "MIW_PLACE_MEASURE", "divisor: the measuring launch runs spp / divisor samples" },
     { "MIW_PLACE_SPREAD", "0 | 1: placed pieces = consecutive sorted lanes | one lane of every cost stratum" },
@@ -218,6 +219,7 @@
     DevBuf<Bvh8Node> d_nodes8; DevBuf<Tri> d_tris8; DevBuf<float> d_tri_vn8; uint32_t nodes8_count = 0, nodes8_depth = 0;
     DevBuf<float> d_env_data, d_env_levels; DevBuf<EnvmapRec> d_env; EnvmapRec env_host{}; size_t env_levels_total = 0;
     bool have_env = false;
+    bool shape_normals = false, emitter_normals = false;
     SceneView view{};
     TraceLds lds_cfg{}; size_t lds_bytes = 0;
 
@@ -638,6 +640,7 @@
         c->emitters.push_back(r);
     }
     if (!any_emit_normals) c->emit_vnorm.clear();
+    c->shape_normals = any_normals; c->emitter_normals = any_emit_normals;
     if (s->light_count) push_specials();
     else if (s->envmap && s->envmap->emitter_index >= s->emitter_count) push_env();
     if (c->lights_on) { c->nested = c->textured = true; c->diffuse_only = c->trio = false; }
@@ -1218,6 +1221,7 @@
     X(MATS_TRIO, false, __VA_ARGS__) X(MATS_PLAIN, false, __VA_ARGS__) X(MATS_PLAIN, true, __VA_ARGS__)
 #define MIW_PHASED_LIST(X) MIW_TREE_CLASSES(X, 4, 2, true) MIW_TREE_CLASSES(X, 4, 2, false) MIW_TREE_CLASSES(X, 4, 1, true) MIW_TREE_CLASSES(X, 4, 1, false) MIW_TREE_CLASSES(X, 3, 1, false)
 #define MIW_POOLED_LIST(X) X(MATS_ALL, true, 12, 1) X(MATS_TRIO, false, 12, 1) X(MATS_TRIO, false, 8, 2) X(MATS_PLAIN, false, 12, 1) X(MATS_PLAIN, true, 12, 1)
+#define MIW_LEAN_LIST(X) X(2, MATS_DIFFUSE) X(1, MATS_DIFFUSE) X(2, MATS_PLAIN) X(1, MATS_PLAIN)
 #define MIW_PICKED(T, M, A) (pick.tiny == (T) && pick.mats == (M) && pick.analytic == (A))
 
 static miw_pick::Facts pick_facts(const mi_ctx *c, const Options &opt) {
@@ -1922,6 +1926,7 @@
         if (phased8) { view8.nodes8 = c->d_nodes8.p; view8.tris = c->d_tris8.p; if (view8.tri_vn) view8.tri_vn = c->d_tri_vn8.p; }
         bool packet_shard4 = !phased && tiny && c->diffuse_only && !MIW_SPECTRAL && !direct && c->view.tri_count <= 32u && MIW_PACKET_WAVES > 4 && film_mode == 1 && n_lanes <= 64u * 4u * n_simd;
         if (ropt.off("MIW_PACKET_SHARD4")) packet_shard4 = false;
+        const uint32_t feat = miw_pick::packet_features_kernel(miw_pick::packet_features(c->have_env, c->shape_normals, c->emitter_normals, cfg->moment_pass != 0), !ropt.off("MIW_LEAN"));
         const uint32_t res_waves_compiled = phased ? (uint32_t) ph_waves : !tiny ? (uint32_t) MIW_TREE_WAVES : (c->diffuse_only && !MIW_SPECTRAL ? (c->view.tri_count <= 32u && !packet_shard4 ? (uint32_t) MIW_PACKET_WAVES : 4u) : (uint32_t) MIW_PACKET_WAVES_ALL);
         const uint32_t res_waves = tiny && film_mode == 1 ? std::max(1u, std::min(res_waves_compiled, lds_workgroups(rlds))) : res_waves_compiled;
         bool place = film_mode == 1 && !direct && (tiny || phased_placeable) && n_lanes >= 64u * n_simd / 2u && n_lanes <= 64u * res_waves * n_simd &&
@@ -1963,6 +1968,7 @@
                              per_launch >= cfg->spp && cfg->timeout_s <= 0.f && n_tiles > 0;
         for (uint32_t done = 0; done < cfg->spp; ) {
             uint32_t end = cfg->spp - done < per_launch ? cfg->spp : done + per_launch;
+            uint32_t feat_launched = FEAT_ALL;
             if (film_mode == 1) {
                 HIP_TRY(c, hipMemsetAsync(c->d_next_pixel.p, 0, c->d_next_pixel.n * sizeof(uint32_t), s));
                 rcfg.queues = 1u; Q.lane_cost = nullptr; Q.lane_sorted = nullptr; Q.piece_list = nullptr; Q.simd_ids = nullptr;
@@ -2073,10 +2079,17 @@
                     MIW_TIMED(6, hipLaunchKernelGGL((k_path_resident<true, 2, MATS_DIFFUSE, false, INTEG_PATH, true>), pgrid, block, rlds, s, P, c->view, Q, (double *) nullptr, c->d_cnt.p, rcfg, end, TA, c->d_next_pixel.p));
                 else if (Q.group_done)
                     MIW_TIMED(6, hipLaunchKernelGGL((k_path_resident<true, 1, MATS_DIFFUSE, false, INTEG_PATH, true>), pgrid, block, rlds, s, P, c->view, Q, (double *) nullptr, c->d_cnt.p, rcfg, end, TA, c->d_next_pixel.p));
+                else if (packet_shard4 && !Q.group_done && feat == FEAT_NONE) {
+                    feat_launched = FEAT_NONE;
+                    MIW_TIMED(6, hipLaunchKernelGGL((k_path_resident<true, 2, MATS_DIFFUSE, false, INTEG_PATH, false, 4, FEAT_NONE>), pgrid, block, rlds, s, P, c->view, Q, (double *) nullptr, c->d_cnt.p, rcfg, end, TA, c->d_next_pixel.p));
+                }
                 else if (packet_shard4 && !Q.group_done)
                     MIW_TIMED(6, hipLaunchKernelGGL((k_path_resident<true, 2, MATS_DIFFUSE, false, INTEG_PATH, false, 4>), pgrid, block, rlds, s, P, c->view, Q, (double *) nullptr, c->d_cnt.p, rcfg, end, TA, c->d_next_pixel.p));
                 else {
                     const miw_pick::Pick pick = direct ? miw_pick::resident_direct(facts) : miw_pick::resident_path(facts, false);
+#define MIW_LEAN_LAUNCH(T, M) if (feat == FEAT_NONE && !direct && MIW_PICKED(T, M, false)) { feat_launched = FEAT_NONE; MIW_TIMED(6, hipLaunchKernelGGL((k_path_resident<true, T, M, false, INTEG_PATH, false, 0, FEAT_NONE>), pgrid, block, rlds, s, P, c->view, Q, (double *) nullptr, c->d_cnt.p, rcfg, end, TA, c->d_next_pixel.p)); } else
+                    MIW_LEAN_LIST(MIW_LEAN_LAUNCH)
+#undef MIW_LEAN_LAUNCH
 #define MIW_RESIDENT_LAUNCH(T, M, A, I) if (integ == (I) && MIW_PICKED(T, M, A)) MIW_TIMED(6, hipLaunchKernelGGL((k_path_resident<true, T, M, A, I>), pgrid, block, (T) != 0 ? rlds : rlds_plain, s, P, c->view, Q, (double *) nullptr, c->d_cnt.p, rcfg, end, TA, c->d_next_pixel.p)); else
                     MIW_RESIDENT_LIST(MIW_RESIDENT_LAUNCH) return fail(c, MI_ERR_STATE, "render: no k_path_resident<true, %d, %d, %d, %u> in the library", pick.tiny, pick.mats, (int) pick.analytic, integ);
 #undef MIW_RESIDENT_LAUNCH
@@ -2093,6 +2106,7 @@
                 if (c->replay_enqueued) { K.film_overlapped = 1u; K.film_groups = c->replay_launches; }
                 Q.group_done = nullptr; Q.group_expected = nullptr; Q.group_flag = nullptr;
             }
+            if (ropt.get("MIW_DEBUG") && tiny && !phased) fprintf(stderr, "[miwave] packet path kernel launched: scene features 0x%x of 0x%x compiled in (mask chosen for the render: 0x%x)\n", feat_launched, (uint32_t) FEAT_ALL, feat);
             K.n_path++; K.iterations++;
             done = end;
             if ((++launches % sync_every == 0 || cfg->timeout_s > 0.f || c->cancel.load()) && done < cfg->spp) {
```

After: 4936 (median of 6 runs). +2.8%, better.
